# AnishDelft/ModelCompression

Hardware: AMD Instinct MI355X
Metric: images/sec (fwd+bwd, 416x416) (higher is better)
Workload: dtype fp16

## Files before the change

### include/mcamd.h

```cpp
#ifndef MCAMD_H
#define MCAMD_H

#include <stddef.h>
#include <stdint.h>

#ifdef __cplusplus
extern "C" {
#endif

#define MCAMD_OK 0
#define MCAMD_EINVAL (-1)
#define MCAMD_ELAUNCH (-2)
#define MCAMD_EWORKSPACE (-3)

int mcamd_version(void);
void mcamd_reload_config(void);
const char* mcamd_arch(void);
const char* mcamd_last_error(void);

typedef struct mcamd_conv_geom {
    int32_t B, H, W;
    int32_t ksize;
    int32_t cin;
    int32_t cout;
// ... 11 lines not shown
#define MCAMD_EPI_NCHW_F32 1
#define MCAMD_EPI_PAD_F16 2
#define MCAMD_EPI_RAW_F32 3
typedef struct mcamd_conv_epilogue {
    int32_t mode;
    int32_t y_ld, y_choff;
    void* y;
    const float* bias;
    float* stats;
    int32_t stats_rows;
    int32_t stats_ld;
    const float* scale;
    const float* shift;
    float slope;
    int32_t* overflow;
    int32_t dst_mode;
    void* y2;
    int32_t y2_ld, y2_choff;
    int32_t concurrent;
} mcamd_conv_epilogue;

int32_t mcamd_conv_stats_rows(const mcamd_conv_geom* g);
int32_t mcamd_conv_stats_rows_mode(const mcamd_conv_geom* g, int32_t mode);

int mcamd_conv_tile_info(const mcamd_conv_geom* g, int32_t dgrad, int32_t out[4]);

int64_t mcamd_packed_elems_fwd(const mcamd_conv_geom* g);
int64_t mcamd_packed_elems_dgrad(const mcamd_conv_geom* g);

typedef struct mcamd_chan_map {
    const int32_t* rows;
    const int32_t* cols;
} mcamd_chan_map;

int mcamd_pack_weights(const mcamd_conv_geom* g, const float* w_oihw, const float* mask_oihw,
                       const mcamd_chan_map* map, void* wp_fwd, void* wp_dgrad, void* stream);

typedef struct mcamd_pack_job {
    const float* w;
    const float* mask;
    void* dst_fwd;
    void* dst_dgrad;
    const int32_t* rows;
    const int32_t* cols;
    int64_t first_tile;
    int32_t cout, cin, ksize;
    int32_t split;
    int32_t f8_wexp;
} mcamd_pack_job;
int mcamd_pack_weights_many(const mcamd_pack_job* jobs_dev, int32_t njobs, int64_t total_tiles, void* stream);

int mcamd_conv_fwd(const mcamd_conv_geom* g, const void* x, const void* wp_fwd,
                   const mcamd_conv_epilogue* epi, void* stream);

int32_t mcamd_conv_fwd_sparse24_ok(const mcamd_conv_geom* g);
int mcamd_sparse24_elems(const mcamd_conv_geom* g, int64_t out[2]);
int mcamd_pack_sparse24(const mcamd_conv_geom* g, const float* w_oihw, const float* mask_oihw, void* wsp, void* idx, void* stream);
int mcamd_conv_fwd_sparse24(const mcamd_conv_geom* g, const void* x, const void* wsp, const void* idx,
                            const mcamd_conv_epilogue* epi, void* stream);

int32_t mcamd_conv_fwd_q8_ok(const mcamd_conv_geom* g);
int mcamd_q8_elems(const mcamd_conv_geom* g, int64_t out[2]);
int mcamd_pack_q8(const mcamd_conv_geom* g, const float* w_oihw, const float* mask_oihw, void* wq, int32_t* wexp, void* stream);
int mcamd_conv_fwd_q8(const mcamd_conv_geom* g, const void* x8, const void* wq, const int32_t* wexp,
                      const mcamd_conv_epilogue* epi, int32_t y_f8, int32_t y2_f8, void* stream);
int mcamd_cast_q8(const void* src, int64_t pixels, int32_t src_ld, int32_t src_choff, int32_t C, void* dst, int32_t dst_ld,
                  int32_t dst_choff, void* stream);

int32_t mcamd_conv_fwd_q8_stats_rows(const mcamd_conv_geom* g);
int mcamd_fakequant_q8(const mcamd_conv_geom* g, const float* w_oihw, const float* mask_oihw, const int32_t* wexp,
                       float* wq_oihw, void* stream);
int mcamd_cast_q8_train(void* src, int64_t pixels, int32_t src_ld, int32_t src_choff, int32_t C, void* dst, int32_t dst_ld,
                        int32_t dst_choff, void* stream);

int32_t mcamd_conv_fwd_q8_sparse24_ok(const mcamd_conv_geom* g);
int mcamd_q8_sparse24_elems(const mcamd_conv_geom* g, int64_t out[3]);
int mcamd_pack_q8_sparse24(const mcamd_conv_geom* g, const float* w_oihw, const float* mask_oihw, void* wq, void* idx,
                           int32_t* wexp, void* stream);
int mcamd_conv_fwd_q8_sparse24(const mcamd_conv_geom* g, const void* x8, const void* wq, const void* idx, const int32_t* wexp,
                               const mcamd_conv_epilogue* epi, int32_t y_f8, int32_t y2_f8, void* stream);

int mcamd_conv_dgrad(const mcamd_conv_geom* g, const void* dy, int32_t dy_ld, int32_t dy_choff,
                     const void* wp_dgrad, const mcamd_conv_epilogue* epi, void* stream);

size_t mcamd_conv_wgrad_workspace_bytes(const mcamd_conv_geom* g);
int mcamd_conv_wgrad(const mcamd_conv_geom* g, const void* x, const void* dy, int32_t dy_ld,
                     int32_t dy_choff, const float* mask_oihw, const mcamd_chan_map* map,
                     float grad_scale, float* dw_oihw, float* dbias, void* workspace,
                     size_t workspace_bytes, void* stream);

#define MCAMD_WGRAD_GENERIC 0
#define MCAMD_WGRAD_STEM 1
#define MCAMD_WGRAD_WIN 2
#define MCAMD_WGRAD_NINE 3
#define MCAMD_WGRAD_NINE_WIDE 4
#define MCAMD_WFIN_ROW 0
#define MCAMD_WFIN_VEC 1
#define MCAMD_WFIN_GENERIC 2
#define MCAMD_WGRAD_PLAN_INFO_N 13
int mcamd_conv_wgrad_plan_info(const mcamd_conv_geom* g, int32_t has_cmap, int32_t out[MCAMD_WGRAD_PLAN_INFO_N]);
int32_t mcamd_wgrad_generic_instances(int32_t* out, int32_t cap);

int mcamd_bn_coeffs(const float* stats, int32_t stats_rows, int32_t stats_ld, int32_t C, int64_t count,
                    const float* gamma, const float* beta, float* running_mean, float* running_var,
                    float momentum, float eps, int32_t training,
                    float* scale, float* shift, float* save_mean, float* save_invstd,
                    const int32_t* chan_perm, void* stream);

int mcamd_bn_coeffs_ex(const float* stats, int32_t stats_rows, int32_t stats_ld, int32_t C, int64_t count,
                       const float* gamma, const float* beta, float* running_mean, float* running_var,
                       float momentum, float eps, int32_t training,
                       float* scale, float* shift, float* save_mean, float* save_invstd,
                       const int32_t* chan_perm, int32_t ones_channel, void* stream);

#define MCAMD_DST_PLAIN 0
#define MCAMD_DST_POOL 1
#define MCAMD_DST_REORG 2
typedef struct mcamd_act_desc {
    int32_t B, H, W, C;
    const void* y; int32_t y_ld, y_choff;
    const float* scale; const float* shift;
    float slope;
    int32_t mode;
    void* dst; int32_t dst_ld, dst_choff;
    void* dst2; int32_t dst2_ld, dst2_choff;
    int32_t y_dtype;
    int32_t planes;
    int32_t dst_plane, dst2_plane;
    int32_t dst_pad, dst2_pad;
    const float* border;
    int32_t planes2;
    void* pool_act;
    int32_t pool_act_ld, pool_act_pad;
    void* dst_q8;
    void* dst2_q8;
} mcamd_act_desc;
int mcamd_bn_act_fwd(const mcamd_act_desc* d, void* stream);

typedef struct mcamd_act_bwd_desc {
    int32_t B, H, W, C;
    const void* y; int32_t y_ld, y_choff;
    const float* scale; const float* shift; const float* mean; const float* invstd;
    float slope;
    int32_t mode;
    const void* g; int32_t g_ld, g_choff;
    const void* g2; int32_t g2_ld, g2_choff;
    void* dy; int32_t dy_ld, dy_choff;
    float* dgamma; float* dbeta;
    float grad_scale;
    const float* dy_keep;
    const int32_t* chan_perm;
    int32_t y_dtype;
    int32_t* overflow;
    int32_t dy_pad;
    int32_t skip_dead_param_grads;
    const void* act;
    int32_t act_ld, act_choff, act_pad;
    const void* pool_out;
    int32_t pool_out_ld, pool_out_choff, pool_out_pad;
} mcamd_act_bwd_desc;
size_t mcamd_bn_act_bwd_workspace_bytes(const mcamd_act_bwd_desc* d);
int mcamd_bn_act_bwd(const mcamd_act_bwd_desc* d, void* workspace, size_t workspace_bytes, void* stream);

typedef struct mcamd_fold_desc {
    const float* w; const float* mask;
    const int32_t* rows; const int32_t* cols;
    const float* beta; float slope;
    int32_t n, cin_t, cin_k, cin_aug, ksize;
} mcamd_fold_desc;
int mcamd_fold_weights(const mcamd_fold_desc* d, float* waug, void* stream);
typedef struct mcamd_fold_job {
    mcamd_fold_desc d;
    float* waug;
    int64_t first_block;
} mcamd_fold_job;
int mcamd_fold_weights_many(const mcamd_fold_job* jobs_dev, int32_t njobs, int64_t total_blocks, void* stream);
int mcamd_unfold_wgrad(const mcamd_fold_desc* d, const float* dwaug, float* dw_oihw, float* prod_dbeta,
                       float* prod_dgamma, int32_t accumulate, void* stream);

typedef struct mcamd_stem_block_desc {
    int32_t B, H, W;
    const void* x;
    const void* wp;
    const float* gamma; const float* beta;
    float* running_mean; float* running_var;
    float momentum, eps;
    int32_t training;
    float* scale; float* shift; float* save_mean; float* save_invstd;
    float slope;
    void* dst; int32_t dst_ld, dst_choff;
    const void* g; int32_t g_ld, g_choff;
    const float* mask;
    float grad_scale;
    float* dw;
    float* dgamma; float* dbeta;
    int32_t cout;
    int32_t planes;
    const void* x_lo;
    const void* wp_lo;
} mcamd_stem_block_desc;
size_t mcamd_stem_block_workspace_bytes(void);
int mcamd_stem_block_fwd(const mcamd_stem_block_desc* d, void* workspace, size_t workspace_bytes, void* stream);
int mcamd_stem_block_bwd(const mcamd_stem_block_desc* d, void* workspace, size_t workspace_bytes, void* stream);
int32_t mcamd_stem_block_stats_rows(const mcamd_stem_block_desc* d);
int mcamd_stem_block_stats(const mcamd_stem_block_desc* d, float* stats, int32_t stats_rows, int32_t stats_ld, void* stream);

int mcamd_nchw_f32_to_padded_nhwc_f16(const float* src, int32_t B, int32_t C, int32_t H, int32_t W,
                                      float mul, void* dst, int32_t dst_ld, int32_t dst_choff, int32_t* overflow,
                                      void* stream);
int mcamd_nchw_f32_to_padded_nhwc_f16_pad(const float* src, int32_t B, int32_t C, int32_t H, int32_t W,
                                          float mul, void* dst, int32_t dst_ld, int32_t dst_choff, int32_t pad,
                                          int32_t* overflow, void* stream);
int mcamd_nchw_f32_to_padded_nhwc_f16_split(const float* src, int32_t B, int32_t C, int32_t H, int32_t W,
                                            void* dst, int32_t dst_ld, int32_t dst_choff, int32_t plane, void* stream);

int mcamd_nchw_f32_to_nhwc4_split(const float* src, int32_t B, int32_t H, int32_t W, void* hi, void* lo, void* stream);
int mcamd_pack_stem_split(const float* w_oihw, const float* mask_oihw, int32_t cout, void* wp_hi, void* wp_lo, void* stream);

int32_t mcamd_stem_conv_f32_stats_rows(void);
int mcamd_stem_conv_f32(const float* x_nchw, int32_t B, int32_t H, int32_t W, const float* w_oihw,
                        const float* mask_oihw, int32_t cout, float* weff_scratch, float* y, int32_t y_ld,
                        float* stats, int32_t stats_rows, int32_t stats_ld, void* stream);

typedef struct mcamd_region_desc {
    const float* output; const float* target;
    int32_t B, H, W, num_anchors, num_classes, max_boxes;
    float anchors[16];
    float coord_scale, noobject_scale, object_scale, class_scale, thresh;
} mcamd_region_desc;
size_t mcamd_region_loss_workspace_bytes(int32_t B);
int mcamd_region_loss(const mcamd_region_desc* d, float* loss, float* grad, int32_t* counts, void* workspace,
                      size_t workspace_bytes, void* stream);

typedef struct mcamd_augment_desc {
    int64_t src_off;
    int64_t tmp_off;
    int32_t src_w, src_h;
    int32_t crop_x, crop_y;
    int32_t crop_w, crop_h;
    int32_t flip;
    int32_t hk, vk;
    int32_t hcoef_off, vcoef_off;
// ... 50 lines not shown
```

### modelcompression_amd/_lib.py

```python
import ctypes as C
import os

_HERE = os.path.dirname(os.path.abspath(__file__))
LIB_PATH = os.path.join(_HERE, "libmcamd.so")


class McamdError(RuntimeError):
    pass


class ConvGeom(C.Structure):
    _fields_ = [("B", C.c_int32), ("H", C.c_int32), ("W", C.c_int32), ("ksize", C.c_int32),
                ("cin", C.c_int32), ("cout", C.c_int32), ("x_ld", C.c_int32), ("x_choff", C.c_int32),
                ("stem", C.c_int32), ("pad", C.c_int32), ("x_wrap", C.c_int32), ("x_f8", C.c_int32), ("x_f8_wexp", C.c_int32)]


class ConvEpilogue(C.Structure):
    _fields_ = [("mode", C.c_int32), ("y_ld", C.c_int32), ("y_choff", C.c_int32),
                ("y", C.c_void_p), ("bias", C.c_void_p), ("stats", C.c_void_p),
                ("stats_rows", C.c_int32), ("stats_ld", C.c_int32),
                ("scale", C.c_void_p), ("shift", C.c_void_p), ("slope", C.c_float), ("overflow", C.c_void_p),
                ("dst_mode", C.c_int32), ("y2", C.c_void_p), ("y2_ld", C.c_int32), ("y2_choff", C.c_int32),
                ("concurrent", C.c_int32)]


class ActDesc(C.Structure):
    _fields_ = [("B", C.c_int32), ("H", C.c_int32), ("W", C.c_int32), ("C", C.c_int32),
                ("y", C.c_void_p), ("y_ld", C.c_int32), ("y_choff", C.c_int32),
                ("scale", C.c_void_p), ("shift", C.c_void_p), ("slope", C.c_float), ("mode", C.c_int32),
                ("dst", C.c_void_p), ("dst_ld", C.c_int32), ("dst_choff", C.c_int32),
                ("dst2", C.c_void_p), ("dst2_ld", C.c_int32), ("dst2_choff", C.c_int32),
                ("y_dtype", C.c_int32), ("planes", C.c_int32), ("dst_plane", C.c_int32), ("dst2_plane", C.c_int32),
                ("dst_pad", C.c_int32), ("dst2_pad", C.c_int32), ("border", C.c_void_p), ("planes2", C.c_int32),
                ("pool_act", C.c_void_p), ("pool_act_ld", C.c_int32), ("pool_act_pad", C.c_int32),
                ("dst_q8", C.c_void_p), ("dst2_q8", C.c_void_p)]


class ChanMap(C.Structure):
    _fields_ = [("rows", C.c_void_p), ("cols", C.c_void_p)]


class PackJob(C.Structure):
    _fields_ = [("w", C.c_void_p), ("mask", C.c_void_p), ("dst_fwd", C.c_void_p), ("dst_dgrad", C.c_void_p),
                ("rows", C.c_void_p), ("cols", C.c_void_p),
                ("first_tile", C.c_int64), ("cout", C.c_int32), ("cin", C.c_int32), ("ksize", C.c_int32),
                ("split", C.c_int32), ("f8_wexp", C.c_int32)]


class ActBwdDesc(C.Structure):
    _fields_ = [("B", C.c_int32), ("H", C.c_int32), ("W", C.c_int32), ("C", C.c_int32),
                ("y", C.c_void_p), ("y_ld", C.c_int32), ("y_choff", C.c_int32),
                ("scale", C.c_void_p), ("shift", C.c_void_p), ("mean", C.c_void_p), ("invstd", C.c_void_p),
                ("slope", C.c_float), ("mode", C.c_int32),
                ("g", C.c_void_p), ("g_ld", C.c_int32), ("g_choff", C.c_int32),
                ("g2", C.c_void_p), ("g2_ld", C.c_int32), ("g2_choff", C.c_int32),
                ("dy", C.c_void_p), ("dy_ld", C.c_int32), ("dy_choff", C.c_int32),
                ("dgamma", C.c_void_p), ("dbeta", C.c_void_p), ("grad_scale", C.c_float),
                ("dy_keep", C.c_void_p), ("chan_perm", C.c_void_p), ("y_dtype", C.c_int32),
                ("overflow", C.c_void_p), ("dy_pad", C.c_int32), ("skip_dead_param_grads", C.c_int32),
                ("act", C.c_void_p), ("act_ld", C.c_int32), ("act_choff", C.c_int32), ("act_pad", C.c_int32),
                ("pool_out", C.c_void_p), ("pool_out_ld", C.c_int32), ("pool_out_choff", C.c_int32),
                ("pool_out_pad", C.c_int32)]


class FoldDesc(C.Structure):
    _fields_ = [("w", C.c_void_p), ("mask", C.c_void_p), ("rows", C.c_void_p), ("cols", C.c_void_p),
                ("beta", C.c_void_p), ("slope", C.c_float),
                ("n", C.c_int32), ("cin_t", C.c_int32), ("cin_k", C.c_int32), ("cin_aug", C.c_int32), ("ksize", C.c_int32)]


class StemBlockDesc(C.Structure):
    _fields_ = [("B", C.c_int32), ("H", C.c_int32), ("W", C.c_int32),
                ("x", C.c_void_p), ("wp", C.c_void_p), ("gamma", C.c_void_p), ("beta", C.c_void_p),
                ("running_mean", C.c_void_p), ("running_var", C.c_void_p),
                ("momentum", C.c_float), ("eps", C.c_float), ("training", C.c_int32),
                ("scale", C.c_void_p), ("shift", C.c_void_p), ("save_mean", C.c_void_p), ("save_invstd", C.c_void_p),
                ("slope", C.c_float),
                ("dst", C.c_void_p), ("dst_ld", C.c_int32), ("dst_choff", C.c_int32),
                ("g", C.c_void_p), ("g_ld", C.c_int32), ("g_choff", C.c_int32),
                ("mask", C.c_void_p), ("grad_scale", C.c_float),
                ("dw", C.c_void_p), ("dgamma", C.c_void_p), ("dbeta", C.c_void_p), ("cout", C.c_int32), ("planes", C.c_int32),
                ("x_lo", C.c_void_p), ("wp_lo", C.c_void_p)]


class RegionDesc(C.Structure):
    _fields_ = [("output", C.c_void_p), ("target", C.c_void_p),
                ("B", C.c_int32), ("H", C.c_int32), ("W", C.c_int32), ("num_anchors", C.c_int32), ("num_classes", C.c_int32),
                ("max_boxes", C.c_int32), ("anchors", C.c_float * 16),
                ("coord_scale", C.c_float), ("noobject_scale", C.c_float), ("object_scale", C.c_float),
                ("class_scale", C.c_float), ("thresh", C.c_float)]


class FoldJob(C.Structure):
    _fields_ = [("d", FoldDesc), ("waug", C.c_void_p), ("first_block", C.c_int64)]


class AugmentDesc(C.Structure):
    _fields_ = [("src_off", C.c_int64), ("tmp_off", C.c_int64),
                ("src_w", C.c_int32), ("src_h", C.c_int32), ("crop_x", C.c_int32), ("crop_y", C.c_int32),
                ("crop_w", C.c_int32), ("crop_h", C.c_int32), ("flip", C.c_int32),
                ("hk", C.c_int32), ("vk", C.c_int32), ("hcoef_off", C.c_int32), ("vcoef_off", C.c_int32),
                ("lut_off", C.c_int32)]


class AugmentBatch(C.Structure):
    _fields_ = [("desc", C.c_void_p), ("desc_dev", C.c_void_p),
                ("src", C.c_void_p), ("src_bytes", C.c_int64),
                ("coef", C.c_void_p), ("coef_elems", C.c_int64),
                ("lut", C.c_void_p), ("lut_bytes", C.c_int64),
                ("tmp", C.c_void_p), ("tmp_bytes", C.c_int64),
                ("out", C.c_void_p), ("B", C.c_int32), ("H", C.c_int32), ("W", C.c_int32)]


EPI_RAW_F16, EPI_NCHW_F32, EPI_PAD_F16, EPI_RAW_F32 = 0, 1, 2, 3
DST_PLAIN, DST_POOL, DST_REORG = 0, 1, 2
WGRAD_GENERIC, WGRAD_STEM, WGRAD_WIN, WGRAD_NINE, WGRAD_NINE_WIDE = 0, 1, 2, 3, 4
WFIN_ROW, WFIN_VEC, WFIN_GENERIC = 0, 1, 2
WGRAD_PLAN_INFO_N = 13

_P, _I32, _I64, _F, _SZ = C.c_void_p, C.c_int32, C.c_int64, C.c_float, C.c_size_t
SIGNATURES = {
    "mcamd_version": (C.c_int, []),
    "mcamd_arch": (C.c_char_p, []),
    "mcamd_last_error": (C.c_char_p, []),
    "mcamd_reload_config": (None, []),
    "mcamd_conv_stats_rows": (_I32, [C.POINTER(ConvGeom)]),
    "mcamd_conv_stats_rows_mode": (_I32, [C.POINTER(ConvGeom), _I32]),
    "mcamd_conv_fwd_f8_ok": (_I32, [C.POINTER(ConvGeom)]),
    "mcamd_conv_tile_info": (C.c_int, [C.POINTER(ConvGeom), _I32, C.POINTER(_I32)]),
    "mcamd_packed_elems_fwd": (_I64, [C.POINTER(ConvGeom)]),
    "mcamd_packed_elems_dgrad": (_I64, [C.POINTER(ConvGeom)]),
    "mcamd_pack_weights": (C.c_int, [C.POINTER(ConvGeom), _P, _P, C.POINTER(ChanMap), _P, _P, _P]),
    "mcamd_pack_weights_many": (C.c_int, [_P, _I32, _I64, _P]),
    "mcamd_conv_fwd": (C.c_int, [C.POINTER(ConvGeom), _P, _P, C.POINTER(ConvEpilogue), _P]),
    "mcamd_conv_fwd_sparse24_ok": (_I32, [C.POINTER(ConvGeom)]),
    "mcamd_sparse24_elems": (C.c_int, [C.POINTER(ConvGeom), C.POINTER(_I64)]),
    "mcamd_pack_sparse24": (C.c_int, [C.POINTER(ConvGeom), _P, _P, _P, _P, _P]),
    "mcamd_conv_fwd_sparse24": (C.c_int, [C.POINTER(ConvGeom), _P, _P, _P, C.POINTER(ConvEpilogue), _P]),
    "mcamd_conv_fwd_q8_ok": (_I32, [C.POINTER(ConvGeom)]),
    "mcamd_q8_elems": (C.c_int, [C.POINTER(ConvGeom), C.POINTER(_I64)]),
    "mcamd_pack_q8": (C.c_int, [C.POINTER(ConvGeom), _P, _P, _P, _P, _P]),
    "mcamd_conv_fwd_q8": (C.c_int, [C.POINTER(ConvGeom), _P, _P, _P, C.POINTER(ConvEpilogue), _I32, _I32, _P]),
    "mcamd_conv_fwd_q8_sparse24_ok": (_I32, [C.POINTER(ConvGeom)]),
    "mcamd_q8_sparse24_elems": (C.c_int, [C.POINTER(ConvGeom), C.POINTER(_I64)]),
    "mcamd_pack_q8_sparse24": (C.c_int, [C.POINTER(ConvGeom), _P, _P, _P, _P, _P, _P]),
    "mcamd_conv_fwd_q8_sparse24": (C.c_int, [C.POINTER(ConvGeom), _P, _P, _P, _P, C.POINTER(ConvEpilogue), _I32, _I32, _P]),
    "mcamd_cast_q8": (C.c_int, [_P, _I64, _I32, _I32, _I32, _P, _I32, _I32, _P]),
    "mcamd_conv_fwd_q8_stats_rows": (_I32, [C.POINTER(ConvGeom)]),
    "mcamd_fakequant_q8": (C.c_int, [C.POINTER(ConvGeom), _P, _P, _P, _P, _P]),
    "mcamd_cast_q8_train": (C.c_int, [_P, _I64, _I32, _I32, _I32, _P, _I32, _I32, _P]),
    "mcamd_conv_dgrad": (C.c_int, [C.POINTER(ConvGeom), _P, _I32, _I32, _P, C.POINTER(ConvEpilogue), _P]),
    "mcamd_conv_wgrad_workspace_bytes": (_SZ, [C.POINTER(ConvGeom)]),
    "mcamd_conv_wgrad": (C.c_int, [C.POINTER(ConvGeom), _P, _P, _I32, _I32, _P, C.POINTER(ChanMap), _F, _P, _P, _P, _SZ, _P]),
    "mcamd_conv_wgrad_plan_info": (C.c_int, [C.POINTER(ConvGeom), _I32, C.POINTER(_I32)]),
    "mcamd_wgrad_generic_instances": (_I32, [C.POINTER(_I32), _I32]),
    "mcamd_bn_coeffs": (C.c_int, [_P, _I32, _I32, _I32, _I64, _P, _P, _P, _P, _F, _F, _I32, _P, _P, _P, _P, _P, _P]),
    "mcamd_bn_coeffs_ex": (C.c_int, [_P, _I32, _I32, _I32, _I64, _P, _P, _P, _P, _F, _F, _I32, _P, _P, _P, _P, _P, _I32, _P]),
    "mcamd_fold_weights": (C.c_int, [C.POINTER(FoldDesc), _P, _P]),
    "mcamd_fold_weights_many": (C.c_int, [_P, _I32, _I64, _P]),
    "mcamd_unfold_wgrad": (C.c_int, [C.POINTER(FoldDesc), _P, _P, _P, _P, _I32, _P]),
    "mcamd_bn_act_fwd": (C.c_int, [C.POINTER(ActDesc), _P]),
    "mcamd_bn_act_bwd_workspace_bytes": (_SZ, [C.POINTER(ActBwdDesc)]),
    "mcamd_bn_act_bwd": (C.c_int, [C.POINTER(ActBwdDesc), _P, _SZ, _P]),
    "mcamd_stem_block_workspace_bytes": (_SZ, []),
    "mcamd_stem_block_fwd": (C.c_int, [C.POINTER(StemBlockDesc), _P, _SZ, _P]),
    "mcamd_stem_block_bwd": (C.c_int, [C.POINTER(StemBlockDesc), _P, _SZ, _P]),
    "mcamd_stem_block_stats_rows": (_I32, [C.POINTER(StemBlockDesc)]),
    "mcamd_stem_block_stats": (C.c_int, [C.POINTER(StemBlockDesc), _P, _I32, _I32, _P]),
    "mcamd_nchw_f32_to_nhwc4_split": (C.c_int, [_P, _I32, _I32, _I32, _P, _P, _P]),
    "mcamd_pack_stem_split": (C.c_int, [_P, _P, _I32, _P, _P, _P]),
    "mcamd_nchw_f32_to_padded_nhwc_f16": (C.c_int, [_P, _I32, _I32, _I32, _I32, _F, _P, _I32, _I32, _P, _P]),
    "mcamd_nchw_f32_to_padded_nhwc_f16_pad": (C.c_int, [_P, _I32, _I32, _I32, _I32, _F, _P, _I32, _I32, _I32, _P, _P]),
    "mcamd_nchw_f32_to_padded_nhwc_f16_split": (C.c_int, [_P, _I32, _I32, _I32, _I32, _P, _I32, _I32, _I32, _P]),
    "mcamd_stem_conv_f32_stats_rows": (_I32, []),
    "mcamd_stem_conv_f32": (C.c_int, [_P, _I32, _I32, _I32, _P, _P, _I32, _P, _P, _I32, _P, _I32, _I32, _P]),
    "mcamd_region_loss_workspace_bytes": (_SZ, [_I32]),
    "mcamd_region_loss": (C.c_int, [C.POINTER(RegionDesc), _P, _P, _P, _P, _SZ, _P]),
    "mcamd_augment": (C.c_int, [C.POINTER(AugmentBatch), _P]),
    "mcamd_plan_begin": (C.c_int, [C.POINTER(_P), _I32]),
    "mcamd_plan_mark": (_I32, []),
    "mcamd_plan_end": (_P, []),
    "mcamd_plan_segments": (_I32, [_P]),
    "mcamd_plan_launches": (_I32, [_P]),
    "mcamd_plan_run": (C.c_int, [_P, _I32, _I32, C.POINTER(_P), _I32]),
    "mcamd_plan_destroy": (None, [_P]),
    "mcamd_stream_wait": (C.c_int, [_P, _P]),
    "mcamd_memset_zero": (C.c_int, [_P, _SZ, _P]),
    "mcamd_step_flags": (C.c_int, [_P, _I32, _P, _P, _P, _P, _P]),
    "mcamd_kth_magnitude_workspace_bytes": (_SZ, []),
    "mcamd_kth_magnitude": (C.c_int, [C.POINTER(_P), C.POINTER(_I64), _I32, _I64, _P, _P, _SZ, _P]),
    "mcamd_magnitude_mask": (C.c_int, [_P, _I64, _P, _P, _P]),
    "mcamd_filter_scores_workspace_bytes": (_SZ, [_I32]),
    "mcamd_filter_scores": (C.c_int, [_P, _I32, _I32, _I32, _I32, _P, _P, _SZ, _P]),
    "mcamd_filter_mean_square": (C.c_int, [_P, _I32, _I32, _I32, _I32, _P, _P, _SZ, _P]),
    "mcamd_filter_mask": (C.c_int, [_P, _I32, _I64, _P, _P]),
    "mcamd_count_zeros": (C.c_int, [_P, _I64, _P, _P]),
    "mcamd_masked_residual": (C.c_int, [_P, _P, _I64, _P, _P]),
    "mcamd_nm_mask": (C.c_int, [_P, _P, _I32, _I32, _I32, _I32, _I32, _P, _P]),
    "mcamd_nm_violations": (C.c_int, [_P, _I32, _I32, _I32, _P, _P]),
}

_lib = None


def lib():
    global _lib
    if _lib is None:
        if not os.path.exists(LIB_PATH):
            raise McamdError(
                "libmcamd.so is missing (%s). Build it with `python -m modelcompression_amd.build`; "
                "modelcompression_amd has no CPU/PyTorch fallback for its compute path." % LIB_PATH)
        import torch
        h = C.CDLL(LIB_PATH)
        for name, (res, args) in SIGNATURES.items():
            fn = getattr(h, name)
            fn.restype = res
            fn.argtypes = args
        _lib = h
    return _lib


def reload_config():
    lib().mcamd_reload_config()


def check(rc, what=""):
    if rc != 0:
        msg = lib().mcamd_last_error().decode()
        raise McamdError("%s failed (%d): %s" % (what or "mcamd call", rc, msg))


def ptr(t):
    return None if t is None else C.c_void_p(t.data_ptr())

# ... 5 lines not shown
```

### modelcompression_amd/csrc/api.hip

```cpp
#include <stdarg.h>
#include <stdlib.h>
#include <string.h>

#include "kernels.h"

static thread_local char g_err[512] = "";

void mcamd_set_error(const char* fmt, ...) {
    va_list ap;
    va_start(ap, fmt);
    vsnprintf(g_err, sizeof(g_err), fmt, ap);
    va_end(ap);
}

int g_mcamd_env_generation = 0;
int McamdEnvSlot::get(const char* name, int dflt) {
    const int g = __atomic_load_n(&g_mcamd_env_generation, __ATOMIC_ACQUIRE);
    if (gen != g) {
        const char* s = getenv(name);
        has = s && *s ? 1 : 0;
        val = has ? atoi(s) : 0;
        __atomic_store_n(&gen, g, __ATOMIC_RELEASE);
    }
    return has ? val : dflt;
// ... 607 lines not shown
    return (int32_t)(((long long)g->B * g->H * g->W + MCAMD_Q8_TILE_M - 1) / MCAMD_Q8_TILE_M);
}

extern "C" int mcamd_fakequant_q8(const mcamd_conv_geom* g, const float* w_oihw, const float* mask_oihw, const int32_t* wexp,
                                  float* wq_oihw, void* stream) {
    if (mcamd_recording()) {
        MCAMD_REQUIRE(g, "fakequant_q8: null geometry");
        const mcamd_conv_geom g_ = *g;
        return mcamd_rec_push(stream, [=](void* s) { return mcamd_fakequant_q8(&g_, w_oihw, mask_oihw, wexp, wq_oihw, s); });
    }
    MCAMD_REQUIRE(g && mcamd_conv_fwd_q8_ok(g), "fakequant_q8: geometry has no fp8 form (mcamd_conv_fwd_q8_ok)");
    MCAMD_REQUIRE(w_oihw && wexp && wq_oihw, "fakequant_q8: null pointer");
    return mcamd_fakequant_q8_launch(w_oihw, mask_oihw, wexp, wq_oihw, g->cout, g->cin, ntaps_of(g), (hipStream_t)stream);
}

extern "C" int32_t mcamd_conv_fwd_q8_sparse24_ok(const mcamd_conv_geom* g) {
    return mcamd_conv_fwd_q8_ok(g);
}

extern "C" int mcamd_q8_sparse24_elems(const mcamd_conv_geom* g, int64_t out[3]) {
    MCAMD_REQUIRE(g && out, "q8_sparse24_elems: null argument");
    MCAMD_REQUIRE(mcamd_conv_fwd_q8_sparse24_ok(g), "q8_sparse24_elems: geometry has no 2:4 fp8 form (mcamd_conv_fwd_q8_sparse24_ok)");
    const long long npad = round_up_int(g->cout, 256), ktot = (long long)ntaps_of(g) * g->cin;
    out[0] = npad * ktot / 2;
    out[1] = npad * ktot / 32;
    out[2] = npad;
    return MCAMD_OK;
}

extern "C" int mcamd_pack_q8_sparse24(const mcamd_conv_geom* g, const float* w_oihw, const float* mask_oihw, void* wq, void* idx,
                                      int32_t* wexp, void* stream) {
    if (mcamd_recording()) {
        MCAMD_REQUIRE(g, "pack_q8_sparse24: null geometry");
        const mcamd_conv_geom g_ = *g;
        return mcamd_rec_push(stream, [=](void* s) { return mcamd_pack_q8_sparse24(&g_, w_oihw, mask_oihw, wq, idx, wexp, s); });
    }
    MCAMD_REQUIRE(g && mcamd_conv_fwd_q8_sparse24_ok(g), "pack_q8_sparse24: geometry has no 2:4 fp8 form (mcamd_conv_fwd_q8_sparse24_ok)");
    MCAMD_REQUIRE(w_oihw && wq && idx && wexp, "pack_q8_sparse24: null pointer");
    return mcamd_pack_q8_sparse24_launch(w_oihw, mask_oihw, wq, idx, wexp, g->cout, g->cin, ntaps_of(g), (hipStream_t)stream);
}

extern "C" int mcamd_conv_fwd_q8_sparse24(const mcamd_conv_geom* g, const void* x8, const void* wq, const void* idx,
                                          const int32_t* wexp, const mcamd_conv_epilogue* epi, int32_t y_f8, int32_t y2_f8,
                                          void* stream) {
    if (mcamd_recording()) {
        MCAMD_REQUIRE(g && epi, "conv_fwd_q8_sparse24: null geometry / epilogue");
        const mcamd_conv_geom g_ = *g;
        const mcamd_conv_epilogue e_ = *epi;
        return mcamd_rec_push(stream, [=](void* s) { return mcamd_conv_fwd_q8_sparse24(&g_, x8, wq, idx, wexp, &e_, y_f8, y2_f8, s); });
    }
    if (check_geom(g, "conv_fwd_q8_sparse24")) return MCAMD_EINVAL;
    MCAMD_REQUIRE(mcamd_conv_fwd_q8_sparse24_ok(g), "conv_fwd_q8_sparse24: geometry has no 2:4 fp8 form (mcamd_conv_fwd_q8_sparse24_ok)");
    MCAMD_REQUIRE(x8 && wq && idx && wexp, "conv_fwd_q8_sparse24: null input");
    MCAMD_REQUIRE(epi && epi->mode == MCAMD_EPI_PAD_F16, "conv_fwd_q8_sparse24: epilogue mode 2 (MCAMD_EPI_PAD_F16) only");
    IgemmArgs a;
    fill_operand(a, g, x8, wq, g->x_ld, g->x_choff, g->cout, g->cin, 0);
    if (fill_epilogue(a, epi, g->cout, "conv_fwd_q8_sparse24", 0)) return MCAMD_EINVAL;
    return mcamd_conv_q8_sparse_launch(a, idx, wexp, y_f8 != 0, y2_f8 != 0, (hipStream_t)stream);
}

static int cast_q8_any(const void* src, int64_t pixels, int32_t src_ld, int32_t src_choff, int32_t C, void* dst, int32_t dst_ld,
                       int32_t dst_choff, int back, void* stream) {
    MCAMD_REQUIRE(src && dst && pixels > 0 && C > 0, "cast_q8: null pointer / empty");
    MCAMD_REQUIRE(C % 8 == 0 && src_ld % 8 == 0 && src_choff % 8 == 0 && dst_ld % 8 == 0 && dst_choff % 8 == 0 &&
                      src_choff >= 0 && dst_choff >= 0 && src_choff + C <= src_ld && dst_choff + C <= dst_ld,
                  "cast_q8: channel slices must be multiples of 8 inside their leading dimensions");
    return mcamd_cast_q8_launch(src, pixels, src_ld, src_choff, C, dst, dst_ld, dst_choff, back, (hipStream_t)stream);
}

extern "C" int mcamd_cast_q8(const void* src, int64_t pixels, int32_t src_ld, int32_t src_choff, int32_t C, void* dst,
                             int32_t dst_ld, int32_t dst_choff, void* stream) {
    if (mcamd_recording())
        return mcamd_rec_push(stream, [=](void* s) { return mcamd_cast_q8(src, pixels, src_ld, src_choff, C, dst, dst_ld, dst_choff, s); });
    return cast_q8_any(src, pixels, src_ld, src_choff, C, dst, dst_ld, dst_choff, 0, stream);
}

extern "C" int mcamd_cast_q8_train(void* src, int64_t pixels, int32_t src_ld, int32_t src_choff, int32_t C, void* dst,
                                   int32_t dst_ld, int32_t dst_choff, void* stream) {
    if (mcamd_recording())
        return mcamd_rec_push(stream, [=](void* s) { return mcamd_cast_q8_train(src, pixels, src_ld, src_choff, C, dst, dst_ld, dst_choff, s); });
    return cast_q8_any(src, pixels, src_ld, src_choff, C, dst, dst_ld, dst_choff, 1, stream);
}

extern "C" int mcamd_conv_dgrad(const mcamd_conv_geom* g, const void* dy, int32_t dy_ld, int32_t dy_choff,
                                const void* wp_dgrad, const mcamd_conv_epilogue* epi, void* stream) {
    if (mcamd_recording()) {
        MCAMD_REQUIRE(g && epi, "conv_dgrad: null geometry / epilogue");
        const mcamd_conv_geom g_ = *g;
        const mcamd_conv_epilogue e_ = *epi;
        return mcamd_rec_push(stream, [=](void* s) { return mcamd_conv_dgrad(&g_, dy, dy_ld, dy_choff, wp_dgrad, &e_, s); });
    }
    if (check_geom(g, "conv_dgrad")) return MCAMD_EINVAL;
    MCAMD_REQUIRE(g->x_wrap == 0 && g->x_f8 == 0, "conv_dgrad: x_wrap / x_f8 are forward-only fields");
    MCAMD_REQUIRE(!g->stem, "conv_dgrad: the stem layer has no input gradient");
    MCAMD_REQUIRE(dy && wp_dgrad, "conv_dgrad: null input");
    int cout_p = cout_p_of(g);
    MCAMD_REQUIRE(dy_ld % 8 == 0 && dy_choff % 8 == 0 && dy_choff + cout_p <= dy_ld,
                  "conv_dgrad: dy slice [%d, %d) does not fit dy_ld %d", dy_choff, dy_choff + cout_p, dy_ld);
    IgemmArgs a;
    fill_operand(a, g, dy, wp_dgrad, dy_ld, dy_choff, g->cin, cout_p, 0);
    MCAMD_REQUIRE(epi && epi->mode != MCAMD_EPI_PAD_F16 && !epi->stats && epi->dst_mode == 0 && !epi->y2,
                  "conv_dgrad: epilogue must be mode 0 (no stats) or 1");
    a.concurrent = epi->concurrent != 0;
    const ConvRoute r = conv_route(g, a.concurrent ? DIR_DGRAD_CONCURRENT : DIR_DGRAD, epi->mode, MCAMD_DST_PLAIN, false);
    if (fill_epilogue(a, epi, g->cin, "conv_dgrad", r.rows)) return MCAMD_EINVAL;
    return launch_route(a, r, g, (hipStream_t)stream);
}

static WgradPlan wgrad_plan_for(const mcamd_conv_geom* g) {
    if (mcamd_wgrad_stem_ok(g->stem, g->cout, g->W, (long long)g->B * g->H * g->W))
        return mcamd_wgrad_stem_plan((long long)g->B * g->H * g->W);
    if (mcamd_wgrad_win_ok(g->ksize, g->stem, g->cout, cin_tap_of(g), g->W, (long long)g->B * g->H * g->W))
        return mcamd_wgrad_win_plan((long long)g->B * g->H * g->W, g->cout);
    if (mcamd_wgrad_use9(g->ksize, g->stem, g->cout, cin_tap_of(g), g->W))
        return mcamd_wgrad_plan9(padded_pixels(g), g->cout, cin_tap_of(g), g->W, g->W + pw_of(g), g->B);
    return mcamd_wgrad_plan((long long)g->B * g->H * g->W, g->cout, cin_tap_of(g), ntaps_of(g));
}

extern "C" size_t mcamd_conv_wgrad_workspace_bytes(const mcamd_conv_geom* g) {
    if (!g) return 0;
    return wgrad_plan_for(g).bytes;
}

extern "C" int mcamd_conv_wgrad_plan_info(const mcamd_conv_geom* g, int32_t has_cmap, int32_t out[MCAMD_WGRAD_PLAN_INFO_N]) {
    if (check_geom(g, "conv_wgrad_plan_info")) return MCAMD_EINVAL;
    MCAMD_REQUIRE(out, "conv_wgrad_plan_info: null output");
    MCAMD_REQUIRE(!(g->stem && has_cmap), "conv_wgrad_plan_info: the stem layer takes no input-channel map");
    const WgradPlan p = wgrad_plan_for(g);
    const WgradFinish f = mcamd_wgrad_finish_pick(p.nsplit, g->stem, g->cin, g->ksize, has_cmap != 0);
    const int tiles = p.n_otiles * p.n_tapgroups * p.n_ctiles;
    out[0] = p.nine == 2 ? MCAMD_WGRAD_NINE_WIDE : p.nine ? MCAMD_WGRAD_NINE : p.stemw == 1 ? MCAMD_WGRAD_STEM
             : p.stemw == 2 ? MCAMD_WGRAD_WIN : MCAMD_WGRAD_GENERIC;
    out[1] = p.tmo, out[2] = p.tnc, out[3] = p.taps, out[4] = p.kp, out[5] = p.ns;
    out[6] = p.nsplit, out[7] = p.pix_per_split, out[8] = p.rows_pad;
    out[9] = f.kernel, out[10] = f.sg;
    out[11] = tiles;
    out[12] = p.stemw ? p.nsplit : round_up_int(tiles * p.nsplit, 8);
    return MCAMD_OK;
}

extern "C" int32_t mcamd_wgrad_generic_instances(int32_t* out, int32_t cap) {
    static_assert(sizeof(int32_t) == sizeof(int), "instance tuples are copied as int");
    return mcamd_wgrad_instances((int (*)[4])out, out ? cap : 0);
}

extern "C" int mcamd_conv_wgrad(const mcamd_conv_geom* g, const void* x, const void* dy, int32_t dy_ld, int32_t dy_choff,
                                const float* mask_oihw, const mcamd_chan_map* map, float grad_scale, float* dw_oihw,
                                float* dbias, void* workspace, size_t workspace_bytes, void* stream) {
    if (mcamd_recording()) {
        MCAMD_REQUIRE(g, "conv_wgrad: null geometry");
        const mcamd_conv_geom g_ = *g;
        const bool has_map = map != nullptr;
        const mcamd_chan_map m_ = has_map ? *map : mcamd_chan_map{nullptr, nullptr};
        return mcamd_rec_push(stream, [=](void* s) {
            return mcamd_conv_wgrad(&g_, x, dy, dy_ld, dy_choff, mask_oihw, has_map ? &m_ : nullptr, grad_scale, dw_oihw, dbias,
                                    workspace, workspace_bytes, s);
        });
    }
    if (check_geom(g, "conv_wgrad")) return MCAMD_EINVAL;
    MCAMD_REQUIRE(g->x_wrap == 0 && g->x_f8 == 0, "conv_wgrad: x_wrap / x_f8 are forward-only fields");
    MCAMD_REQUIRE(x && dy && dw_oihw && workspace, "conv_wgrad: null argument");
    MCAMD_REQUIRE(grad_scale > 0.f, "conv_wgrad: grad_scale must be positive");
    const int* rmap = map ? (const int*)map->rows : nullptr;
    const int* cmap = map ? (const int*)map->cols : nullptr;
    MCAMD_REQUIRE(!(g->stem && cmap), "conv_wgrad: the stem layer takes no input-channel map");
    const int cin_tap = cin_tap_of(g), ntaps = ntaps_of(g);
    const long long M = (long long)g->B * g->H * g->W;
    WgradPlan p = wgrad_plan_for(g);
    MCAMD_REQUIRE(dy_ld % 8 == 0 && dy_choff % 8 == 0 && dy_choff + p.rows_pad <= dy_ld,
                  "conv_wgrad: dy slice [%d, %d) does not fit dy_ld %d", dy_choff, dy_choff + p.rows_pad, dy_ld);
    if (workspace_bytes < p.bytes) {
        mcamd_set_error("conv_wgrad: workspace %zu < %zu bytes", workspace_bytes, p.bytes);
        return MCAMD_EWORKSPACE;
    }
    hipStream_t st = (hipStream_t)stream;
    WgradArgs a;
    memset(&a, 0, sizeof(a));
    a.x = (const half_t*)x;
    a.dy = (const half_t*)dy;
    a.slab = (float*)workspace;
    a.x_ld = g->x_ld;
    a.x_row_stride = (g->W + pw_of(g)) * g->x_ld;
    a.x_img_stride = (long long)(g->H + pw_of(g)) * a.x_row_stride;
    a.x_off = g->x_choff;
    a.dy_ld = dy_ld;
    a.dy_row_stride = (g->W + pw_of(g)) * dy_ld;
    a.dy_img_stride = (long long)(g->H + pw_of(g)) * a.dy_row_stride;
    a.dy_off = dy_choff + a.dy_row_stride + dy_ld;
    a.dy_zero_off = dy_choff;
// ... 22 lines not shown
```

### modelcompression_amd/csrc/bn_act.hip

```cpp
#include "common.h"
#include "conv_epi.h"

constexpr int RED_CPB = 8, RED_RG = 128;

__device__ __forceinline__ double shfl_xor_f64(double v, int m) {
    int lo = __double2loint(v), hi = __double2hiint(v);
    lo = __shfl_xor(lo, m);
    hi = __shfl_xor(hi, m);
    return __hiloint2double(hi, lo);
}

__device__ __forceinline__ void block_reduce2(double& a, double& b, double (*red)[16][RED_CPB]) {
    const int lane = threadIdx.x & 63, wave = threadIdx.x >> 6, cx = threadIdx.x & (RED_CPB - 1);
#pragma unroll
    for (int m = RED_CPB; m < 64; m <<= 1) {
        a += shfl_xor_f64(a, m);
        b += shfl_xor_f64(b, m);
    }
    if (lane < RED_CPB) {
        red[0][wave][cx] = a;
        red[1][wave][cx] = b;
    }
    __syncthreads();
    if (threadIdx.x < RED_CPB) {
// ... 421 lines not shown
            }
        }
    }
    if (PHASE == 1 && sat && a.overflow) atomicOr(a.overflow, 1);

    if (PHASE == 0) {
        block_partials_to_slab(sb, sg, CH, a.slab, a.C);
    }
}

template <int PHASE, bool Y32>
__global__ __launch_bounds__(256) void bn_plain_bwd_kernel(ActBwdArgs a) {
    const int CH = a.C >> 3, lg = __ffs(CH) - 1;
    const int c8 = (threadIdx.x & (CH - 1)) * 8;
    float sc[8], sh[8], mu[8], is[8], A[8], Bc[8], dm[8];
    loadf8(a.scale + c8, sc);
    loadf8(a.shift + c8, sh);
    loadf8(a.mean + c8, mu);
    loadf8(a.invstd + c8, is);
    if (PHASE == 1) {
        float c1[8], c2[8];
        loadf8(a.coef + c8, c1);
        loadf8(a.coef + a.C + c8, c2);
        if (a.dy_keep) {
            float kp[8];
            loadf8(a.dy_keep + c8, kp);
#pragma unroll
            for (int i = 0; i < 8; ++i) dm[i] = kp[i] != 0.f ? sc[i] : 0.f;
        } else {
#pragma unroll
            for (int i = 0; i < 8; ++i) dm[i] = sc[i];
        }
#pragma unroll
        for (int i = 0; i < 8; ++i) {
            Bc[i] = dm[i] * c2[i] * is[i];
            A[i] = dm[i] * c1[i] - Bc[i] * mu[i];
        }
    }
    float sb[8], sg[8];
#pragma unroll
    for (int i = 0; i < 8; ++i) sb[i] = sg[i] = 0.f;
    float satmax = 0.f;
    const int HW = a.H * a.W;
    const unsigned npix = (unsigned)(a.items >> lg);
    const unsigned stride = (gridDim.x * 256u) >> lg;
    unsigned pix = (blockIdx.x * 256u + threadIdx.x) >> lg;
    int b = (int)(pix / (unsigned)HW), rem = (int)(pix - (unsigned)b * (unsigned)HW);
    int h = rem / a.W, w = rem - h * a.W;
    const int sb_ = (int)(stride / (unsigned)HW), srem = (int)(stride - (unsigned)sb_ * (unsigned)HW);
    const int sh_ = srem / a.W, sw_ = srem - sh_ * a.W;
    for (; pix < npix; pix += stride) {
        float yv[8], gv[8];
        load_y<Y32>(a.y, (long long)pix * a.y_ld + a.y_choff + c8, yv);
        load8(a.g + (long long)pix * a.g_ld + a.g_choff + c8, gv);
        float out[8];
#pragma unroll
        for (int i = 0; i < 8; ++i) {
            const float z = yv[i] * sc[i] + sh[i];
            const float gz = z > 0.f ? gv[i] : gv[i] * a.slope;
            if (PHASE == 0) {
                sb[i] += gz;
                sg[i] += gz * ((yv[i] - mu[i]) * is[i]);
            } else {
                const float o = dm[i] * gz - (Bc[i] * yv[i] + A[i]);
                out[i] = o;
                satmax = fmaxf(satmax, fabsf(o));
            }
        }
        if (PHASE == 1) {
            store8(a.dy + pad_off(b, h, w, a.H, a.W, a.dy_ld, a.dy_pw) + a.dy_choff + c8, out);
            w += sw_;
            if (w >= a.W) w -= a.W, ++h;
            h += sh_;
            if (h >= a.H) h -= a.H, ++b;
            b += sb_;
        }
    }
    if (PHASE == 1 && satmax > 65504.f && a.overflow) atomicOr(a.overflow, 1);
    if (PHASE == 0) {
        block_partials_to_slab(sb, sg, CH, a.slab, a.C);
    }
}

constexpr float BN_ACT_T = 0.03125f;

__device__ __forceinline__ bool act_xhat_source(const float (&sc)[8], const float (&sh)[8], const float (&mu)[8],
                                                const float (&is)[8], bool have_y, float (&off)[8], float (&mul)[8],
                                                bool (&usey)[8]) {
    bool any = false;
#pragma unroll
    for (int i = 0; i < 8; ++i) {
        const float beta = sh[i] + mu[i] * sc[i];
        usey[i] = have_y && fabsf(sc[i]) < BN_ACT_T * fmaxf(fabsf(beta), 1.f) * is[i];
        off[i] = usey[i] ? mu[i] : beta;
        mul[i] = usey[i] ? is[i] : (sc[i] != 0.f ? is[i] / sc[i] : 0.f);
        any |= usey[i];
    }
    return any;
}

template <int PHASE>
__global__ __launch_bounds__(256) void bn_plain_bwd_act_kernel(ActBwdArgs a) {
    const int CH = a.C >> 3, lg = __ffs(CH) - 1;
    const int c8 = (threadIdx.x & (CH - 1)) * 8;
    float sc[8], sh[8], mu[8], is[8], off[8], mul[8], P[8], Q[8], dm[8];
    bool usey[8];
    loadf8(a.scale + c8, sc);
    loadf8(a.shift + c8, sh);
    loadf8(a.mean + c8, mu);
    loadf8(a.invstd + c8, is);
    const bool need_y = act_xhat_source(sc, sh, mu, is, a.y != nullptr, off, mul, usey);
    if (PHASE == 1) {
        float c1[8], c2[8];
        loadf8(a.coef + c8, c1);
        loadf8(a.coef + a.C + c8, c2);
        if (a.dy_keep) {
            float kp[8];
            loadf8(a.dy_keep + c8, kp);
#pragma unroll
            for (int i = 0; i < 8; ++i) dm[i] = kp[i] != 0.f ? sc[i] : 0.f;
        } else {
#pragma unroll
            for (int i = 0; i < 8; ++i) dm[i] = sc[i];
        }
#pragma unroll
        for (int i = 0; i < 8; ++i) {
            P[i] = dm[i] * c2[i] * mul[i];
            Q[i] = dm[i] * c1[i] - P[i] * off[i];
        }
    }
    float sb[8], sg[8];
#pragma unroll
    for (int i = 0; i < 8; ++i) sb[i] = sg[i] = 0.f;
    float satmax = 0.f;
    const float inv_slope = 1.0f / a.slope;
    const int HW = a.H * a.W;
    const unsigned npix = (unsigned)(a.items >> lg);
    const unsigned stride = (gridDim.x * 256u) >> lg;
    unsigned pix = (blockIdx.x * 256u + threadIdx.x) >> lg;
    int b = (int)(pix / (unsigned)HW), rem = (int)(pix - (unsigned)b * (unsigned)HW);
    int h = rem / a.W, w = rem - h * a.W;
    const int sb_ = (int)(stride / (unsigned)HW), srem = (int)(stride - (unsigned)sb_ * (unsigned)HW);
    const int sh_ = srem / a.W, sw_ = srem - sh_ * a.W;
    for (; pix < npix; pix += stride) {
        float av[8], gv[8];
        load8(a.act + pad_off(b, h, w, a.H, a.W, a.act_ld, a.act_pw) + a.act_choff + c8, av);
        load8(a.g + (long long)pix * a.g_ld + a.g_choff + c8, gv);
        float out[8], z[8];
#pragma unroll
        for (int i = 0; i < 8; ++i) z[i] = av[i] > 0.f ? av[i] : av[i] * inv_slope;
        if (need_y) {
            float yv[8];
            load_y<true>(a.y, (long long)pix * a.y_ld + a.y_choff + c8, yv);
#pragma unroll
            for (int i = 0; i < 8; ++i) z[i] = usey[i] ? yv[i] : z[i];
        }
#pragma unroll
        for (int i = 0; i < 8; ++i) {
            const float gz = av[i] > 0.f ? gv[i] : gv[i] * a.slope;
            if (PHASE == 0) {
                sb[i] += gz;
                sg[i] += gz * ((z[i] - off[i]) * mul[i]);
            } else {
                const float o = dm[i] * gz - (P[i] * z[i] + Q[i]);
                out[i] = o;
                satmax = fmaxf(satmax, fabsf(o));
            }
        }
        if (PHASE == 1) store8(a.dy + pad_off(b, h, w, a.H, a.W, a.dy_ld, a.dy_pw) + a.dy_choff + c8, out);
        w += sw_;
        if (w >= a.W) w -= a.W, ++h;
        h += sh_;
        if (h >= a.H) h -= a.H, ++b;
        b += sb_;
    }
    if (PHASE == 1 && satmax > 65504.f && a.overflow) atomicOr(a.overflow, 1);
    if (PHASE == 0) {
        block_partials_to_slab(sb, sg, CH, a.slab, a.C);
    }
}

template <int PHASE, bool Y32, bool G2>
// ... 327 lines not shown
                }
        }
#pragma unroll
        for (int i = 0; i < 8; ++i) {
            if (r == 0) best[i] = av[0][i], ys[i] = yv[0][i];
#pragma unroll
            for (int k = r == 0 ? 1 : 0; k < 2; ++k) {
                const bool gt = av[k][i] > best[i];
                best[i] = gt ? av[k][i] : best[i], ys[i] = gt ? yv[k][i] : ys[i];
            }
        }
    }
#pragma unroll
    for (int i = 0; i < 8; ++i) z[i] = usey[i] ? ys[i] : z[i];
}
template <bool ACT>
__global__ __launch_bounds__(256) void bn_pool_sums_kernel(ActBwdArgs a) {
    const int CH = a.C >> 3, lg = __ffs(CH) - 1;
    const int c8 = (threadIdx.x & (CH - 1)) * 8;
    float sc[8], sh[8], mu[8], is[8], off[8], mul[8];
    bool usey[8];
    loadf8(a.scale + c8, sc);
    loadf8(a.shift + c8, sh);
    loadf8(a.mean + c8, mu);
    loadf8(a.invstd + c8, is);
    const bool need_y = act_xhat_source(sc, sh, mu, is, a.y != nullptr, off, mul, usey);
    float sb[8], sg[8];
#pragma unroll
    for (int i = 0; i < 8; ++i) sb[i] = sg[i] = 0.f;
    const float inv_slope = 1.0f / a.slope;
    const int Ho = a.H >> 1, Wo = a.W >> 1, HoWo = Ho * Wo;
    const unsigned npix = (unsigned)(a.items >> lg);
    const unsigned stride = (gridDim.x * 256u) >> lg;
    PoolPos p0 = pool_pos((blockIdx.x * 256u + threadIdx.x) >> lg, HoWo, Wo);
    const half_t* pout = a.pool_out + a.pool_out_choff + c8;
    const half_t* gp = a.g + a.g_choff + c8;
    auto add = [&](const float (&z)[8], const float (&pv)[8], const float (&gv)[8]) {
#pragma unroll
        for (int i = 0; i < 8; ++i) {
            const float gz = pv[i] > 0.f ? gv[i] : gv[i] * a.slope;
            sb[i] += gz;
            sg[i] += gz * ((z[i] - off[i]) * mul[i]);
        }
    };
    auto window = [&](const PoolPos& p, float (&pv)[8], float (&gv)[8]) {
        load8(pout + pad_off(p.b, p.ho, p.wo, Ho, Wo, a.pool_out_ld, a.pool_out_pw), pv);
        load8(gp + (long long)p.pix * a.g_ld, gv);
    };
    auto z_of = [&](const float (&pv)[8], float (&z)[8]) {
#pragma unroll
        for (int i = 0; i < 8; ++i) z[i] = pv[i] > 0.f ? pv[i] : pv[i] * inv_slope;
    };
    if (need_y) {
        const PoolPos step = pool_pos(stride, HoWo, Wo);
        for (; p0.pix < npix; pool_pos_step(p0, step, Ho, Wo)) {
            float pv[8], gv[8], z[8];
            window(p0, pv, gv);
            z_of(pv, z);
            pool_sums_z_from_y<ACT>(a, p0, c8, usey, sc, sh, z);
            add(z, pv, gv);
        }
    } else {
        const PoolPos step2 = pool_pos(2u * stride, HoWo, Wo);
        PoolPos p1 = pool_pos(p0.pix + stride, HoWo, Wo);
        for (; p1.pix < npix; pool_pos_step(p0, step2, Ho, Wo), pool_pos_step(p1, step2, Ho, Wo)) {
            float pv0[8], gv0[8], pv1[8], gv1[8], z[8];
            window(p0, pv0, gv0);
            window(p1, pv1, gv1);
            z_of(pv0, z);
            add(z, pv0, gv0);
            z_of(pv1, z);
            add(z, pv1, gv1);
        }
        if (p0.pix < npix) {
            float pv[8], gv[8], z[8];
            window(p0, pv, gv);
            z_of(pv, z);
            add(z, pv, gv);
        }
    }
    block_partials_to_slab(sb, sg, CH, a.slab, a.C);
}

__global__ __launch_bounds__(1024) void bn_bwd_finalize_kernel(const float* slab, int nblocks, int C, double count,
                                                               float inv_scale, float* dgamma, float* dbeta,
                                                               float* coef, const int* perm, int skip_from) {
    __shared__ double red[2][16][RED_CPB];
    const int cx = threadIdx.x & (RED_CPB - 1), ry = threadIdx.x / RED_CPB;
    const int c = blockIdx.x * RED_CPB + cx;
    double sb = 0.0, sg = 0.0;
    if (c < C) {
        for (int p = ry; p < nblocks; p += RED_RG) {
            sb += (double)slab[((long long)p * 2 + 0) * C + c];
            sg += (double)slab[((long long)p * 2 + 1) * C + c];
        }
    }
    block_reduce2(sb, sg, red);
    if (ry != 0 || c >= C) return;
    const int pc = perm ? perm[c] : c;
    const bool skip = skip_from > 0 && c >= skip_from;
    if (dbeta && !skip) dbeta[pc] = (float)(sb * inv_scale);
    if (dgamma && !skip) dgamma[pc] = (float)(sg * inv_scale);
    coef[c] = (float)(sb / count);
    coef[C + c] = (float)(sg / count);
}

__global__ __launch_bounds__(256) void nchw_to_nhwc_kernel(const float* src, int B, int C, int H, int W, float mul,
                                                           half_t* dst, int ld, int choff, int cgroups, int* overflow,
                                                           int plane, int pw) {
    bool sat = false;
    const long long HW = (long long)H * W;
    const long long items = (long long)B * HW * cgroups;
    for (long long item = (long long)blockIdx.x * 256 + threadIdx.x; item < items; item += (long long)gridDim.x * 256) {
        long long pg = item / ((long long)B * HW);
        long long pix = item - pg * (long long)B * HW;
        int b = (int)(pix / HW);
        int rem = (int)(pix - (long long)b * HW);
        int h = rem / W, w = rem - h * W;
        int c0 = (int)pg * 8;
        half_t* d = dst + pad_off(b, h, w, H, W, ld, pw) + choff + c0;
        const float* s = src + ((long long)b * C + c0) * HW + rem;
        int nc = C - c0 < 8 ? C - c0 : 8;
        if (overflow)
            for (int i = 0; i < nc; ++i) sat |= fabsf(s[i * HW] * mul) > 65504.f;
        if (plane > 0) {
            for (int i = 0; i < nc; ++i) {
                const float v = s[i * HW] * mul;
                const half_t hi = sat_half(v);
                d[i] = hi;
                d[plane + i] = (half_t)(v - (float)hi);
                d[2 * plane + i] = hi;
            }
        } else if (ld == 4) {
            h4_t q;
#pragma unroll
            for (int i = 0; i < 4; ++i) q[i] = (i < nc) ? sat_half(s[i * HW] * mul) : (half_t)0.f;
            *(h4_t*)d = q;
        } else if (nc == 8) {
            float v[8];
#pragma unroll
            for (int i = 0; i < 8; ++i) v[i] = s[i * HW] * mul;
            store8(d, v);
        } else {
            for (int i = 0; i < nc; ++i) d[i] = sat_half(s[i * HW] * mul);
        }
    }
    if (sat && overflow) atomicOr(overflow, 1);
}

static int stream_grid(long long items) {
    long long g = (items + 255) / 256;
    if (g > 4096) g = 4096;
    if (g < 1) g = 1;
    return (int)g;
}

extern "C" int mcamd_bn_coeffs_ex(const float* stats, int32_t stats_rows, int32_t stats_ld, int32_t C, int64_t count,
                                  const float* gamma, const float* beta, float* running_mean, float* running_var,
                                  float momentum, float eps, int32_t training, float* scale, float* shift,
                                  float* save_mean, float* save_invstd, const int32_t* chan_perm, int32_t ones_channel,
                                  void* stream) {
    if (mcamd_recording())
        return mcamd_rec_push(stream, [=](void* s) {
            return mcamd_bn_coeffs_ex(stats, stats_rows, stats_ld, C, count, gamma, beta, running_mean, running_var, momentum, eps,
                                      training, scale, shift, save_mean, save_invstd, chan_perm, ones_channel, s);
        });
    MCAMD_REQUIRE(C > 0 && gamma && beta && running_mean && running_var && scale && shift, "bn_coeffs: null argument");
    MCAMD_REQUIRE(!training || (stats && stats_rows > 0 && stats_ld >= C && count > 0), "bn_coeffs: bad statistics slab");
    MCAMD_REQUIRE(ones_channel < C, "bn_coeffs: ones_channel %d outside the %d channels", ones_channel, C);
    hipLaunchKernelGGL(bn_coeffs_kernel, dim3((C + RED_CPB - 1) / RED_CPB), dim3(1024), 0, (hipStream_t)stream, stats, stats_rows,
                       stats_ld, C, (double)count, gamma, beta, running_mean, running_var, momentum, eps, training,
                       scale, shift, save_mean, save_invstd, (const int*)chan_perm, ones_channel < 0 ? -1 : ones_channel);
    MCAMD_LAUNCH_CHECK("bn_coeffs");
    return MCAMD_OK;
}

extern "C" int mcamd_bn_coeffs(const float* stats, int32_t stats_rows, int32_t stats_ld, int32_t C, int64_t count,
// ... 136 lines not shown
    float* coef = (float*)workspace + (size_t)kBwdBlocks * 2 * d->C;
    a.coef = coef;
    a.dy_keep = d->dy_keep;
    a.overflow = (int*)d->overflow;
    a.B = d->B, a.H = d->H, a.W = d->W, a.C = d->C;
    a.y_ld = d->y_ld, a.y_choff = d->y_choff, a.g_ld = d->g_ld, a.g_choff = d->g_choff;
    a.g2_ld = d->g2_ld, a.g2_choff = d->g2_choff, a.dy_ld = d->dy_ld, a.dy_choff = d->dy_choff;
    MCAMD_REQUIRE(d->dy_pad == 0 || d->dy_pad == 1, "bn_act_bwd: dy_pad must be 0 or 1");
    a.dy_pw = d->dy_pad ? 1 : 2;
    a.slope = d->slope;
    a.act = (const half_t*)d->act;
    a.act_ld = d->act_ld, a.act_choff = d->act_choff;
    a.act_pw = d->act_pad ? 1 : 2;
    if (d->act) {
        MCAMD_REQUIRE((d->mode == MCAMD_DST_PLAIN && !d->g2) || d->mode == MCAMD_DST_POOL,
                      "bn_act_bwd: `act` (backward from the stored activation) is for PLAIN blocks without a second gradient "
                      "and for MaxPool blocks (a full-resolution copy of the activation)");
        MCAMD_REQUIRE(d->act_ld % 8 == 0 && d->act_choff % 8 == 0 && d->act_choff + d->C <= d->act_ld &&
                          (d->act_pad == 0 || d->act_pad == 1),
                      "bn_act_bwd: activation slice [%d, %d) does not fit act_ld %d", d->act_choff, d->act_choff + d->C, d->act_ld);
        MCAMD_REQUIRE(d->slope > 0.f, "bn_act_bwd: `act` needs an invertible activation (slope > 0)");
        MCAMD_REQUIRE(!d->y || d->y_dtype == 1, "bn_act_bwd: with `act`, `y` is NULL or the fp32 raw output (read for the "
                                                "channels with |gamma| < %g max(|beta|, 1) only)", (double)BN_ACT_T);
    }
    a.pool_out = MCAMD_ENV_INT("MCAMD_BN_POOL_SUMS_POOLED", 1) != 0 ? (const half_t*)d->pool_out : nullptr;
    a.pool_out_ld = d->pool_out_ld, a.pool_out_choff = d->pool_out_choff;
    a.pool_out_pw = d->pool_out_pad ? 1 : 2;
    if (d->pool_out) {
        MCAMD_REQUIRE(d->mode == MCAMD_DST_POOL && !d->g2 && (d->act || (d->y && y32)) && d->slope > 0.f,
                      "bn_act_bwd: `pool_out` (sums from the pooled activation) is for MaxPool blocks without a second gradient, "
                      "with `act` or an fp32 `y`, and an invertible activation (slope > 0)");
        MCAMD_REQUIRE(d->pool_out_ld % 8 == 0 && d->pool_out_choff % 8 == 0 && d->pool_out_choff + d->C <= d->pool_out_ld &&
                          (d->pool_out_pad == 0 || d->pool_out_pad == 1),
                      "bn_act_bwd: pooled activation slice [%d, %d) does not fit pool_out_ld %d", d->pool_out_choff,
                      d->pool_out_choff + d->C, d->pool_out_ld);
    }
    long long pixels = (long long)d->B * d->H * d->W;
    double count = (double)pixels;
    if (d->mode != MCAMD_DST_PLAIN) pixels /= 4;
    a.items = pixels * (d->C / 8);
    int grid = stream_grid(a.items);
    const int max_blocks = MCAMD_ENV_INT("MCAMD_BN_BWD_BLOCKS", kBwdBlocks);
    if (grid > kBwdBlocks) grid = kBwdBlocks;
    if (max_blocks >= 1 && grid > max_blocks) grid = max_blocks;
    hipStream_t st = (hipStream_t)stream;
#define BWD_INST(MODE_, PHASE)                                                                                     \
    do {                                                                                                          \
        if (y32) hipLaunchKernelGGL((bn_act_bwd_kernel<MODE_, PHASE, true>), dim3(grid), dim3(256), 0, st, a);    \
        else hipLaunchKernelGGL((bn_act_bwd_kernel<MODE_, PHASE, false>), dim3(grid), dim3(256), 0, st, a);       \
    } while (0)
#define BWD_LAUNCH(PHASE)                                                                                         \
    if (d->mode == MCAMD_DST_PLAIN)                                                                               \
        BWD_INST(MCAMD_DST_PLAIN, PHASE);                                                                         \
    else if (d->mode == MCAMD_DST_POOL)                                                                           \
        BWD_INST(MCAMD_DST_POOL, PHASE);                                                                          \
    else if (d->mode == MCAMD_DST_REORG)                                                                          \
        BWD_INST(MCAMD_DST_REORG, PHASE);                                                                         \
    else                                                                                                          \
        MCAMD_REQUIRE(false, "bn_act_bwd: bad mode %d", d->mode);
    const bool pool_fast_on = MCAMD_ENV_INT("MCAMD_BN_POOL_FAST", 1) != 0;
    const bool pool_fast = pool_fast_on && d->mode == MCAMD_DST_POOL && a.items < (1ll << 31) &&
                           (unsigned long long)grid * 256ull < (1ull << 31);
#define POOL_INST(PHASE, Y32_, G2_) hipLaunchKernelGGL((bn_pool_bwd_kernel<PHASE, Y32_, G2_>), dim3(grid), dim3(256), 0, st, a)
#define POOL_LAUNCH(PHASE)                                                                                        \
    do {                                                                                                          \
        if (a.act && d->g2) hipLaunchKernelGGL((bn_pool_bwd_act_kernel<PHASE, true>), dim3(grid), dim3(256), 0, st, a);   \
        else if (a.act) hipLaunchKernelGGL((bn_pool_bwd_act_kernel<PHASE, false>), dim3(grid), dim3(256), 0, st, a);      \
        else if (y32 && d->g2) POOL_INST(PHASE, true, true);                                                      \
        else if (y32) POOL_INST(PHASE, true, false);                                                              \
        else if (d->g2) POOL_INST(PHASE, false, true);                                                            \
        else POOL_INST(PHASE, false, false);                                                                      \
    } while (0)
    const bool plain_fast = MCAMD_ENV_INT("MCAMD_BN_PLAIN_FAST", 1) != 0 &&
                            d->mode == MCAMD_DST_PLAIN && !d->g2 && a.items < (1ll << 31) &&
                            (unsigned long long)grid * 256ull < (1ull << 31);
    MCAMD_REQUIRE(!d->act || plain_fast || pool_fast, "bn_act_bwd: `act` needs the plain / pool fast path (fewer than 2^31 items, "
                                                      "MCAMD_BN_POOL_FAST / MCAMD_BN_PLAIN_FAST not 0)");
#define PLAIN_LAUNCH(PHASE)                                                                                       \
    do {                                                                                                          \
        if (a.act) hipLaunchKernelGGL((bn_plain_bwd_act_kernel<PHASE>), dim3(grid), dim3(256), 0, st, a);         \
        else if (y32) hipLaunchKernelGGL((bn_plain_bwd_kernel<PHASE, true>), dim3(grid), dim3(256), 0, st, a);    \
        else hipLaunchKernelGGL((bn_plain_bwd_kernel<PHASE, false>), dim3(grid), dim3(256), 0, st, a);            \
    } while (0)
    if (pool_fast && a.pool_out && a.act) hipLaunchKernelGGL(bn_pool_sums_kernel<true>, dim3(grid), dim3(256), 0, st, a);
    else if (pool_fast && a.pool_out) hipLaunchKernelGGL(bn_pool_sums_kernel<false>, dim3(grid), dim3(256), 0, st, a);
    else if (pool_fast) POOL_LAUNCH(0);
    else if (plain_fast) PLAIN_LAUNCH(0);
    else {
        BWD_LAUNCH(0)
    }
    MCAMD_LAUNCH_CHECK("bn_act_bwd reduce");
    hipLaunchKernelGGL(bn_bwd_finalize_kernel, dim3((d->C + RED_CPB - 1) / RED_CPB), dim3(1024), 0, st, (const float*)a.slab, grid, d->C,
                       count, 1.0f / d->grad_scale, d->dgamma, d->dbeta, coef, (const int*)d->chan_perm,
                       d->skip_dead_param_grads);
    MCAMD_LAUNCH_CHECK("bn_act_bwd finalize");
    if (pool_fast) POOL_LAUNCH(1);
    else if (plain_fast) PLAIN_LAUNCH(1);
    else {
        BWD_LAUNCH(1)
    }
    MCAMD_LAUNCH_CHECK("bn_act_bwd apply");
#undef POOL_LAUNCH
#undef PLAIN_LAUNCH
#undef POOL_INST
#undef BWD_LAUNCH
#undef BWD_INST
    return MCAMD_OK;
}

extern "C" int mcamd_nchw_f32_to_padded_nhwc_f16(const float* src, int32_t B, int32_t C, int32_t H, int32_t W, float mul,
                                                 void* dst, int32_t dst_ld, int32_t dst_choff, int32_t* overflow,
                                                 void* stream) {
    if (mcamd_recording())
        return mcamd_rec_push(stream, [=](void* s) {
            return mcamd_nchw_f32_to_padded_nhwc_f16(src, B, C, H, W, mul, dst, dst_ld, dst_choff, overflow, s);
        });
    MCAMD_REQUIRE(src && dst && B > 0 && C > 0 && H > 0 && W > 0, "nchw_to_nhwc: bad argument");
    MCAMD_REQUIRE(dst_choff + C <= dst_ld || dst_ld == 4, "nchw_to_nhwc: channel slice exceeds ld");
    MCAMD_REQUIRE((C >= 8) ? (dst_ld % 8 == 0 && dst_choff % 8 == 0) : true, "nchw_to_nhwc: alignment");
    int cgroups = (C + 7) / 8;
    long long items = (long long)B * H * W * cgroups;
    hipLaunchKernelGGL(nchw_to_nhwc_kernel, dim3(stream_grid(items)), dim3(256), 0, (hipStream_t)stream, src, B, C, H, W,
                       mul, (half_t*)dst, dst_ld, dst_choff, cgroups, (int*)overflow, 0, 2);
    MCAMD_LAUNCH_CHECK("nchw_to_nhwc");
    return MCAMD_OK;
}

extern "C" int mcamd_nchw_f32_to_padded_nhwc_f16_pad(const float* src, int32_t B, int32_t C, int32_t H, int32_t W, float mul,
                                                     void* dst, int32_t dst_ld, int32_t dst_choff, int32_t pad,
                                                     int32_t* overflow, void* stream) {
    if (mcamd_recording())
        return mcamd_rec_push(stream, [=](void* s) {
            return mcamd_nchw_f32_to_padded_nhwc_f16_pad(src, B, C, H, W, mul, dst, dst_ld, dst_choff, pad, overflow, s);
        });
    MCAMD_REQUIRE(src && dst && B > 0 && C > 0 && H > 0 && W > 0 && (pad == 0 || pad == 1), "nchw_to_nhwc_pad: bad argument");
    MCAMD_REQUIRE(dst_choff + C <= dst_ld && dst_ld != 4, "nchw_to_nhwc_pad: channel slice exceeds ld (and not the stem image)");
    MCAMD_REQUIRE((C >= 8) ? (dst_ld % 8 == 0 && dst_choff % 8 == 0) : true, "nchw_to_nhwc_pad: alignment");
    int cgroups = (C + 7) / 8;
    long long items = (long long)B * H * W * cgroups;
    hipLaunchKernelGGL(nchw_to_nhwc_kernel, dim3(stream_grid(items)), dim3(256), 0, (hipStream_t)stream, src, B, C, H, W,
                       mul, (half_t*)dst, dst_ld, dst_choff, cgroups, (int*)overflow, 0, pad ? 1 : 2);
    MCAMD_LAUNCH_CHECK("nchw_to_nhwc_pad");
    return MCAMD_OK;
}

extern "C" int mcamd_nchw_f32_to_padded_nhwc_f16_split(const float* src, int32_t B, int32_t C, int32_t H, int32_t W,
                                                       void* dst, int32_t dst_ld, int32_t dst_choff, int32_t plane,
                                                       void* stream) {
    if (mcamd_recording())
        return mcamd_rec_push(stream, [=](void* s) {
            return mcamd_nchw_f32_to_padded_nhwc_f16_split(src, B, C, H, W, dst, dst_ld, dst_choff, plane, s);
        });
    MCAMD_REQUIRE(src && dst && B > 0 && C > 0 && H > 0 && W > 0, "nchw_to_nhwc_split: bad argument");
    MCAMD_REQUIRE(plane >= C && dst_choff + 2 * plane + C <= dst_ld, "nchw_to_nhwc_split: three planes of %d channels, %d apart, exceed ld %d",
                  C, plane, dst_ld);
    int cgroups = (C + 7) / 8;
    long long items = (long long)B * H * W * cgroups;
    hipLaunchKernelGGL(nchw_to_nhwc_kernel, dim3(stream_grid(items)), dim3(256), 0, (hipStream_t)stream, src, B, C, H, W,
                       1.0f, (half_t*)dst, dst_ld, dst_choff, cgroups, (int*)nullptr, plane, 2);
    MCAMD_LAUNCH_CHECK("nchw_to_nhwc_split");
    return MCAMD_OK;
}
```

### modelcompression_amd/csrc/common.h

```cpp
#pragma once
#include <hip/hip_runtime.h>
#include <stdint.h>
#include <stdio.h>

#include <mutex>

#include "../../include/mcamd.h"

typedef _Float16 half_t;
typedef _Float16 h8_t __attribute__((ext_vector_type(8)));
typedef _Float16 h4_t __attribute__((ext_vector_type(4)));
typedef _Float16 h2_t __attribute__((ext_vector_type(2)));
typedef float f32x16_t __attribute__((ext_vector_type(16)));
typedef float f32x4_t __attribute__((ext_vector_type(4)));
typedef __fp16 fp16x4_t __attribute__((__vector_size__(4 * sizeof(__fp16))));
typedef int i32x8_t __attribute__((ext_vector_type(8)));
typedef int i32x4_t __attribute__((ext_vector_type(4)));
typedef int i32x2_t __attribute__((ext_vector_type(2)));

#define MCAMD_WAVE 64

#define MCAMD_LDS_OPT_IN(kernel, bytes)                                                                       \
    do {                                                                                                      \
        static std::once_flag once_;                                                                          \
        std::call_once(once_, [&] {                                                                           \
            (void)hipFuncSetAttribute((const void*)(kernel), hipFuncAttributeMaxDynamicSharedMemorySize,      \
                                      (int)(bytes));                                                          \
        });                                                                                                   \
    } while (0)

void mcamd_set_error(const char* fmt, ...);

extern int g_mcamd_env_generation;
struct McamdEnvSlot {
    int gen = -1, has = 0, val = 0;
    int get(const char* name, int dflt);
};
#define MCAMD_ENV_INT(name, dflt) (([]() -> McamdEnvSlot* { static McamdEnvSlot slot_; return &slot_; }())->get(name, dflt))

#define MCAMD_REQUIRE(cond, ...)            \
    do {                                    \
        if (!(cond)) {                      \
            mcamd_set_error(__VA_ARGS__);   \
            return MCAMD_EINVAL;            \
        }                                   \
    } while (0)

#define MCAMD_LAUNCH_CHECK(what)                                                    \
    do {                                                                            \
        hipError_t e_ = hipGetLastError();                                          \
        if (e_ != hipSuccess) {                                                     \
            mcamd_set_error("%s: launch failed: %s", what, hipGetErrorString(e_));  \
            return MCAMD_ELAUNCH;                                                   \
        }                                                                           \
    } while (0)

#include <functional>
struct mcamd_plan;
extern thread_local mcamd_plan* g_mcamd_rec;
static inline bool mcamd_recording() { return g_mcamd_rec != nullptr; }
int mcamd_rec_push(void* stream, std::function<int(void*)> fn);

static inline int round_up_int(int v, int m) { return (v + m - 1) / m * m; }
static inline long long round_up_ll(long long v, long long m) { return (v + m - 1) / m * m; }

__device__ __forceinline__ int mfma32_row(int reg, int lane) { return (reg & 3) + 8 * (reg >> 2) + 4 * (lane >> 5); }

__device__ __forceinline__ void glds16(const void* gsrc, void* lds_wave_base) {
    __builtin_amdgcn_global_load_lds((const __attribute__((address_space(1))) void*)gsrc,
                                     (__attribute__((address_space(3))) void*)lds_wave_base, 16, 0, 0);
}

template <int N>
__device__ __forceinline__ void wait_vmcnt() {
    asm volatile("s_waitcnt vmcnt(%0)" ::"n"(N) : "memory");
}

__device__ __forceinline__ long long pad_off(int b, int h, int w, int H, int W, int ld, int pw = 2) {
    return (((long long)b * (H + pw) + h + 1) * (W + pw) + w + 1) * ld;
}

template <int CPR>
__device__ __forceinline__ int swz(int row) {
    return CPR == 4 ? ((row >> 2) & 3) : ((row >> 1) & 7);
}

#define MCAMD_F8_SXL 12
#define MCAMD_F8_SX8 1
#define MCAMD_F8_WEXP_DEFAULT 5
static_assert(MCAMD_F8_SXL == MCAMD_F8_SX8 + 11, "one scale for both correction terms: w_lo is scaled 2^11 above w_hi");
```

### modelcompression_amd/csrc/conv_epi.h

```cpp
#pragma once
#include "kernels.h"

__device__ __forceinline__ void split_image(int p, int HW, int& b, int& hw) {
    b = p / HW;
    hw = p - b * HW;
}
__device__ __forceinline__ void split_pixel(int p, int HW, int W, int& b, int& h, int& w) {
    int r;
    split_image(p, HW, b, r);
    h = r / W;
    w = r - h * W;
}

__device__ __forceinline__ void tile_pixel(const IgemmArgs& __restrict__ a, bool pooled, int m, int& b, int& h, int& w) {
    if (pooled) {
        const int Wo = a.W >> 1, q = m & 3;
        int ho, wo;
        split_pixel(m >> 2, (a.H >> 1) * Wo, Wo, b, ho, wo);
        h = 2 * ho + (q >> 1);
        w = 2 * wo + (q & 1);
    } else {
        split_pixel(m, a.HW, a.W, b, h, w);
    }
}
// ... 49 lines not shown
                                               int mt, int nt, int tid) {
    constexpr int CH = COLS / 8;
    if (a.dst_mode == MCAMD_DST_PLAIN) {
        for (int slot = tid; slot < ROWS * CH; slot += NT) {
            const int row = slot / CH, ch = slot - row * CH;
            const int m = mt * ROWS + row;
            const int n0 = nt * COLS + ch * 8;
            if (m < a.M && n0 < a.N) {
                int b, h, w;
                split_pixel(m, a.HW, a.W, b, h, w);
                put8(a.y, y_f8, pad_off(b, h, w, a.H, a.W, a.y_ld) + a.y_choff + n0, bt, ht, row * PITCH + ch * 8);
            }
        }
        return;
    }
    const int Wo = a.W >> 1, Ho = a.H >> 1, HWo = Ho * Wo;
    if (a.dst_mode == MCAMD_DST_POOL) {
        const bool has2 = a.y2 != nullptr;
        for (int slot = tid; slot < (ROWS / 4) * CH; slot += NT) {
            const int pr = slot / CH, ch = slot - pr * CH;
            const int idx = mt * (ROWS / 4) + pr;
            const int n0 = nt * COLS + ch * 8;
            if (4 * idx < a.M && n0 < a.N) {
                int b, ho, wo;
                split_pixel(idx, HWo, Wo, b, ho, wo);
                const long long off = pad_off(b, ho, wo, Ho, Wo, a.y_ld) + a.y_choff + n0;
                if (y_f8) {
                    unsigned k0 = 0, k1 = 0;
#pragma unroll
                    for (int q = 0; q < 4; ++q) {
                        const i32x2_t v = *(const i32x2_t*)(bt + (4 * pr + q) * PITCH + ch * 8);
                        k0 = e4m3_max4(k0, e4m3_key((unsigned)v[0]));
                        k1 = e4m3_max4(k1, e4m3_key((unsigned)v[1]));
                    }
                    i32x2_t mx;
                    mx[0] = (int)e4m3_unkey(k0), mx[1] = (int)e4m3_unkey(k1);
                    *(i32x2_t*)((char*)a.y + off) = mx;
                } else {
                    h8_t v[4];
#pragma unroll
                    for (int q = 0; q < 4; ++q) v[q] = *(const h8_t*)(ht + (4 * pr + q) * PITCH + ch * 8);
                    h8_t mx;
#pragma unroll
                    for (int e = 0; e < 8; ++e) {
                        const half_t m01 = v[0][e] > v[1][e] ? v[0][e] : v[1][e], m23 = v[2][e] > v[3][e] ? v[2][e] : v[3][e];
                        mx[e] = m01 > m23 ? m01 : m23;
                    }
                    *(h8_t*)((half_t*)a.y + off) = mx;
                }
                if (has2) {
#pragma unroll
                    for (int q = 0; q < 4; ++q)
                        put8(a.y2, y2_f8, pad_off(b, 2 * ho + (q >> 1), 2 * wo + (q & 1), a.H, a.W, a.y2_ld) + a.y2_choff + n0,
                             bt, ht, (4 * pr + q) * PITCH + ch * 8);
                }
            }
        }
    } else {
        for (int slot = tid; slot < ROWS * CH; slot += NT) {
            const int row = slot / CH, ch = slot - row * CH;
            const int m = mt * ROWS + row;
            const int n0 = nt * COLS + ch * 8;
            if (m < a.M && n0 < a.N) {
                int b, ho, wo;
                split_pixel(m >> 2, HWo, Wo, b, ho, wo);
                put8(a.y, y_f8, pad_off(b, ho, wo, Ho, Wo, a.y_ld) + a.y_choff + (m & 3) * a.N + n0, bt, ht, row * PITCH + ch * 8);
            }
        }
    }
}

template <int ROWS, int COLS, int NT>
__device__ __forceinline__ void store_raw_tile(const IgemmArgs& __restrict__ a, const half_t* ct, int mt, int nt, int tid) {
    constexpr int CH = COLS / 8;
    half_t* y = (half_t*)a.y;
    for (int slot = tid; slot < ROWS * CH; slot += NT) {
        const int row = slot / CH, ch = slot - row * CH;
        const int m = mt * ROWS + row;
        const int n0 = nt * COLS + ch * 8;
        if (m < a.M && n0 < a.N) *(h8_t*)(y + (long long)m * a.y_ld + a.y_choff + n0) = *(const h8_t*)(ct + row * COLS + ch * 8);
    }
}

template <int BMW, int PITCH, int WM, int WN, int TM, int TN, class ScaleOf>
__device__ __forceinline__ bool write_ch_tile(const IgemmArgs& __restrict__ a, const f32x16_t (&acc)[TM][TN], ScaleOf scale_of, bool need_b,
                                              bool need_h, char* bt, half_t* ht, int nt, int wm, int wn, int lane) {
    bool sat = false;
#pragma unroll
    for (int i = 0; i < TM; ++i) {
#pragma unroll
        for (int g = 0; g < 4; ++g) {
            const int ch0 = wm * WM + i * 32 + 8 * g + 4 * (lane >> 5);
            float sc[4], sh[4];
#pragma unroll
            for (int e = 0; e < 4; ++e) {
                const int n = nt * BMW + ch0 + e;
                sc[e] = 1.f, sh[e] = 0.f;
                if (n < a.N) {
                    sc[e] = scale_of(n);
                    if (a.shift) sh[e] = a.shift[n];
                }
            }
#pragma unroll
            for (int j = 0; j < TN; ++j) {
                const int pix = wn * WN + j * 32 + (lane & 31);
                float v[4];
#pragma unroll
                for (int e = 0; e < 4; ++e) {
                    v[e] = acc[i][j][4 * g + e] * sc[e] + sh[e];
                    v[e] = v[e] > 0.f ? v[e] : v[e] * a.slope;
                }
                if (need_b) *(int*)(bt + pix * PITCH + ch0) = e4m3_bytes4(v);
                if (need_h) {
                    h4_t hv;
#pragma unroll
                    for (int e = 0; e < 4; ++e) {
                        sat |= fabsf(v[e]) > 65504.f;
                        hv[e] = (half_t)fminf(fmaxf(v[e], -65504.f), 65504.f);
                    }
                    *(h4_t*)(ht + pix * PITCH + ch0) = hv;
                }
            }
        }
    }
    return sat;
}
```

### modelcompression_amd/csrc/conv_igemm.hip

```cpp
#include "kernels.h"
#include "conv_epi.h"
#include <stdlib.h>


template <int BM, int BN, int WM, int WN, int BK, int NSTAGE, int EPI>
__global__ __launch_bounds__((BM / WM) * (BN / WN) * 64,
                              (BN >= 128 ? (NSTAGE * BK <= 96 ? 3 : 2) : (BN >= 64 ? 3 : 4)))
void igemm_kernel(IgemmArgs a) {
    constexpr int WAVES_N = BN / WN;
    constexpr int NT = (BM / WM) * (BN / WN) * 64;
    constexpr int CPR = BK / 8;
    constexpr int A_SLOTS = BM * CPR, B_SLOTS = BN * CPR;
    constexpr int A_IT = (A_SLOTS + NT - 1) / NT, B_IT = (B_SLOTS + NT - 1) / NT;
    constexpr int TM = WM / 32, TN = WN / 32;
    constexpr int STAGE_BYTES = (A_SLOTS + B_SLOTS) * 16;
    constexpr int DMIN = A_SLOTS / NT + B_SLOTS / NT;
    static_assert(A_SLOTS % 64 == 0 && B_SLOTS % 64 == 0, "whole waves per DMA instruction");
    static_assert(NSTAGE >= 2 && NSTAGE <= 4 && DMIN * (NSTAGE - 2) < 64, "vmcnt immediate range");

    extern __shared__ __attribute__((aligned(16))) char smem[];

    const int tid = threadIdx.x;
    const int lane = tid & 63;
    const int wave = __builtin_amdgcn_readfirstlane(tid >> 6);
    const int wm = wave / WAVES_N, wn = wave % WAVES_N;
    int nt, pslot;
    if (a.xcd_order == 0) {
        const int total_items = a.num_ntiles * a.num_pslots;
        const int chunk = (total_items + 7) >> 3;
        const int item = (blockIdx.x & 7) * chunk + (blockIdx.x >> 3);
        if ((int)(blockIdx.x >> 3) >= chunk || item >= total_items) return;
        nt = item / a.num_pslots;
        pslot = item - nt * a.num_pslots;
    } else {
        if (!xcd_tile(a.num_ntiles, a.num_pslots, nt, pslot)) return;
    }
    const int nchunks = a.ktot / BK;
    const int cpt = a.cin_tap / BK;

    long long bbase[B_IT];
#pragma unroll
    for (int it = 0; it < B_IT; ++it) {
        int slot = it * NT + tid;
        int row = slot / CPR, phys = slot % CPR;
        int logical = phys ^ swz<CPR>(row);
        bbase[it] = (long long)(nt * BN + row) * a.ktot + logical * 8;
    }

    float s1[TN], s2[TN];
#pragma unroll
    for (int j = 0; j < TN; ++j) s1[j] = s2[j] = 0.f;
    bool sat = false;

    for (int mt = pslot; mt < a.num_mtiles; mt += a.num_pslots) {
        long long abase[A_IT];
#pragma unroll
        for (int it = 0; it < A_IT; ++it) {
            int slot = it * NT + tid;
            int row = slot / CPR, phys = slot % CPR;
            int logical = phys ^ swz<CPR>(row);
            abase[it] = tile_x_base(a, EPI == MCAMD_EPI_PAD_F16 && a.dst_mode != 0, mt * BM + row) + logical * 8;
        }

        f32x16_t acc[TM][TN];
#pragma unroll
        for (int i = 0; i < TM; ++i)
#pragma unroll
            for (int j = 0; j < TN; ++j)
#pragma unroll
                for (int r = 0; r < 16; ++r) acc[i][j][r] = 0.f;

        auto stage = [&](int q, int buf) {
            const int sub = a.kb / BK > 0 ? a.kb / BK : 1, per_block = a.ntaps * sub;
            const int cb = q / per_block, r = q - cb * per_block;
            const int tap = r / sub;
            int cbo = cb * a.kb;
            if (cbo >= a.wrap) cbo -= a.wrap;
            int koff = a.tap_off[tap] + cbo + (r - tap * sub) * BK;
            char* sa = smem + buf * STAGE_BYTES;
            char* sb = sa + A_SLOTS * 16;
#pragma unroll
            for (int it = 0; it < A_IT; ++it) {
                int wslot = it * NT + wave * 64;
                if (wslot < A_SLOTS) glds16(a.x + abase[it] + koff, sa + wslot * 16);
            }
#pragma unroll
            for (int it = 0; it < B_IT; ++it) {
                int wslot = it * NT + wave * 64;
                if (wslot < B_SLOTS) glds16(a.w + bbase[it] + (long long)q * BK, sb + wslot * 16);
            }
        };

        __syncthreads();
#pragma unroll
        for (int p = 0; p < NSTAGE - 1; ++p)
            if (p < nchunks) stage(p, p);
        int sidx = 0;
        for (int q = 0; q < nchunks; ++q) {
            int issued = q + NSTAGE - 1;
            if (issued > nchunks) issued = nchunks;
            const int inflight = issued - q - 1;
            if (NSTAGE == 2 || inflight == 0) wait_vmcnt<0>();
            else if (inflight == 1) wait_vmcnt<DMIN>();
            else wait_vmcnt<(NSTAGE > 3 ? 2 * DMIN : DMIN)>();
            __builtin_amdgcn_s_barrier();
            if (q + NSTAGE - 1 < nchunks) {
                int ns = sidx + NSTAGE - 1;
                if (ns >= NSTAGE) ns -= NSTAGE;
                stage(q + NSTAGE - 1, ns);
            }
            const char* sa = smem + sidx * STAGE_BYTES;
            const char* sb = sa + A_SLOTS * 16;
            sidx = sidx + 1 == NSTAGE ? 0 : sidx + 1;
            constexpr int KS = BK / 16;
            constexpr int NSET = (TM * TN <= 4) ? 2 : 1;
            h8_t af[NSET][TM], bf[NSET][TN];
            auto load_frags = [&](int s, int set) {
                const int chunk = 2 * s + (lane >> 5);
#pragma unroll
                for (int i = 0; i < TM; ++i) {
                    int row = wm * WM + i * 32 + (lane & 31);
                    af[set][i] = *(const h8_t*)(sa + (row * CPR + (chunk ^ swz<CPR>(row))) * 16);
                }
#pragma unroll
                for (int j = 0; j < TN; ++j) {
                    int row = wn * WN + j * 32 + (lane & 31);
                    bf[set][j] = *(const h8_t*)(sb + (row * CPR + (chunk ^ swz<CPR>(row))) * 16);
                }
            };
            if (NSET == 2) load_frags(0, 0);
#pragma unroll
            for (int s = 0; s < KS; ++s) {
                if (NSET == 2) {
                    if (s + 1 < KS) load_frags(s + 1, (s + 1) & 1);
                    __builtin_amdgcn_sched_barrier(0);
                } else {
                    load_frags(s, 0);
                }
                constexpr int M1 = NSET - 1;
#pragma unroll
                for (int i = 0; i < TM; ++i)
#pragma unroll
                    for (int j = 0; j < TN; ++j)
                        acc[i][j] = __builtin_amdgcn_mfma_f32_32x32x16_f16(af[s & M1][i], bf[s & M1][j], acc[i][j], 0, 0, 0);
                if (NSET == 2) __builtin_amdgcn_sched_barrier(0);
            }
        }

        if constexpr (EPI == MCAMD_EPI_NCHW_F32) {
            float* y = (float*)a.y;
#pragma unroll
            for (int i = 0; i < TM; ++i)
#pragma unroll
                for (int r = 0; r < 16; ++r) {
                    int m = mt * BM + wm * WM + i * 32 + mfma32_row(r, lane);
                    if (m < a.M) {
                        int b, hw;
                        split_image(m, a.HW, b, hw);
#pragma unroll
                        for (int j = 0; j < TN; ++j) {
                            int n = nt * BN + wn * WN + j * 32 + (lane & 31);
                            if (n < a.N) {
                                float v = acc[i][j][r];
                                if (a.bias) v += a.bias[n];
                                y[((long long)b * a.N + n) * a.HW + hw] = v;
                            }
                        }
                    }
                }
        } else if constexpr (EPI == MCAMD_EPI_RAW_F32) {
            float* y = (float*)a.y;
            const int mlim = a.M - mt * BM;
#pragma unroll
            for (int j = 0; j < TN; ++j) {
                const int n = nt * BN + wn * WN + j * 32 + (lane & 31);
#pragma unroll
                for (int i = 0; i < TM; ++i)
#pragma unroll
                    for (int r = 0; r < 16; ++r) {
                        const int row = wm * WM + i * 32 + mfma32_row(r, lane);
                        const float v = acc[i][j][r];
                        if (row < mlim) {
                            if (n < a.N) y[(long long)(mt * BM + row) * a.y_ld + a.y_choff + n] = v;
                            s1[j] += v;
                            s2[j] += v * v;
                        }
                    }
            }
        } else {
            __syncthreads();
            half_t* ct = (half_t*)smem;
            const int mlim = a.M - mt * BM;
#pragma unroll
            for (int j = 0; j < TN; ++j) {
                const int col = wn * WN + j * 32 + (lane & 31);
                float sc = 1.f, sh = 0.f;
                if constexpr (EPI == MCAMD_EPI_PAD_F16) {
                    int n = nt * BN + col;
                    if (n < a.N) {
                        if (a.scale) sc = a.scale[n];
                        if (a.shift) sh = a.shift[n];
                    }
                }
#pragma unroll
                for (int i = 0; i < TM; ++i)
#pragma unroll
                    for (int r = 0; r < 16; ++r) {
                        const int row = wm * WM + i * 32 + mfma32_row(r, lane);
                        float v = acc[i][j][r];
                        if constexpr (EPI == MCAMD_EPI_PAD_F16) {
                            v = v * sc + sh;
                            v = v > 0.f ? v : v * a.slope;
                        }
                        half_t hv = (half_t)fminf(fmaxf(v, -65504.f), 65504.f);
                        sat |= fabsf(v) > 65504.f;
                        ct[row * BN + col] = hv;
                        if (EPI == MCAMD_EPI_RAW_F16 && a.stats) {
                            float fv = (row < mlim) ? (float)hv : 0.f;
                            s1[j] += fv;
                            s2[j] += fv * fv;
                        }
                    }
            }
            __syncthreads();
            if constexpr (EPI == MCAMD_EPI_PAD_F16) store_pad_tile<BM, BN, BN, NT>(a, nullptr, ct, false, false, mt, nt, tid);
            else store_raw_tile<BM, BN, NT>(a, ct, mt, nt, tid);
        }
    }

    if (sat && a.overflow) atomicOr(a.overflow, 1);
    if ((EPI == MCAMD_EPI_RAW_F16 || EPI == MCAMD_EPI_RAW_F32) && a.stats) {
#pragma unroll
        for (int j = 0; j < TN; ++j) {
            s1[j] += __shfl_xor(s1[j], 32);
            s2[j] += __shfl_xor(s2[j], 32);
        }
        __syncthreads();
        float* red = (float*)smem;
        if (lane < 32) {
#pragma unroll
            for (int j = 0; j < TN; ++j) {
                red[(wm * 2 + 0) * BN + wn * WN + j * 32 + lane] = s1[j];
                red[(wm * 2 + 1) * BN + wn * WN + j * 32 + lane] = s2[j];
            }
        }
        __syncthreads();
        for (int t = tid; t < 2 * BN; t += NT) {
            int which = t / BN, col = t - which * BN;
            float v = 0.f;
#pragma unroll
            for (int k = 0; k < BM / WM; ++k) v += red[(k * 2 + which) * BN + col];
            a.stats[((long long)pslot * 2 + which) * a.stats_ld + nt * BN + col] = v;
        }
    }
}

struct TileCfg {
    int bm, bn, bk;
    int kind;
};

static TileCfg pick_tile(long long M, int n, int cin_tap, int ktot, bool raw_epilogue = true, bool concurrent = false) {
    TileCfg t;
    t.kind = 0;
    if (raw_epilogue && mcamd_small3x3_ok(M, n, cin_tap, ktot)) {
        t.bm = 32, t.bn = round_up_int(n, 32), t.bk = cin_tap, t.kind = 4;
        return t;
    }
    {
        const int pp = MCAMD_ENV_INT("MCAMD_PP", 1);
        if (pp && ktot >= 256 && n >= 128 && M >= 256) {
            bool use = pp == 2;
            int bm = 256, bn = 256;
            if (pp == 1 && ktot >= 1152) {
                double best_cost = -1.0, best_span = 0.0;
                const int bms[2] = {256, 192}, bns[2] = {256, 128};
                for (int cn = 0; cn < 2; ++cn) {
                    if (n < bns[cn]) continue;
                    for (int c = 0; c < 2; ++c) {
                        const long long tiles = ((M + bms[c] - 1) / bms[c]) * ((n + bns[cn] - 1) / bns[cn]);
                        const long long rounds = (tiles + 255) / 256;
                        const double fill = (double)tiles / (double)(rounds * 256);
                        const double rate = bns[cn] == 256 ? 1.0 : 0.8;
                        if (fill < 0.8 && !(concurrent && rounds == 1 && fill >= 0.4)) continue;
                        const double span = (double)rounds * bms[c] * bns[cn] / rate;
                        const double cost = concurrent ? (double)tiles * bms[c] * bns[cn] / rate : span;
                        const bool better = best_cost < 0 || (concurrent ? (cost < 0.97 * best_cost || (cost < 1.03 * best_cost && span < best_span))
                                                                         : cost < best_cost);
                        if (better) best_cost = cost, best_span = span, bm = bms[c], bn = bns[cn];
                    }
                }
                use = best_cost >= 0;
            }
            if (pp >= 2) {
                if (MCAMD_ENV_INT("MCAMD_PP_BM", 256) == 192) bm = 192;
                if (MCAMD_ENV_INT("MCAMD_PP_BN", 256) == 128) bn = 128;
            }
            if (use) {
                t.bm = bm, t.bn = bn, t.bk = 32, t.kind = 2;
                return t;
            }
        }
    }
    int best = 128, waste = round_up_int(n, 128);
    for (int bn = 64; bn >= 32; bn /= 2)
        if (round_up_int(n, bn) < waste) {
            waste = round_up_int(n, bn);
            best = bn;
        }
    t.bm = 128;
    t.bn = best;
    if (t.bn == 128 && (n % 64 == 0 || round_up_int(n, 64) == round_up_int(n, 128))) {
        const long long t128 = ((M + 127) / 128) * ((n + 127) / 128);
        if (t128 < 256 && 2 * t128 <= 512) t.bn = 64;
    }
    int want_bk = MCAMD_ENV_INT("MCAMD_BK", 64);
    t.bk = (want_bk == 64 && cin_tap % 64 == 0) ? 64 : 32;
    if (t.bm == 128 && t.bn == 128 && t.bk == 64 && ktot >= 2048) {
        const long long nt = (n + 127) / 128;
        const long long t128 = ((M + 127) / 128) * nt, t192 = ((M + 191) / 192) * nt;
        const long long cost128 = ((t128 + 511) / 512) * 128, cost192 = ((t192 + 511) / 512) * 192;
        if (cost192 <= cost128) t.bm = 192;
    }
    return t;
}

static int igemm_mtiles(long long M, int bm) { return (int)((M + bm - 1) / bm); }

ConvRoute mcamd_igemm_route(long long M, int n, int cin_tap, int ktot, bool raw_epilogue, bool concurrent) {
    const TileCfg t = pick_tile(M, n, cin_tap, ktot, raw_epilogue, concurrent);
    if (t.kind == ROUTE_SMALL3X3) return {t.kind, t.bm, t.bn, t.bk, mcamd_small3x3_rows(M)};
    int ntiles = (n + t.bn - 1) / t.bn;
    int mtiles = igemm_mtiles(M, t.bm);
    int target = t.kind == ROUTE_PP ? 256 : 2048;
    int p = target / ntiles;
    if (p < 1) p = 1;
    if (p > mtiles) p = mtiles;
    return {t.kind, t.bm, t.bn, t.bk, p};
}

template <int BM, int BN, int WM, int WN, int BK, int NSTAGE, int EPI>
static void launch_inst(const IgemmArgs& a, int rows, int ntiles, hipStream_t st) {
    constexpr int NT = (BM / WM) * (BN / WN) * 64;
    constexpr int STAGE_BYTES = (BM + BN) * (BK / 8) * 16;
    size_t lds = NSTAGE * STAGE_BYTES;
    if (lds < (size_t)BM * BN * 2) lds = (size_t)BM * BN * 2;
    if (lds < (size_t)(BM / WM) * 2 * BN * 4) lds = (size_t)(BM / WM) * 2 * BN * 4;
    if (lds > 64 * 1024) MCAMD_LDS_OPT_IN((igemm_kernel<BM, BN, WM, WN, BK, NSTAGE, EPI>), lds);
    hipLaunchKernelGGL((igemm_kernel<BM, BN, WM, WN, BK, NSTAGE, EPI>), dim3(round_up_int(rows, 8) * ntiles + 8), dim3(NT), lds, st, a);
}

template <int BM, int BN, int WM, int WN, int BK, int NSTAGE>
static void launch_one(const IgemmArgs& a, int rows, int ntiles, hipStream_t st) {
    if (a.mode == MCAMD_EPI_NCHW_F32) launch_inst<BM, BN, WM, WN, BK, NSTAGE, MCAMD_EPI_NCHW_F32>(a, rows, ntiles, st);
    else if (a.mode == MCAMD_EPI_RAW_F32) launch_inst<BM, BN, WM, WN, BK, NSTAGE, MCAMD_EPI_RAW_F32>(a, rows, ntiles, st);
    else if (a.mode == MCAMD_EPI_PAD_F16) launch_inst<BM, BN, WM, WN, BK, NSTAGE, MCAMD_EPI_PAD_F16>(a, rows, ntiles, st);
    else launch_inst<BM, BN, WM, WN, BK, NSTAGE, MCAMD_EPI_RAW_F16>(a, rows, ntiles, st);
}

int mcamd_igemm_launch(IgemmArgs& a, const ConvRoute& r, hipStream_t st) {
    if (a.cin_tap % r.bk != 0 || a.ktot % r.bk != 0) {
        mcamd_set_error("igemm: K per tap (%d) must be a multiple of %d", a.cin_tap, r.bk);
        return MCAMD_EINVAL;
    }
    const int rows = r.rows, ntiles = (a.N + r.bn - 1) / r.bn;
    a.num_mtiles = igemm_mtiles(a.M, r.bm);
    a.num_pslots = rows;
    a.num_ntiles = ntiles;
    a.xcd_order = 1;
    if (r.kernel == ROUTE_PP) return mcamd_igemm_pp_launch(a, r.bm, r.bn, rows, ntiles, st);
    const int stages = r.bk == 32 ? 3 : 2;
#define I_CASE(BN_, WM_, WN_, BK_, ST_)                              \
    if (!done && r.bm == 128 && r.bn == BN_ && r.bk == BK_ && stages == ST_) { \
        launch_one<128, BN_, WM_, WN_, BK_, ST_>(a, rows, ntiles, st); \
        done = true;                                                  \
    }
    bool done = false;
    if (r.bm == 192 && r.bn == 128 && r.bk == 64) { launch_one<192, 128, 96, 64, 64, 2>(a, rows, ntiles, st); done = true; }
    I_CASE(128, 64, 64, 32, 3) I_CASE(128, 64, 64, 64, 2)
    I_CASE(64, 64, 32, 32, 3) I_CASE(64, 64, 32, 64, 2)
    I_CASE(32, 32, 32, 32, 3) I_CASE(32, 32, 32, 64, 2)
#undef I_CASE
    if (!done) {
        mcamd_set_error("igemm: no kernel instance for BM %d BN %d BK %d stages %d", r.bm, r.bn, r.bk, stages);
        return MCAMD_EINVAL;
    }
    MCAMD_LAUNCH_CHECK("igemm");
    return MCAMD_OK;
}
```

### modelcompression_amd/csrc/conv_igemm_pp.hip

```cpp
#include "kernels.h"
#include "conv_epi.h"
#include <stdlib.h>

namespace {

constexpr int BK = 32, NST = 4;
constexpr int WAVES_N = 4;
constexpr int NT = 512;
constexpr int CPR = BK / 8;

template <int MS> struct Shape;
template <> struct Shape<32> {
    typedef f32x16_t acc_t;
    static constexpr int AR = 16, KS = 2;
    __device__ static __forceinline__ int swz4(int row) { return (row >> 2) & 3; }
    __device__ static __forceinline__ int rowof(int r, int lane) { return mfma32_row(r, lane); }
    __device__ static __forceinline__ acc_t mfma(h8_t a, h8_t b, acc_t c) {
        return __builtin_amdgcn_mfma_f32_32x32x16_f16(a, b, c, 0, 0, 0);
    }
};
template <> struct Shape<16> {
    typedef f32x4_t acc_t;
    static constexpr int AR = 4, KS = 1;
    __device__ static __forceinline__ int swz4(int row) {
        const int q = (row >> 2) & 3;
        return (((q & 1) ^ (q >> 1)) << 1) | (q >> 1);
    }
    __device__ static __forceinline__ int rowof(int r, int lane) { return (lane >> 4) * 4 + r; }
    __device__ static __forceinline__ acc_t mfma(h8_t a, h8_t b, acc_t c) {
        return __builtin_amdgcn_mfma_f32_16x16x32_f16(a, b, c, 0, 0, 0);
    }
};

__device__ __forceinline__ i32x8_t read_pair(const char* p0, const char* p1) {
    const i32x4_t lo = *(const i32x4_t*)p0, hi = *(const i32x4_t*)p1;
    return __builtin_shufflevector(lo, hi, 0, 1, 2, 3, 4, 5, 6, 7);
}
__device__ __forceinline__ h8_t half_of(i32x8_t v, int s) {
    const i32x4_t q = s ? __builtin_shufflevector(v, v, 4, 5, 6, 7) : __builtin_shufflevector(v, v, 0, 1, 2, 3);
    return __builtin_bit_cast(h8_t, q);
}

}

template <int EPI, int BM, int BN, int MS, bool F8 = false>
__global__ __launch_bounds__(512, 1) void igemm_pp_kernel(IgemmArgs a) {
    static_assert(!F8 || MS == 32, "the fp8 correction chunks are 32x32x64 blocks");
    typedef Shape<MS> SH;
    typedef typename SH::acc_t acc_v;
    constexpr int AR = SH::AR, KS = SH::KS;
    constexpr int WN = BN / WAVES_N, B_SLOTS = BN * CPR, B_IT = B_SLOTS / NT;
    static_assert(BN == 256 || BN == 128, "wave tiles of 64 or 32 columns");
    constexpr int WM = BM / 2, TM = WM / MS, TN = WN / MS;
    constexpr int A_SLOTS = BM * CPR;
    constexpr int A_IT = (A_SLOTS + NT - 1) / NT;
    constexpr bool RAGGED = A_SLOTS % NT != 0;
    constexpr int DPC = A_IT + B_IT;
    constexpr int STAGE_BYTES = (A_SLOTS + B_SLOTS) * 16;
    static_assert(BM == 256 || BM == 192, "wave tiles of 128 or 96 rows");
    extern __shared__ __attribute__((aligned(16))) char smem[];
    const int tid = threadIdx.x, lane = tid & 63;
    const int wave = __builtin_amdgcn_readfirstlane(tid >> 6);
    const int wm = wave / WAVES_N, wn = wave % WAVES_N;
    const int group = wave >> 2;
    auto wait_chunks = [&](int n) {
        if (RAGGED && group == 1) {
            if (n == 2) wait_vmcnt<2 * (DPC - 1)>();
            else if (n == 1) wait_vmcnt<DPC - 1>();
            else wait_vmcnt<0>();
        } else {
            if (n == 2) wait_vmcnt<2 * DPC>();
            else if (n == 1) wait_vmcnt<DPC>();
            else wait_vmcnt<0>();
        }
    };

    int nt, pslot;
    if (!xcd_tile(a.num_ntiles, a.num_pslots, nt, pslot)) return;
    const int nchunks = a.ktot / BK;
    const int cpt = a.cin_tap / BK;

    long long bbase[B_IT];
#pragma unroll
    for (int it = 0; it < B_IT; ++it) {
        const int slot = it * NT + tid;
        const int row = slot / CPR, phys = slot % CPR;
        bbase[it] = (long long)(nt * BN + row) * a.ktot + (phys ^ SH::swz4(row)) * 8;
    }

    float s1[TN], s2[TN];
#pragma unroll
    for (int j = 0; j < TN; ++j) s1[j] = s2[j] = 0.f;
    bool sat = false;

    for (int mt = pslot; mt < a.num_mtiles; mt += a.num_pslots) {
        long long abase[A_IT];
#pragma unroll
        for (int it = 0; it < A_IT; ++it) {
            const int slot = it * NT + tid;
            const int row = (slot / CPR) % BM, phys = slot % CPR;
            abase[it] = tile_x_base(a, EPI == MCAMD_EPI_PAD_F16 && a.dst_mode != 0, mt * BM + row) + (phys ^ SH::swz4(row)) * 8;
        }

        acc_v acc[TM][TN];
#pragma unroll
        for (int i = 0; i < TM; ++i)
#pragma unroll
            for (int j = 0; j < TN; ++j)
#pragma unroll
                for (int r = 0; r < AR; ++r) acc[i][j][r] = 0.f;

        const char* aptr[A_IT];
        const char* bptr[B_IT];
#pragma unroll
        for (int it = 0; it < A_IT; ++it) aptr[it] = (const char*)(a.x + abase[it]);
#pragma unroll
        for (int it = 0; it < B_IT; ++it) bptr[it] = (const char*)(a.w + bbase[it]);
        int st_cb = 0, st_tap = 0, st_c = 0, st_q = 0;
        auto stage_next = [&]() {
            const int koff = (a.tap_off[st_tap] + (st_cb >= a.wrap ? st_cb - a.wrap : st_cb) + st_c) * 2;
            const int woff = st_q * (BK * 2);
            char* sa = smem + (st_q & (NST - 1)) * STAGE_BYTES;
            char* sb = sa + A_SLOTS * 16;
#pragma unroll
            for (int it = 0; it < A_IT; ++it)
                if (it * NT + wave * 64 < A_SLOTS) glds16(aptr[it] + koff, sa + (it * NT + wave * 64) * 16);
#pragma unroll
            for (int it = 0; it < B_IT; ++it) glds16(bptr[it] + woff, sb + (it * NT + wave * 64) * 16);
            ++st_q;
            st_c += BK;
            if (st_c == a.kb) {
                st_c = 0;
                if (++st_tap == a.ntaps) {
                    st_tap = 0;
                    st_cb += a.kb;
                }
            }
        };
        const int lrow = lane & (MS - 1);
        const int c0 = (lane / MS) ^ SH::swz4(lrow);
        const int a_off0 = ((wm * WM + lrow) * CPR + c0) * 16, a_off1 = ((wm * WM + lrow) * CPR + (c0 ^ 2)) * 16;
        const int b_off0 = A_SLOTS * 16 + ((wn * WN + lrow) * CPR + c0) * 16;
        const int b_off1 = A_SLOTS * 16 + ((wn * WN + lrow) * CPR + (c0 ^ 2)) * 16;

        __syncthreads();
#pragma unroll
        for (int q = 0; q < NST - 1; ++q)
            if (q < nchunks) stage_next();
        wait_chunks(nchunks >= 3 ? 2 : nchunks - 1);
        __builtin_amdgcn_s_barrier();
        if (group == 1) __builtin_amdgcn_s_barrier();

        auto chunk_phases = [&](const int p, const bool IS8) __attribute__((always_inline)) {
            __builtin_amdgcn_sched_barrier(0);
            const bool more = p + NST - 1 < nchunks;
            const int koff = (a.tap_off[st_tap] + (st_cb >= a.wrap ? st_cb - a.wrap : st_cb) + st_c) * 2;
            const int woff = st_q * (BK * 2);
            char* sa = smem + (st_q & (NST - 1)) * STAGE_BYTES;
            char* sb = sa + A_SLOTS * 16;
            auto issue_piece = [&](int piece) {
                if (piece < A_IT) {
                    if (piece * NT + wave * 64 < A_SLOTS) glds16(aptr[piece] + koff, sa + (piece * NT + wave * 64) * 16);
                } else if (piece - A_IT < B_IT) {
                    glds16(bptr[piece - A_IT] + woff, sb + ((piece - A_IT) * NT + wave * 64) * 16);
                }
            };
            wait_chunks(p + 2 < nchunks ? 1 : 0);
            const char* sbase = smem + (p & (NST - 1)) * STAGE_BYTES;
            h8_t af[F8 ? 1 : KS][F8 ? 1 : TM], bf[F8 ? 1 : KS][F8 ? 1 : TN];
            i32x8_t af8[F8 ? TM : 1], bf8[F8 ? TN : 1];
            if constexpr (F8) {
#pragma unroll
                for (int j = 0; j < TN; ++j) bf8[j] = read_pair(sbase + b_off0 + j * (MS * CPR * 16), sbase + b_off1 + j * (MS * CPR * 16));
#pragma unroll
                for (int i = 0; i < TM; ++i) af8[i] = read_pair(sbase + a_off0 + i * (MS * CPR * 16), sbase + a_off1 + i * (MS * CPR * 16));
            } else {
// ... 34 lines not shown
            }
            if (!did8) {
#pragma unroll
                for (int s = 0; s < KS; ++s)
#pragma unroll
                    for (int i = 0; i < TM; ++i)
#pragma unroll
                        for (int j = 0; j < TN; ++j) {
                            if constexpr (F8) acc[i][j] = SH::mfma(half_of(af8[i], s), half_of(bf8[j], s), acc[i][j]);
                            else acc[i][j] = SH::mfma(af[s][i], bf[s][j], acc[i][j]);
                            const int m = (s * TM + i) * TN + j;
                            constexpr int NM = KS * TM * TN;
#pragma unroll
                            for (int q = 0; q < 4; ++q)
                                if (more && q * NM / 4 + (NM >= 8 ? 1 : 0) == m) issue_piece(q);
                        }
            }
            __builtin_amdgcn_s_setprio(0);
            if (more) {
                ++st_q;
                st_c += BK;
                if (st_c == a.kb) {
                    st_c = 0;
                    if (++st_tap == a.ntaps) {
                        st_tap = 0;
                        st_cb += a.kb;
                    }
                }
            }
            __builtin_amdgcn_sched_barrier(0);
            __builtin_amdgcn_s_barrier();
        };
        {
            const int p8 = F8 ? (a.f8_from < nchunks ? a.f8_from : nchunks) : nchunks;
            int p = 0;
            for (; p < p8; ++p) chunk_phases(p, false);
            if constexpr (F8)
                for (; p < nchunks; ++p) chunk_phases(p, true);
        }
        if (group == 0) __builtin_amdgcn_s_barrier();
        if constexpr (F8) asm volatile("s_nop 15\n\ts_nop 15" ::: "memory");

        if constexpr (EPI == MCAMD_EPI_NCHW_F32) {
            float* y = (float*)a.y;
#pragma unroll
            for (int i = 0; i < TM; ++i)
#pragma unroll
                for (int r = 0; r < AR; ++r) {
                    const int m = mt * BM + wm * WM + i * MS + SH::rowof(r, lane);
                    if (m < a.M) {
                        int b, hw;
                        split_image(m, a.HW, b, hw);
#pragma unroll
                        for (int j = 0; j < TN; ++j) {
                            const int n = nt * BN + wn * WN + j * MS + (lane & (MS - 1));
                            if (n < a.N) {
                                float v = acc[i][j][r];
                                if (a.bias) v += a.bias[n];
                                y[((long long)b * a.N + n) * a.HW + hw] = v;
                            }
                        }
                    }
                }
        } else if constexpr (EPI == MCAMD_EPI_RAW_F32) {
            float* y = (float*)a.y;
            const int mlim = a.M - mt * BM;
#pragma unroll
            for (int j = 0; j < TN; ++j) {
                const int n = nt * BN + wn * WN + j * MS + (lane & (MS - 1));
#pragma unroll
                for (int i = 0; i < TM; ++i)
#pragma unroll
                    for (int r = 0; r < AR; ++r) {
                        const int row = wm * WM + i * MS + SH::rowof(r, lane);
                        const float v = acc[i][j][r];
                        if (row < mlim) {
                            if (n < a.N) y[(long long)(mt * BM + row) * a.y_ld + a.y_choff + n] = v;
                            s1[j] += v;
                            s2[j] += v * v;
                        }
                    }
            }
        } else {
            __syncthreads();
            half_t* ct = (half_t*)smem;
            const int mlim = a.M - mt * BM;
#pragma unroll
            for (int j = 0; j < TN; ++j) {
                const int col = wn * WN + j * MS + (lane & (MS - 1));
                float sc = 1.f, sh = 0.f;
                if constexpr (EPI == MCAMD_EPI_PAD_F16) {
                    const int n = nt * BN + col;
                    if (n < a.N) {
                        if (a.scale) sc = a.scale[n];
                        if (a.shift) sh = a.shift[n];
                    }
                }
#pragma unroll
                for (int i = 0; i < TM; ++i)
#pragma unroll
                    for (int r = 0; r < AR; ++r) {
                        const int row = wm * WM + i * MS + SH::rowof(r, lane);
                        float v = acc[i][j][r];
                        if constexpr (EPI == MCAMD_EPI_PAD_F16) {
                            v = v * sc + sh;
                            v = v > 0.f ? v : v * a.slope;
                        }
                        const half_t hv = (half_t)fminf(fmaxf(v, -65504.f), 65504.f);
                        sat |= fabsf(v) > 65504.f;
                        ct[row * BN + col] = hv;
                        if (EPI == MCAMD_EPI_RAW_F16 && a.stats) {
                            const float fv = (row < mlim) ? (float)hv : 0.f;
                            s1[j] += fv;
                            s2[j] += fv * fv;
                        }
                    }
            }
            __syncthreads();
            if constexpr (EPI == MCAMD_EPI_PAD_F16) store_pad_tile<BM, BN, BN, NT>(a, nullptr, ct, false, false, mt, nt, tid);
            else store_raw_tile<BM, BN, NT>(a, ct, mt, nt, tid);
        }
    }

    if (sat && a.overflow) atomicOr(a.overflow, 1);
    if ((EPI == MCAMD_EPI_RAW_F16 || EPI == MCAMD_EPI_RAW_F32) && a.stats) {
#pragma unroll
        for (int j = 0; j < TN; ++j) {
            s1[j] += __shfl_xor(s1[j], 32);
            s2[j] += __shfl_xor(s2[j], 32);
            if (MS == 16) {
                s1[j] += __shfl_xor(s1[j], 16);
                s2[j] += __shfl_xor(s2[j], 16);
            }
        }
        __syncthreads();
        float* red = (float*)smem;
        if (lane < MS) {
#pragma unroll
            for (int j = 0; j < TN; ++j) {
                red[(wm * 2 + 0) * BN + wn * WN + j * MS + lane] = s1[j];
                red[(wm * 2 + 1) * BN + wn * WN + j * MS + lane] = s2[j];
            }
        }
        __syncthreads();
        for (int t = tid; t < 2 * BN; t += NT) {
            const int which = t / BN, col = t - which * BN;
            float v = 0.f;
#pragma unroll
            for (int k = 0; k < BM / WM; ++k) v += red[(k * 2 + which) * BN + col];
            a.stats[((long long)pslot * 2 + which) * a.stats_ld + nt * BN + col] = v;
        }
    }
}

template <int EPI, int BM, int BN, int MS, bool F8 = false>
static void launch_pp(const IgemmArgs& a, int rows, int ntiles, hipStream_t st) {
    constexpr size_t ring = (size_t)NST * (BM + BN) * CPR * 16;
    static_assert((size_t)BM * BN * 2 <= ring, "output tile fits the ring");
    MCAMD_LDS_OPT_IN((igemm_pp_kernel<EPI, BM, BN, MS, F8>), ring);
    hipLaunchKernelGGL((igemm_pp_kernel<EPI, BM, BN, MS, F8>), dim3(round_up_int(rows, 8) * ntiles + 8), dim3(NT), ring, st, a);
}

int mcamd_igemm_pp_launch(const IgemmArgs& a, int bm, int bn, int rows, int ntiles, hipStream_t st) {
    if (a.cin_tap % BK != 0 || a.ktot < BK || a.kb % BK != 0 || (bm != 256 && bm != 192) || (bn != 256 && bn != 128)) {
        mcamd_set_error("igemm_pp: K per tap (%d) must be a multiple of %d, tile (%d x %d) 256|192 x 256|128", a.cin_tap, BK, bm, bn);
        return MCAMD_EINVAL;
    }
    if (a.f8_from != 0x7fffffff) {
        if (a.mode != MCAMD_EPI_RAW_F32 || a.f8_from <= 0 || a.f8_from >= a.ktot / BK || a.wrap != 0x7fffffff) {
            mcamd_set_error("igemm_pp: the fp8 correction form needs epilogue mode 3, no x_wrap and 0 < f8_from (%d) < chunks", a.f8_from);
            return MCAMD_EINVAL;
        }
        if (bm == 256 && bn == 256) launch_pp<MCAMD_EPI_RAW_F32, 256, 256, 32, true>(a, rows, ntiles, st);
        else if (bm == 192 && bn == 256) launch_pp<MCAMD_EPI_RAW_F32, 192, 256, 32, true>(a, rows, ntiles, st);
        else if (bm == 256) launch_pp<MCAMD_EPI_RAW_F32, 256, 128, 32, true>(a, rows, ntiles, st);
        else launch_pp<MCAMD_EPI_RAW_F32, 192, 128, 32, true>(a, rows, ntiles, st);
        MCAMD_LAUNCH_CHECK("igemm_pp(f8)");
        return MCAMD_OK;
    }
    const int ms = MCAMD_ENV_INT("MCAMD_PP_MFMA", 16) == 32 ? 32 : 16;
#define PP_SHAPE(EPI_, BM_, BN_)                                           \
    do {                                                                   \
        if (ms == 32) launch_pp<EPI_, BM_, BN_, 32>(a, rows, ntiles, st);  \
        else launch_pp<EPI_, BM_, BN_, 16>(a, rows, ntiles, st);           \
    } while (0)
#define PP_CASE(EPI_)                                                      \
    do {                                                                   \
        if (bm == 256 && bn == 256) PP_SHAPE(EPI_, 256, 256);              \
        else if (bm == 192 && bn == 256) PP_SHAPE(EPI_, 192, 256);         \
        else if (bm == 256) PP_SHAPE(EPI_, 256, 128);                      \
        else PP_SHAPE(EPI_, 192, 128);                                     \
    } while (0)
    if (a.mode == MCAMD_EPI_NCHW_F32) PP_CASE(MCAMD_EPI_NCHW_F32);
    else if (a.mode == MCAMD_EPI_RAW_F32) PP_CASE(MCAMD_EPI_RAW_F32);
    else if (a.mode == MCAMD_EPI_PAD_F16) PP_CASE(MCAMD_EPI_PAD_F16);
    else PP_CASE(MCAMD_EPI_RAW_F16);
#undef PP_CASE
#undef PP_SHAPE
    MCAMD_LAUNCH_CHECK("igemm_pp");
    return MCAMD_OK;
}
```

### modelcompression_amd/csrc/kernels.h

```cpp
#pragma once
#include "common.h"

struct IgemmArgs {
    const half_t* x;
    const half_t* w;
    void* y;
    const float* bias;
    float* stats;
    const float* scale;
    const float* shift;
    long long x_img_stride;
    int x_row_stride;
    int x_ld;
    int x_off;
    int H, W, HW, M, N;
    int ktot;
    int cin_tap;
    int ntaps;
    int kb;
    int tap_off[9];
    int mode;
    int y_ld, y_choff;
    int stats_ld;
    float slope;
    int num_mtiles;
    int num_pslots;
    int num_ntiles;
    int xcd_order;
    int* overflow;
    int dst_mode;
    void* y2;
    int y2_ld, y2_choff;
    int concurrent;
    int wrap;
    int f8_from;
    int f8_sb;
};


struct StemArgs {
    const half_t* x;
    const half_t* w;
    half_t* y;
    float* stats;
    int y_ld, y_choff, stats_ld;
    int H, W, HW, M;
};

struct WgradArgs {
    const half_t* x;
    const half_t* dy;
    float* slab;
    long long x_img_stride, dy_img_stride;
    int x_row_stride, dy_row_stride, x_ld, dy_ld;
    int x_off;
    int dy_off;
    int dy_zero_off;
    int H, W, HW, M;
    int rows_pad;
    int ktot, cin_tap, ntaps;
    int tap_off[9];
    int n_ctiles;
    int n_otiles, n_tapgroups, nsplit;
    int pix_per_split;
};

struct WgradPlan {
    int tmo, tnc, taps, kp, rows_pad, n_otiles, n_ctiles, n_tapgroups, nsplit, pix_per_split;
    int nine;
    int stemw;
    int ns;
    size_t bytes;
};

struct WgradFinish {
    int kernel;
    int sg;
};

enum { ROUTE_IGEMM = 0, ROUTE_STEM = 1, ROUTE_PP = 2, ROUTE_SMALL3X3 = 4, ROUTE_WIN3X3 = 5, ROUTE_WRES = 6, ROUTE_SMALL3X3_SPLIT = 7 };
struct ConvRoute {
    int kernel;
    int bm, bn, bk;
    int rows;
};

ConvRoute mcamd_igemm_route(long long M, int n, int cin_tap, int ktot, bool raw_epilogue, bool concurrent);
int mcamd_igemm_pp_launch(const IgemmArgs& a, int bm, int bn, int rows, int ntiles, hipStream_t st);
int mcamd_igemm_launch(IgemmArgs& a, const ConvRoute& r, hipStream_t st);
int mcamd_sparse24_launch(IgemmArgs& a, const void* idx, hipStream_t st);
int mcamd_pack_sparse24_launch(const float* w, const float* mask, void* vals, void* idx, int cout, int cin, int ntaps,
                               int cin_tap, int kb, hipStream_t st);
int mcamd_conv_q8_launch(IgemmArgs& a, const void* wexp, int y_f8, int y2_f8, hipStream_t st);
int mcamd_pack_q8_launch(const float* w, const float* mask, void* wq, void* wexp, int cout, int cin, int ntaps, hipStream_t st);
#define MCAMD_Q8_TILE_M 128
int mcamd_cast_q8_launch(const void* src, long long pixels, int src_ld, int src_choff, int C, void* dst, int dst_ld,
                         int dst_choff, int back, hipStream_t st);
int mcamd_fakequant_q8_launch(const float* w, const float* mask, const void* wexp, float* out, int cout, int cin, int ntaps,
                              hipStream_t st);
int mcamd_conv_q8_sparse_launch(IgemmArgs& a, const void* idx, const void* wexp, int y_f8, int y2_f8, hipStream_t st);
int mcamd_pack_q8_sparse24_launch(const float* w, const float* mask, void* wq, void* idx, void* wexp, int cout, int cin,
                                  int ntaps, hipStream_t st);

WgradPlan mcamd_wgrad_plan(long long M, int cout, int cin_tap, int ntaps);
int mcamd_wgrad_launch(WgradArgs& a, const WgradPlan& p, hipStream_t st);
bool mcamd_wgrad_stem_ok(int stem, int cout, int W, long long M);
WgradPlan mcamd_wgrad_stem_plan(long long M);
int mcamd_wgrad_stem_launch(WgradArgs& a, const WgradPlan& p, hipStream_t st);
bool mcamd_wgrad_win_ok(int ksize, int stem, int cout, int cin_tap, int W, long long M);
WgradPlan mcamd_wgrad_win_plan(long long M, int cout);
int mcamd_wgrad_win_launch(WgradArgs& a, const WgradPlan& p, hipStream_t st);
bool mcamd_wgrad_use9(int ksize, int stem, int cout, int cin_tap, int W);
WgradPlan mcamd_wgrad_plan9(long long P, int cout, int cin_tap, int W, int pitch, int B);
int mcamd_wgrad9_launch(const WgradArgs& w, const WgradPlan& p, int pitch, long long P, hipStream_t st);
WgradFinish mcamd_wgrad_finish_pick(int nsplit, int stem, int Cin, int ksize, bool has_cmap);
int mcamd_wgrad_instances(int (*out)[4], int cap);
int mcamd_wgrad_finish_launch(const float* slab, const WgradPlan& p, int ktot, int cin_tap, int stem, int Cout, int Cin,
                              int ksize, const float* mask, float inv_scale, float* dw, const int* rmap, const int* cmap,
                              hipStream_t st);
int mcamd_colsum_launch(const half_t* dy, long long rows, int ld, int choff, int C, float inv_scale, float* out,
                        hipStream_t st, void* scratch, size_t scratch_bytes);

bool mcamd_win3x3_ok(int mode, bool stats, long long M, int n, int cin_tap, int ktot, int H, int W);
int mcamd_win3x3_launch(const IgemmArgs& a, hipStream_t st);
bool mcamd_small3x3_ok(long long M, int n, int cin_tap, int ktot);
int mcamd_small3x3_rows(long long M);
int mcamd_small3x3_launch(const IgemmArgs& a, int rows, hipStream_t st);
bool mcamd_small3x3_split_ok(long long M, int n, int cin_tap, int ktot, int wrap, int mode);
int mcamd_small3x3_split_launch(const IgemmArgs& a, int rows, hipStream_t st);

bool mcamd_wres_ok(int ksize, int stem, int n, int cin_tap, int ktot, int B, int H, int W, int mode);
int mcamd_wres_rows(int n, int B, int H, int W);
int mcamd_wres_launch(IgemmArgs& a, int B, int rows, hipStream_t st);

bool mcamd_stem_direct_ok(int stem, int cout, int mode);
int mcamd_stem_rows(long long M);
int mcamd_stem_launch(const StemArgs& a, int cout, int rows, hipStream_t st);
```

### modelcompression_amd/engine.py

```python
import contextlib
import math
import os
import time

import torch

from . import ops
from . import _lib as L
from ._lib import McamdError


class _T:
    __slots__ = ("buf", "ld", "choff", "C", "H", "W", "ps", "ps0")

    def __init__(self, buf, ld, choff, C, H, W, ps=0):
        self.buf, self.ld, self.choff, self.C, self.H, self.W, self.ps = buf, ld, choff, C, H, W, ps
        self.ps0 = ps


class _Layer:
    pass


def _resolve_routes(blocks):
# ... 11 lines not shown
            raise NotImplementedError("block type %r is outside the YOLOv2 conv hot path" % t)
    return ops_


PLAIN_BLOCK_ERR = 2.9e-4
MIXED_BUDGET = 5.5e-4
MIXED_BUDGET_TRAIN = 7.0e-4
TRAIN_GAIN = 1.1


def _probe_side_stream(device, tries=8):
    lock = None
    try:
        import fcntl
        import tempfile
        lock = open(os.path.join(tempfile.gettempdir(), "mcamd_side_probe.lock"), "w")
        fcntl.flock(lock, fcntl.LOCK_EX)
    except Exception:
        lock = None
    try:
        main = torch.cuda.current_stream(device)
        big = torch.empty(64 << 20, dtype=torch.float32, device=device)
        tiny = torch.zeros(64, dtype=torch.float32, device=device)
        first = None
        for _ in range(tries):
            cand = torch.cuda.Stream(device)
            first = first or cand
            torch.cuda.synchronize(device)
            busy, done = torch.cuda.Event(enable_timing=True), torch.cuda.Event(enable_timing=True)
            for _ in range(80):
                big.fill_(1.0)
            busy.record(main)
            with torch.cuda.stream(cand):
                tiny.add_(1.0)
                done.record(cand)
            torch.cuda.synchronize(device)
            concurrent = done.elapsed_time(busy) > 0.0
            if concurrent:
                return cand, True
        return first, False
    finally:
        if lock is not None:
            try:
                import fcntl
                fcntl.flock(lock, fcntl.LOCK_UN)
                lock.close()
            except Exception:
                pass


class Engine:
    def __init__(self, model, B, H, W, device, grad_scale=256.0, precision="fp16", for_training=False, train_layout=False):
        if precision not in ("fp16", "fp16x3", "mixed", "fp8", "fp8-2:4", "fp8-qat"):
            raise McamdError("precision must be 'fp16', 'fp16x3', 'mixed', 'fp8', 'fp8-2:4' or 'fp8-qat' (got %r)" % (precision,))
        self.model, self.B, self.device = model, B, device
        self.precision = precision
        self.for_training = bool(for_training)
        self.train_layout = bool(train_layout)
        self.precise = precision not in ("fp16", "fp8", "fp8-2:4", "fp8-qat")
        self.q8 = precision in ("fp8", "fp8-2:4", "fp8-qat")
        self.qat = precision == "fp8-qat"
        self.fp8_layers = []
        self.q8_sparse = precision == "fp8-2:4"
        self.fp8_sparse_layers = []
        self.qbufs = {}
        self._q8_keys = None
        self.grad_scale = float(grad_scale)
        self.serial = 0
        self._packed_sig = None
        self.events = None
        self.overlap_wgrad = os.environ.get("MCAMD_OVERLAP_WGRAD", "1") == "1"
        self.wgrad_chunk = 1
        self.use_plan = os.environ.get("MCAMD_PLAN", "1") == "1"
        self._fwd_plans, self._bwd_plan, self._plan_epoch = {}, None, 0
        self._logits = self._gout = self._flat = None
        self._pack_on_side = False
        self.sparse_layers = []
        self._sparse_mode, self._sparse_keys = None, None
        self.fold_dead = os.environ.get("MCAMD_FOLD_DEAD", "1") == "1"
        self.f8 = precision == "mixed" and os.environ.get("MCAMD_F8", "1") == "1"
        self.bn_narrow_on = True
        self.bwd_from_act = True
        self.pool_act_on = True
        self._side_stream = None
        self._side_concurrent = True
        self._side_ws = None
        self.overflow = torch.zeros(1, dtype=torch.int32, device=device)
        self._build_plan(H, W)

    def _build_plan(self, H0, W0):
        model, B, dev = self.model, self.B, self.device
        blocks = model.blocks
        bops = _resolve_routes(blocks)
        n = len(bops)

        def alias(t):
            while t >= 0 and bops[t][0] == "route" and len(bops[t][1]) == 1:
                t = bops[t][1][0]
            return t

        srcs = [[alias(s) for s in o[1]] for o in bops]
        consumers = {}
        for ind, (t, _) in enumerate(bops):
            if t == "route" and len(srcs[ind]) == 1:
                continue
            for s in srcs[ind]:
                consumers.setdefault(s, []).append(ind)

        shape = {-1: (int(blocks[0]["channels"]), H0, W0)}
        for ind, (t, _) in enumerate(bops):
            if t == "convolutional":
                c, h, w = shape[srcs[ind][0]]
                assert int(blocks[ind + 1]["stride"]) == 1, "only stride-1 convolutions (YOLOv2)"
                shape[ind] = (int(blocks[ind + 1]["filters"]), h, w)
            elif t == "maxpool":
                c, h, w = shape[srcs[ind][0]]
                if int(blocks[ind + 1]["size"]) != 2 or int(blocks[ind + 1]["stride"]) != 2:
                    raise NotImplementedError("only maxpool size=2 stride=2 is on the YOLOv2 path")
                shape[ind] = (c, h // 2, w // 2)
            elif t == "reorg":
                c, h, w = shape[srcs[ind][0]]
                assert int(blocks[ind + 1]["stride"]) == 2
                shape[ind] = (4 * c, h // 2, w // 2)
            elif t == "route":
                if len(srcs[ind]) == 1:
                    shape[ind] = shape[srcs[ind][0]]
                else:
                    (c1, h, w), (c2, h2, w2) = shape[srcs[ind][0]], shape[srcs[ind][1]]
                    assert (h, w) == (h2, w2)
                    shape[ind] = (c1 + c2, h, w)

        self._bops, self._srcs, self._shape = bops, srcs, shape
        conv_inds = [i for i, (t, _) in enumerate(bops) if t == "convolutional"]
        fused = {}
        for ci in conv_inds:
            cons = consumers.get(ci, [])
            pools = [c for c in cons if bops[c][0] == "maxpool"]
            reorgs = [c for c in cons if bops[c][0] == "reorg"]
            if len(pools) == 1 and len(cons) == 1:
                fused[ci] = (L.DST_POOL, pools[0], None)
            elif len(pools) == 1 and not reorgs:
                fused[ci] = (L.DST_POOL, pools[0], ci)
            elif len(reorgs) == 1 and len(cons) == 1:
                fused[ci] = (L.DST_REORG, reorgs[0], None)
            elif not pools and not reorgs:
                fused[ci] = (L.DST_PLAIN, ci, None)
            else:
                raise NotImplementedError("unsupported consumer pattern after conv block %d" % ci)
        for ind, (t, _) in enumerate(bops):
            if t in ("maxpool", "reorg") and not any(f[1] == ind for f in fused.values()):
                raise NotImplementedError("stand-alone %s block %d (not directly after a conv)" % (t, ind))

        place = {}
        self.bufs = []

        self.shared_halo_maxw = 0
        if self.train_layout:
            self.shared_halo_maxw = 26

        def pad_for(w):
            return 1 if (w <= self.shared_halo_maxw and w >= 4) else 0

        def new_buf(Bn, h, w, ld):
            self.bufs.append(ops.alloc_padded(Bn, h, w, ld, dev, pad=pad_for(w)))
            return len(self.bufs) - 1
        self._pad_for = pad_for
# ... 862 lines not shown
                ops.bn_act_fwd(B, lay.H, lay.W, lay.bn_width or lay.cout, lay.y, lay.cout, 0, lay.scale, lay.shift,
                               lay.slope, lay.mode, self.bufs[t.buf], t.ld, t.choff,
                               self.bufs[t2.buf] if t2 is not None else None,
                               t2.ld if t2 is not None else 0, t2.choff if t2 is not None else 0, border=lay.border,
                               planes=self._planes_for(lay.out_id), dst_plane=t.ps, dst2_plane=t2.ps if t2 is not None else 0,
                               dst_pad=self._pad_for(t.W), dst2_pad=self._pad_for(t2.W) if t2 is not None else 0,
                               planes2=self._planes_for(lay.out2_id) if t2 is not None else 0,
                               pool_act=af, pool_act_ld=ops.round_up(lay.cout, 8) if af is not None else 0,
                               pool_act_pad=self._pad_for(lay.W) if af is not None else 0)
                continue
            if not training and self._fused_eval(lay):
                ops.bn_coeffs(None, lay.cout, lay.M, bn.weight.data, bn.bias.data, bn.running_mean, bn.running_var, False,
                              lay.scale, lay.shift, lay.mean, lay.invstd, eps=bn.eps)
                t, t2 = lay.out_t, lay.out2_t
                q8 = self.q8 and lay.q8_on
                y2 = None if t2 is None else (self.qbufs if q8 and lay.q8_y2 else self.bufs)[t2.buf]
                dst = dict(dst_mode=lay.mode, y2=y2, y2_ld=t2.ld if t2 is not None else 0,
                           y2_choff=t2.choff if t2 is not None else 0)
                if q8:
                    x8 = self.qbufs.get(lay.tin.buf)
                    if lay.xq is not None:
                        ti, x8 = lay.tin, lay.xq
                        self._timed('cast', lay, ops.cast_q8, xin, B * (ti.H + 2) * (ti.W + 2), ti.ld, ti.choff, lay.cin,
                                    x8, ti.ld, ti.choff)
                    y = self.qbufs[t.buf] if lay.q8_y else self.bufs[t.buf]
                    if lay.q8s_on:
                        self._timed('fwd', lay, ops.conv_fwd_q8_sparse24, lay.geom_act, x8, lay.wqs, lay.widx8, lay.wexp, y,
                                    t.ld, t.choff, lay.scale, lay.shift, lay.slope, y_f8=lay.q8_y, y2_f8=lay.q8_y2, **dst)
                        continue
                    self._timed('fwd', lay, ops.conv_fwd_q8, lay.geom_act, x8, lay.wq, lay.wexp, y, t.ld, t.choff, lay.scale,
                                lay.shift, lay.slope, y_f8=lay.q8_y, y2_f8=lay.q8_y2, **dst)
                    continue
                if lay.sp_on:
                    self._timed('fwd', lay, ops.conv_fwd_sparse24, lay.geom_act, xin, lay.wsp, lay.widx, self.bufs[t.buf], t.ld,
                                t.choff, lay.scale, lay.shift, lay.slope, **dst)
                    continue
                self._timed('fwd', lay, ops.conv_fwd_padded, lay.geom_act, xin, lay.wp, self.bufs[t.buf], t.ld, t.choff,
                            lay.scale, lay.shift, lay.slope, **dst)
                continue
            if training and self._qat_train(lay):
                self._qat_forward(lay, xin)
                continue
            self._timed('fwd', lay, ops.conv_fwd_raw, lay.geom_act, xin, lay.wp, lay.y, lay.cout, 0, lay.stats if training else None)
            ops.bn_coeffs(lay.stats if training else None, lay.cout, lay.M, bn.weight.data, bn.bias.data,
                          bn.running_mean, bn.running_var, training, lay.scale, lay.shift, lay.mean, lay.invstd,
                          momentum=bn.momentum if bn.momentum is not None else 0.1, eps=bn.eps, perm=lay.perm32,
                          ones_channel=lay.ones_idx)
            t, t2 = lay.out_t, lay.out2_t
            ops.bn_act_fwd(B, lay.H, lay.W, lay.bn_width or lay.cout, lay.y, lay.cout, 0, lay.scale, lay.shift,
                           lay.slope, lay.mode, self.bufs[t.buf], t.ld, t.choff,
                           self.bufs[t2.buf] if t2 is not None else None,
                           t2.ld if t2 is not None else 0, t2.choff if t2 is not None else 0, border=lay.border,
                           dst_pad=self._pad_for(t.W), dst2_pad=self._pad_for(t2.W) if t2 is not None else 0)

    def _qat_forward(self, lay, xin):
        B, bn = self.B, lay.bn
        x8 = self.qbufs.get(lay.tin.buf)
        if lay.xq is not None:
            ti, x8 = lay.tin, lay.xq
            self._timed('cast', lay, ops.cast_q8, xin, ops.padded_pixels(B, ti.H, ti.W, self._pad_for(ti.W)), ti.ld, ti.choff,
                        lay.cin, x8, ti.ld, ti.choff, write_back=True)
        self._timed('fwd', lay, ops.conv_fwd_q8_raw, lay.geom_act, x8, lay.wq, lay.wexp, lay.y, lay.cout, 0, lay.stats)
        ops.bn_coeffs(lay.stats, lay.cout, lay.M, bn.weight.data, bn.bias.data, bn.running_mean, bn.running_var, True,
                      lay.scale, lay.shift, lay.mean, lay.invstd, momentum=bn.momentum if bn.momentum is not None else 0.1,
                      eps=bn.eps)
        t, t2 = lay.out_t, lay.out2_t
        ops.bn_act_fwd(B, lay.H, lay.W, lay.cout, lay.y, lay.cout, 0, lay.scale, lay.shift, lay.slope, lay.mode,
                       self.bufs[t.buf], t.ld, t.choff, self.bufs[t2.buf] if t2 is not None else None,
                       t2.ld if t2 is not None else 0, t2.choff if t2 is not None else 0,
                       dst_pad=self._pad_for(t.W), dst2_pad=self._pad_for(t2.W) if t2 is not None else 0,
                       dst_q8=self.qbufs[t.buf] if lay.q8_y else None,
                       dst2_q8=self.qbufs[t2.buf] if (t2 is not None and lay.q8_y2) else None)

    def _stem_split_forward(self, lay):
        bn, t = lay.bn, lay.out_t
        ops.stem_block_stats(self.B, lay.H, lay.W, lay.sh_img, lay.sh_wp, lay.stats, x_lo=lay.sh_img_lo, wp_lo=lay.sh_wp_lo)
        ops.bn_coeffs(lay.stats, lay.cout, lay.M, bn.weight.data, bn.bias.data, bn.running_mean, bn.running_var, True,
                      lay.scale, lay.shift, lay.mean, lay.invstd, momentum=bn.momentum if bn.momentum is not None else 0.1,
                      eps=bn.eps)
        ops.stem_block_fwd(self.B, lay.H, lay.W, lay.sh_img, lay.sh_wp, bn.weight.data, bn.bias.data, None, None, False,
                           lay.scale, lay.shift, lay.mean, lay.invstd, lay.slope, self.bufs[t.buf], t.ld, t.choff, None,
                           eps=bn.eps, cout=lay.cout, planes=self.act_planes, x_lo=lay.sh_img_lo, wp_lo=lay.sh_wp_lo)

    def bn_act_bwd_layer(self, lay, g, g_ld, g_choff, g2, g2_ld, g2_choff, dy, dgamma, dbeta, grad_scale):
        cb = lay.bn_width or lay.cout
        act = {}
        if self.bwd_from_act and self.precise and lay.mode == L.DST_PLAIN and g2 is None:
            t = lay.out_t
            act = dict(act=self.bufs[t.buf], act_ld=t.ld, act_choff=t.choff, act_pad=self._pad_for(t.W))
        elif self.bwd_from_act and self.precise and self.train_layout and lay.mode == L.DST_POOL and lay.slope > 0.0:
            if self.pool_act_on and getattr(lay, "act_full", None) is not None:
                act = dict(act=lay.act_full, act_ld=ops.round_up(lay.cout, 8), act_choff=0, act_pad=self._pad_for(lay.W))
            if g2 is None and lay.y is not None:
                t = lay.out_t
                act.update(pool_out=self.bufs[t.buf], pool_out_ld=t.ld, pool_out_choff=t.choff,
                           pool_out_pad=self._pad_for(t.W))
        ops.bn_act_bwd(self.B, lay.H, lay.W, cb, lay.y, lay.cout, 0, lay.scale, lay.shift, lay.mean,
                       lay.invstd, lay.slope, lay.mode, g, g_ld, g_choff, dy, lay.cout_p, 0,
                       dgamma, dbeta, grad_scale, g2, g2_ld, g2_choff,
                       self.bwd_ws, None if lay.keep is None else lay.keep[:cb], None if lay.perm32 is None else lay.perm32[:cb],
                       overflow=self.overflow, skip_dead_from=lay.n_act if lay.skip_dead else 0, dy_pad=lay.pad, **act)

    def backward(self, grad_out, on_ready=None):
        S = self.grad_scale
        D = S * float(getattr(self.model, "_grad_div", 1.0))
        if self._flat is None:
            self._flat = torch.empty(self.total_params, dtype=torch.float32, device=self.device)
            self._gout = torch.empty(self.out_shape, dtype=torch.float32, device=self.device)
            self._sizes = [p.numel() for p in self.params]
        flat = self._flat
        views = [v if p.dim() == 1 else v.view(p.shape) for v, p in zip(flat.split_with_sizes(self._sizes), self.params)]
        gmap = {id(p): v for p, v in zip(self.params, views)}
        self._gout.copy_(grad_out.detach())
        main = torch.cuda.current_stream(self.device)
        side = None
        if self.overlap_wgrad and self.events is None:
            side = self._get_side_stream()
            if self._side_ws is None or self._side_ws.numel() < self.wgrad_ws.numel():
                self._side_ws = torch.empty(self.wgrad_ws.numel(), dtype=torch.uint8, device=self.device)
                self._side_ws.record_stream(side)
                self._plan_epoch += 1

        def fence():
            ev2 = torch.cuda.Event()
            ev2.record(main)
            side.wait_event(ev2)
            return torch.cuda.stream(side)

        def on_side():
            return torch.cuda.stream(side)

        def ready(lay):
            if on_ready is None:
                return
            if side is None:
                on_ready(flat, lay.p_lo, lay.p_hi)
            elif getattr(on_ready, "takes_fence", False):
                on_ready(flat, lay.p_lo, lay.p_hi, fence if (lay.fused_stem or lay.stem_shadow) else on_side)
            else:
                with fence():
                    on_ready(flat, lay.p_lo, lay.p_hi)

        if self.use_plan and self.events is None:
            key = (main.cuda_stream, side.cuda_stream if side is not None else 0, D, self._plan_epoch, self._ptr_sig())
            plan = self._bwd_plan
            if plan is None or plan.key != key:
                plan = ops.Plan([main] + ([side] if side is not None else []))
                seg_lays = [[]]

                def close_segment(lay):
                    seg_lays[-1].append(lay)
                    plan.mark()
                    seg_lays.append([])
                with plan:
                    self._backward_body(gmap, main, side, S, D, close_segment)
                plan.key, plan.seg_lays = key, seg_lays
                self._bwd_plan = plan
            if on_ready is None:
                plan.run()
            else:
                for si in range(plan.segments):
                    plan.run(si, si + 1)
                    for lay in plan.seg_lays[si]:
                        ready(lay)
        else:
            self._backward_body(gmap, main, side, S, D, ready)
        return flat, views

    def _backward_body(self, gmap, main, side, S, D, ready):
        pending, chunk = [], self.wgrad_chunk

        def flush():
            if not pending:
                return
            ops.stream_wait(side, main)
            with torch.cuda.stream(side):
                for fn, _ in pending:
                    fn(self._side_ws)
            for _, l in pending:
                ready(l)
            pending.clear()

        for lay in reversed(self.layers):
            if lay.stem_shadow:
                flush()
                cons = self.consumer_of[lay.out_id]
                mask = lay.conv.mask.contiguous() if lay.conv.mask_flag else None
                c = lay.sh_coef
                self._timed('wgrad', lay, ops.stem_block_bwd, self.B, lay.H, lay.W, lay.sh_img, lay.sh_wp,
                            lay.bn.weight.data, c[0], c[1], c[2], c[3], lay.slope, cons.gin, cons.tin.ld,
                            lay.out_t.choff, gmap[id(lay.conv.weight)], gmap[id(lay.bn.weight)], gmap[id(lay.bn.bias)],
                            lay.stem_ws, mask=mask, grad_scale=D)
                ready(lay)
                continue
            if lay.fused_stem:
                flush()
                cons = self.consumer_of[lay.out_id]
                mask = lay.conv.mask.contiguous() if lay.conv.mask_flag else None
                self._timed('wgrad', lay, ops.stem_block_bwd, self.B, lay.H, lay.W, self.bufs[lay.tin.buf], lay.wp,
                            lay.bn.weight.data, lay.scale, lay.shift, lay.mean, lay.invstd, lay.slope, cons.gin, cons.tin.ld,
                            lay.out_t.choff, gmap[id(lay.conv.weight)], gmap[id(lay.bn.weight)], gmap[id(lay.bn.bias)],
                            lay.stem_ws, mask=mask, grad_scale=D)
                ready(lay)
                continue
            if lay.is_last:
                ops.nchw_to_padded(self._gout, lay.dy, lay.cout_p, 0, S, overflow=self.overflow, pad=lay.pad)
            else:
                cons = self.consumer_of[lay.out_id]
                t = lay.out_t
                g2 = g2_ld = g2_choff = None
                if lay.out2_id is not None and lay.out2_id in self.consumer_of:
                    c2, t2 = self.consumer_of[lay.out2_id], lay.out2_t
                    g2, g2_ld, g2_choff = c2.gin, c2.tin.ld, t2.choff
                self.bn_act_bwd_layer(lay, cons.gin, cons.tin.ld, t.choff, g2, g2_ld or 0, g2_choff or 0, lay.dy,
                                      gmap[id(lay.bn.weight)], gmap[id(lay.bn.bias)], D)
            mask = lay.conv.mask.contiguous() if lay.conv.mask_flag else None
            dbias = gmap[id(lay.conv.bias)] if lay.conv.bias is not None else None
            def wgrad_of(ws, lay=lay, mask=mask, dbias=dbias):
                if lay.fold is not None:
                    gw, prod = gmap[id(lay.conv.weight)], lay.fold
                    if lay.perm is not None:
                        ops.memset_zero(gw)
                    self._timed('wgrad', lay, ops.conv_wgrad, lay.geom_act, self.bufs[lay.tin.buf], lay.dy, lay.cout_p, 0,
                                lay.dwaug, None, D, dbias, ws)
                    ops.unfold_wgrad(lay.conv.weight.data, mask, lay.g_rows, lay.g_cols, prod.bn.bias.data, prod.slope, lay.n_act,
                                     lay.fold_cin, lay.dwaug, gw, gmap[id(prod.bn.bias)], gmap[id(prod.bn.weight)],
                                     accumulate=prod.fold_consumers[0] is not lay)
                elif lay.gather:
                    gw = gmap[id(lay.conv.weight)]
                    if lay.perm is not None:
                        ops.memset_zero(gw)
                    self._timed('wgrad', lay, ops.conv_wgrad, lay.geom_act, self.bufs[lay.tin.buf], lay.dy, lay.cout_p, 0,
                                gw, mask, D, dbias, ws, rows=lay.g_rows, cols=lay.g_cols)
                else:
                    self._timed('wgrad', lay, ops.conv_wgrad, lay.geom, self.bufs[lay.tin.buf], lay.dy, lay.cout_p, 0,
                                gmap[id(lay.conv.weight)], mask, D, dbias, ws)

            if side is None:
                wgrad_of(self.wgrad_ws)
                ready(lay)
            else:
                pending.append((wgrad_of, lay))
                if len(pending) >= chunk or lay.li <= 1:
                    flush()
            if lay.li > 0:
                self._timed('dgrad', lay, ops.conv_dgrad_raw, lay.geom_act, lay.dy, lay.cout_p, 0, lay.wd, lay.gin, lay.tin.ld,
                            lay.tin.choff, overflow=self.overflow,
                            concurrent=side is not None and self._side_concurrent)
        if side is not None:
            flush()
            ops.stream_wait(main, side)
```

### modelcompression_amd/ops.py

```python
import collections
import ctypes as C
import weakref

import torch

from . import _lib as L
from ._lib import (ConvGeom, ConvEpilogue, ActDesc, ActBwdDesc, ChanMap, PackJob, StemBlockDesc, FoldDesc, FoldJob, check, ptr,
                   stream_ptr)

HALF = torch.float16
SLACK = 64


def round_up(v, m):
    return (v + m - 1) // m * m


def _need_cuda(*ts):
    for t in ts:
        if t is not None and not t.is_cuda:
            raise L.McamdError("modelcompression_amd compute ops need CUDA (MI355X) tensors; there is no CPU path")


def guard_elems(W, ld):
    return (round_up(W + 3, 4) + 128) * ld + SLACK


_PAD_OF = {}


def alloc_padded(B, H, W, ld, device, pad=0):
    n = (B * (H + 1) * (W + 1) + W + 2) * ld if pad else B * (H + 2) * (W + 2) * ld
    g = guard_elems(W, ld)
    full = torch.zeros(g + n + g, dtype=HALF, device=device)
    buf = full[g:g + n + SLACK]
    buf._mcamd_pad = 1 if pad else 0
    if pad:
        _PAD_OF[buf.data_ptr()] = weakref.ref(buf)
    else:
        _PAD_OF.pop(buf.data_ptr(), None)
    return buf


def pad_of(buf):
    form = getattr(buf, "_mcamd_pad", None)
    if form is not None:
        return form
    ref = _PAD_OF.get(buf.data_ptr())
    if ref is None:
        return 0
    if ref() is None:
        del _PAD_OF[buf.data_ptr()]
        return 0
    return 1


def padded_view(buf, B, H, W, ld, pad=None):
    if pad is None:
        pad = pad_of(buf)
    if pad:
        return torch.as_strided(buf, (B, H + 2, W + 2, ld), ((H + 1) * (W + 1) * ld, (W + 1) * ld, ld, 1))
    return buf[: B * (H + 2) * (W + 2) * ld].view(B, H + 2, W + 2, ld)


F8_WEXP_DEFAULT = 5


def geom(B, H, W, ksize, cin, cout, x_ld, x_choff=0, stem=0, pad=0, x_wrap=0, x_f8=0, x_f8_wexp=F8_WEXP_DEFAULT):
    return ConvGeom(B, H, W, ksize, cin, cout, x_ld, x_choff, stem, pad, x_wrap, x_f8, x_f8_wexp if x_f8 else 0)


def conv_fwd_f8_ok(g):
    return bool(L.lib().mcamd_conv_fwd_f8_ok(C.byref(g)))


def packed_elems(g):
    lib = L.lib()
    return int(lib.mcamd_packed_elems_fwd(C.byref(g))), int(lib.mcamd_packed_elems_dgrad(C.byref(g)))


def _chan_map(g, rows, cols):
    if rows is None and cols is None:
        return None
    m = ChanMap()
    for name, v, n in (("rows", rows, g.cout), ("cols", cols, g.cin)):
        if v is not None:
            if v.dtype != torch.int32 or not v.is_cuda or not v.is_contiguous() or v.numel() != n:
                raise L.McamdError("channel map `%s` must be a contiguous CUDA int32 vector of %d entries" % (name, n))
            setattr(m, name, v.data_ptr())
    return C.byref(m)
# ... 7 lines not shown
        out_fwd = torch.empty(nf, dtype=HALF, device=w.device)
    if want_dgrad and not g.stem and out_dgrad is None:
        out_dgrad = torch.empty(nd, dtype=HALF, device=w.device)
    check(L.lib().mcamd_pack_weights(C.byref(g), ptr(w), ptr(mask), _chan_map(g, rows, cols), ptr(out_fwd) if want_fwd else None,
                                     ptr(out_dgrad) if (want_dgrad and not g.stem) else None, stream_ptr()),
          "mcamd_pack_weights")
    return out_fwd, out_dgrad


def pack_table(jobs, device):
    arr = (PackJob * len(jobs))()
    total = 0
    for a, j in zip(arr, jobs):
        _need_cuda(j["w"], j.get("dst_fwd"), j.get("dst_dgrad"))
        assert j["w"].dtype == torch.float32 and j["w"].is_contiguous()
        a.w = j["w"].data_ptr()
        for name in ("mask", "dst_fwd", "dst_dgrad", "rows", "cols"):
            setattr(a, name, j[name].data_ptr() if j.get(name) is not None else None)
        a.first_tile, a.cout, a.cin, a.ksize = total, j["cout"], j["cin"], j["ksize"]
        a.split = int(j.get("split") or 0)
        a.f8_wexp = int(j.get("f8_wexp", F8_WEXP_DEFAULT))
        total += ((j["cout"] + 31) // 32) * ((j["cin"] + 31) // 32)
    host = torch.frombuffer(bytearray(bytes(arr)), dtype=torch.uint8)
    return host.to(device), len(jobs), total


def pack_many(table, njobs, total):
    check(L.lib().mcamd_pack_weights_many(ptr(table), njobs, total, stream_ptr()), "mcamd_pack_weights_many")


def tile_info(g, dgrad=False, concurrent=False):
    out = (C.c_int32 * 4)()
    check(L.lib().mcamd_conv_tile_info(C.byref(g), (2 if concurrent else 1) if dgrad else 0, out), "mcamd_conv_tile_info")
    return tuple(out)


def stats_rows(g, mode=L.EPI_RAW_F16):
    return int(L.lib().mcamd_conv_stats_rows_mode(C.byref(g), mode))


def _epi(mode, y, y_ld=0, y_choff=0, bias=None, stats=None, stats_rows_=0, stats_ld=0, scale=None, shift=None,
         slope=1.0, overflow=None, dst_mode=0, y2=None, y2_ld=0, y2_choff=0):
    e = ConvEpilogue()
    e.mode, e.y_ld, e.y_choff = mode, y_ld, y_choff
    e.y = y.data_ptr()
    e.bias = bias.data_ptr() if bias is not None else None
    e.stats = stats.data_ptr() if stats is not None else None
    e.stats_rows, e.stats_ld = stats_rows_, stats_ld
    e.scale = scale.data_ptr() if scale is not None else None
    e.shift = shift.data_ptr() if shift is not None else None
    e.slope = slope
    e.overflow = overflow.data_ptr() if overflow is not None else None
    e.dst_mode = dst_mode
    e.y2 = y2.data_ptr() if y2 is not None else None
    e.y2_ld, e.y2_choff = y2_ld, y2_choff
    return e


def conv_fwd_raw(g, x, wp, y, y_ld, y_choff=0, stats=None):
    e = _epi(L.EPI_RAW_F16, y, y_ld, y_choff, stats=stats,
             stats_rows_=stats.shape[0] if stats is not None else 0,
             stats_ld=stats.shape[2] if stats is not None else 0)
    check(L.lib().mcamd_conv_fwd(C.byref(g), ptr(x), ptr(wp), C.byref(e), stream_ptr()), "mcamd_conv_fwd")


def conv_fwd_raw32(g, x, wp, y, y_ld, y_choff=0, stats=None):
    e = _epi(L.EPI_RAW_F32, y, y_ld, y_choff, stats=stats,
             stats_rows_=stats.shape[0] if stats is not None else 0,
             stats_ld=stats.shape[2] if stats is not None else 0)
    check(L.lib().mcamd_conv_fwd(C.byref(g), ptr(x), ptr(wp), C.byref(e), stream_ptr()), "mcamd_conv_fwd")


def conv_fwd_nchw(g, x, wp, y, bias=None):
    e = _epi(L.EPI_NCHW_F32, y, bias=bias)
    check(L.lib().mcamd_conv_fwd(C.byref(g), ptr(x), ptr(wp), C.byref(e), stream_ptr()), "mcamd_conv_fwd")


def conv_fwd_padded(g, x, wp, y, y_ld, y_choff=0, scale=None, shift=None, slope=1.0, dst_mode=0, y2=None, y2_ld=0, y2_choff=0):
    e = _epi(L.EPI_PAD_F16, y, y_ld, y_choff, scale=scale, shift=shift, slope=slope, dst_mode=dst_mode, y2=y2, y2_ld=y2_ld,
             y2_choff=y2_choff)
    check(L.lib().mcamd_conv_fwd(C.byref(g), ptr(x), ptr(wp), C.byref(e), stream_ptr()), "mcamd_conv_fwd")


def conv_dgrad_raw(g, dy, dy_ld, dy_choff, wpd, out, out_ld, out_choff=0, overflow=None, concurrent=False):
    e = _epi(L.EPI_RAW_F16, out, out_ld, out_choff, overflow=overflow)
    e.concurrent = 1 if concurrent else 0
    check(L.lib().mcamd_conv_dgrad(C.byref(g), ptr(dy), dy_ld, dy_choff, ptr(wpd), C.byref(e), stream_ptr()),
          "mcamd_conv_dgrad")


def conv_dgrad_nchw(g, dy, dy_ld, dy_choff, wpd, out):
    e = _epi(L.EPI_NCHW_F32, out)
    check(L.lib().mcamd_conv_dgrad(C.byref(g), ptr(dy), dy_ld, dy_choff, ptr(wpd), C.byref(e), stream_ptr()),
          "mcamd_conv_dgrad")


def wgrad_workspace_bytes(g):
    return int(L.lib().mcamd_conv_wgrad_workspace_bytes(C.byref(g)))


WgradPlanInfo = collections.namedtuple("WgradPlanInfo", "family tmo tnc taps kp ns nsplit pix_per_split rows_pad finish sg tiles grid")


def wgrad_plan_info(g, has_cmap=False):
    out = (C.c_int32 * L.WGRAD_PLAN_INFO_N)()
    check(L.lib().mcamd_conv_wgrad_plan_info(C.byref(g), 1 if has_cmap else 0, out), "mcamd_conv_wgrad_plan_info")
    return WgradPlanInfo(*out)


def wgrad_generic_instances():
    lib = L.lib()
    n = int(lib.mcamd_wgrad_generic_instances(None, 0))
    out = (C.c_int32 * (4 * n))()
    lib.mcamd_wgrad_generic_instances(out, n)
    return [tuple(out[4 * i:4 * i + 4]) for i in range(n)]


def conv_wgrad(g, x, dy, dy_ld, dy_choff, dw, mask=None, grad_scale=1.0, dbias=None, workspace=None, rows=None, cols=None):
    if workspace is None:
        workspace = torch.empty(wgrad_workspace_bytes(g), dtype=torch.uint8, device=dw.device)
    check(L.lib().mcamd_conv_wgrad(C.byref(g), ptr(x), ptr(dy), dy_ld, dy_choff, ptr(mask), _chan_map(g, rows, cols), grad_scale, ptr(dw),
                                   ptr(dbias), ptr(workspace), workspace.numel(), stream_ptr()), "mcamd_conv_wgrad")


def _perm_ptr(perm, C_):
    if perm is None:
        return None
    if perm.dtype != torch.int32 or perm.numel() != C_ or not perm.is_contiguous() or not perm.is_cuda:
        raise L.McamdError("channel permutation must be a contiguous CUDA int32 vector of %d entries" % C_)
    return perm.data_ptr()


def bn_coeffs(stats, C_, count, gamma, beta, rmean, rvar, training, scale, shift, mean=None, invstd=None,
              momentum=0.1, eps=1e-5, perm=None, ones_channel=-1):
    rows = stats.shape[0] if stats is not None else 0
    ld = stats.shape[2] if stats is not None else 0
    check(L.lib().mcamd_bn_coeffs_ex(ptr(stats), rows, ld, C_, count, ptr(gamma), ptr(beta), ptr(rmean), ptr(rvar),
                                     momentum, eps, 1 if training else 0, ptr(scale), ptr(shift), ptr(mean), ptr(invstd),
                                     _perm_ptr(perm, C_), ones_channel, stream_ptr()), "mcamd_bn_coeffs_ex")


def _fold_desc(w, mask, rows, cols, beta, slope, n, cin_k, aug):
    _need_cuda(w, mask, rows, cols, beta)
    assert w.dtype == torch.float32 and w.is_contiguous() and w.dim() == 4 and w.shape[2] == w.shape[3]
    assert beta.dtype == torch.float32 and beta.numel() == w.shape[1]
    d = FoldDesc()
    d.w = w.data_ptr()
    d.mask = mask.data_ptr() if mask is not None else None
    for name, v, cnt in (("rows", rows, n), ("cols", cols, w.shape[1])):
        if v is not None:
            if v.dtype != torch.int32 or not v.is_contiguous() or v.numel() != cnt:
                raise L.McamdError("fold: channel map `%s` must be a contiguous CUDA int32 vector of %d entries" % (name, cnt))
            setattr(d, name, v.data_ptr())
    d.beta, d.slope = beta.data_ptr(), slope
    assert aug.dtype == torch.float32 and aug.is_contiguous() and aug.dim() == 4 and aug.shape[0] == n and aug.shape[1] > cin_k
    d.n, d.cin_t, d.cin_k, d.cin_aug, d.ksize = n, w.shape[1], cin_k, aug.shape[1], w.shape[2]
    return d


def fold_weights(w, mask, rows, cols, beta, slope, n, cin_k, waug):
    d = _fold_desc(w, mask, rows, cols, beta, slope, n, cin_k, waug)
    check(L.lib().mcamd_fold_weights(C.byref(d), ptr(waug), stream_ptr()), "mcamd_fold_weights")


def fold_table(jobs, device):
    arr = (FoldJob * len(jobs))()
    total = 0
    for a, j in zip(arr, jobs):
        a.d = _fold_desc(j["w"], j["mask"], j["rows"], j["cols"], j["beta"], j["slope"], j["n"], j["cin_k"], j["waug"])
        a.waug = j["waug"].data_ptr()
        a.first_block = total
        total += j["n"]
    host = torch.frombuffer(bytearray(bytes(arr)), dtype=torch.uint8)
    return host.to(device), len(jobs), total


def fold_many(table, njobs, total):
    check(L.lib().mcamd_fold_weights_many(ptr(table), njobs, total, stream_ptr()), "mcamd_fold_weights_many")


def unfold_wgrad(w, mask, rows, cols, beta, slope, n, cin_k, dwaug, dw, prod_dbeta, prod_dgamma, accumulate=False):
    d = _fold_desc(w, mask, rows, cols, beta, slope, n, cin_k, dwaug)
    check(L.lib().mcamd_unfold_wgrad(C.byref(d), ptr(dwaug), ptr(dw), ptr(prod_dbeta), ptr(prod_dgamma), 1 if accumulate else 0,
                                     stream_ptr()), "mcamd_unfold_wgrad")


def bn_act_fwd(B, H, W, C_, y, y_ld, y_choff, scale, shift, slope, mode, dst, dst_ld, dst_choff=0, dst2=None,
               dst2_ld=0, dst2_choff=0, border=None, planes=1, dst_plane=0, dst2_plane=0, dst_pad=0, dst2_pad=0, planes2=0,
               pool_act=None, pool_act_ld=0, pool_act_pad=0, dst_q8=None, dst2_q8=None):
    d = ActDesc()
    d.y_dtype = 1 if y.dtype == torch.float32 else 0
    d.planes, d.dst_plane, d.dst2_plane, d.planes2 = planes, dst_plane, dst2_plane, planes2
    d.dst_pad, d.dst2_pad = dst_pad, dst2_pad
    d.B, d.H, d.W, d.C = B, H, W, C_
    d.y, d.y_ld, d.y_choff = y.data_ptr(), y_ld, y_choff
    d.scale, d.shift, d.slope, d.mode = scale.data_ptr(), shift.data_ptr(), slope, mode
    d.dst, d.dst_ld, d.dst_choff = dst.data_ptr(), dst_ld, dst_choff
    d.dst2 = dst2.data_ptr() if dst2 is not None else None
    d.dst2_ld, d.dst2_choff = dst2_ld, dst2_choff
    if border is not None:
        if border.dtype != torch.float32 or tuple(border.shape) != (16, C_) or not border.is_contiguous():
            raise L.McamdError("bn_act_fwd: border table must be contiguous fp32 [16, %d]" % C_)
        d.border = border.data_ptr()
    if pool_act is not None:
        d.pool_act, d.pool_act_ld, d.pool_act_pad = pool_act.data_ptr(), pool_act_ld, pool_act_pad
    d.dst_q8 = dst_q8.data_ptr() if dst_q8 is not None else None
    d.dst2_q8 = dst2_q8.data_ptr() if dst2_q8 is not None else None
    check(L.lib().mcamd_bn_act_fwd(C.byref(d), stream_ptr()), "mcamd_bn_act_fwd")


def bn_act_bwd(B, H, W, C_, y, y_ld, y_choff, scale, shift, mean, invstd, slope, mode, g, g_ld, g_choff, dy, dy_ld,
               dy_choff, dgamma, dbeta, grad_scale=1.0, g2=None, g2_ld=0, g2_choff=0, workspace=None, dy_keep=None,
               perm=None, overflow=None, skip_dead_from=0, dy_pad=0, act=None, act_ld=0, act_choff=0, act_pad=0,
               pool_out=None, pool_out_ld=0, pool_out_choff=0, pool_out_pad=0):
    d = ActBwdDesc()
    d.skip_dead_param_grads = int(skip_dead_from)
    d.dy_pad = dy_pad
    d.B, d.H, d.W, d.C = B, H, W, C_
    if act is not None:
        d.act, d.act_ld, d.act_choff, d.act_pad = act.data_ptr(), act_ld, act_choff, act_pad
    if pool_out is not None:
        d.pool_out, d.pool_out_ld, d.pool_out_choff, d.pool_out_pad = pool_out.data_ptr(), pool_out_ld, pool_out_choff, pool_out_pad
    d.y, d.y_ld, d.y_choff = (y.data_ptr() if y is not None else None), y_ld, y_choff
    d.scale, d.shift, d.mean, d.invstd = scale.data_ptr(), shift.data_ptr(), mean.data_ptr(), invstd.data_ptr()
    d.slope, d.mode = slope, mode
    d.g, d.g_ld, d.g_choff = g.data_ptr(), g_ld, g_choff
    d.g2 = g2.data_ptr() if g2 is not None else None
    d.g2_ld, d.g2_choff = g2_ld, g2_choff
    d.dy, d.dy_ld, d.dy_choff = dy.data_ptr(), dy_ld, dy_choff
    d.dgamma = dgamma.data_ptr() if dgamma is not None else None
    d.dbeta = dbeta.data_ptr() if dbeta is not None else None
    d.grad_scale = grad_scale
    d.dy_keep = dy_keep.data_ptr() if dy_keep is not None else None
    d.chan_perm = _perm_ptr(perm, C_)
    d.y_dtype = 1 if (y is not None and y.dtype == torch.float32) else 0
    d.overflow = overflow.data_ptr() if overflow is not None else None
    need = int(L.lib().mcamd_bn_act_bwd_workspace_bytes(C.byref(d)))
    if workspace is None:
        workspace = torch.empty(need, dtype=torch.uint8, device=g.device)
    check(L.lib().mcamd_bn_act_bwd(C.byref(d), ptr(workspace), workspace.numel(), stream_ptr()), "mcamd_bn_act_bwd")


def bn_act_bwd_workspace_bytes(C_):
    d = ActBwdDesc()
    d.C = C_
    return int(L.lib().mcamd_bn_act_bwd_workspace_bytes(C.byref(d)))


def stem_block_workspace_bytes():
    return int(L.lib().mcamd_stem_block_workspace_bytes())


def _stem_desc(B, H, W, x, wp, gamma, beta, scale, shift, mean, invstd, slope):
    _need_cuda(x, wp, scale, shift)
    d = StemBlockDesc()
    d.B, d.H, d.W = B, H, W
    d.x, d.wp = x.data_ptr(), wp.data_ptr()
    d.gamma = gamma.data_ptr() if gamma is not None else None
    d.beta = beta.data_ptr() if beta is not None else None
    d.scale, d.shift = scale.data_ptr(), shift.data_ptr()
    d.save_mean = mean.data_ptr() if mean is not None else None
    d.save_invstd = invstd.data_ptr() if invstd is not None else None
    d.slope = slope
    return d


def stem_block_fwd(B, H, W, x, wp, gamma, beta, rmean, rvar, training, scale, shift, mean, invstd, slope, dst, dst_ld,
                   dst_choff, workspace, momentum=0.1, eps=1e-5, cout=32, planes=1, x_lo=None, wp_lo=None):
    d = _stem_desc(B, H, W, x, wp, gamma, beta, scale, shift, mean, invstd, slope)
    d.running_mean = rmean.data_ptr() if rmean is not None else None
    d.running_var = rvar.data_ptr() if rvar is not None else None
    d.momentum, d.eps, d.training = momentum, eps, 1 if training else 0
    d.cout, d.planes = cout, planes
    d.dst, d.dst_ld, d.dst_choff = (dst.data_ptr() if dst is not None else None), dst_ld, dst_choff
    d.x_lo = x_lo.data_ptr() if x_lo is not None else None
    d.wp_lo = wp_lo.data_ptr() if wp_lo is not None else None
    check(L.lib().mcamd_stem_block_fwd(C.byref(d), ptr(workspace), workspace.numel() if workspace is not None else 0,
                                       stream_ptr()), "mcamd_stem_block_fwd")


def stem_block_stats_rows(B, H, W):
    d = StemBlockDesc()
    d.B, d.H, d.W = B, H, W
    return int(L.lib().mcamd_stem_block_stats_rows(C.byref(d)))


def stem_block_stats(B, H, W, x, wp, stats, x_lo=None, wp_lo=None):
    _need_cuda(x, wp, stats)
    assert stats.dtype == torch.float32 and stats.dim() == 3 and stats.shape[1] == 2 and stats.is_contiguous()
    d = StemBlockDesc()
    d.B, d.H, d.W = B, H, W
    d.x, d.wp = x.data_ptr(), wp.data_ptr()
    d.x_lo = x_lo.data_ptr() if x_lo is not None else None
    d.wp_lo = wp_lo.data_ptr() if wp_lo is not None else None
    d.cout = 32
    check(L.lib().mcamd_stem_block_stats(C.byref(d), ptr(stats), stats.shape[0], stats.shape[2], stream_ptr()),
          "mcamd_stem_block_stats")

# ... 372 lines not shown
```

Baseline: 5314.

## Fuse BN backward channel sums into the dgrad epilogue of the consumer conv

Result: faster. 5390, median of 6 (+1.4%).

```diff
diff --git a/include/mcamd.h b/include/mcamd.h
--- a/include/mcamd.h
+++ b/include/mcamd.h
@@ -117,6 +117,22 @@
 
 int mcamd_conv_dgrad(const mcamd_conv_geom* g, const void* dy, int32_t dy_ld, int32_t dy_choff,
                      const void* wp_dgrad, const mcamd_conv_epilogue* epi, void* stream);
+
+typedef struct mcamd_dgrad_sums {
+    float* slab;
+    int32_t rows;
+    int32_t ld;
+    const void* act;
+    int32_t act_ld, act_choff, act_pad;
+    const float* scale; const float* shift; const float* mean; const float* invstd;
+    float slope;
+    const float* y;
+    int32_t y_ld, y_choff;
+    int32_t ch_lo, C;
+} mcamd_dgrad_sums;
+int32_t mcamd_conv_dgrad_sums_rows(const mcamd_conv_geom* g, int32_t concurrent);
+int mcamd_conv_dgrad_sums(const mcamd_conv_geom* g, const void* dy, int32_t dy_ld, int32_t dy_choff,
+                          const void* wp_dgrad, const mcamd_conv_epilogue* epi, const mcamd_dgrad_sums* sums, void* stream);
 
 size_t mcamd_conv_wgrad_workspace_bytes(const mcamd_conv_geom* g);
 int mcamd_conv_wgrad(const mcamd_conv_geom* g, const void* x, const void* dy, int32_t dy_ld,
@@ -193,6 +209,8 @@
     int32_t act_ld, act_choff, act_pad;
     const void* pool_out;
     int32_t pool_out_ld, pool_out_choff, pool_out_pad;
+    const float* sums;
+    int32_t sums_rows, sums_ld;
 } mcamd_act_bwd_desc;
 size_t mcamd_bn_act_bwd_workspace_bytes(const mcamd_act_bwd_desc* d);
 int mcamd_bn_act_bwd(const mcamd_act_bwd_desc* d, void* workspace, size_t workspace_bytes, void* stream);
diff --git a/modelcompression_amd/_lib.py b/modelcompression_amd/_lib.py
--- a/modelcompression_amd/_lib.py
+++ b/modelcompression_amd/_lib.py
@@ -60,7 +60,16 @@
                 ("overflow", C.c_void_p), ("dy_pad", C.c_int32), ("skip_dead_param_grads", C.c_int32),
                 ("act", C.c_void_p), ("act_ld", C.c_int32), ("act_choff", C.c_int32), ("act_pad", C.c_int32),
                 ("pool_out", C.c_void_p), ("pool_out_ld", C.c_int32), ("pool_out_choff", C.c_int32),
-                ("pool_out_pad", C.c_int32)]
+                ("pool_out_pad", C.c_int32),
+                ("sums", C.c_void_p), ("sums_rows", C.c_int32), ("sums_ld", C.c_int32)]
+
+
+class DgradSums(C.Structure):
+    _fields_ = [("slab", C.c_void_p), ("rows", C.c_int32), ("ld", C.c_int32),
+                ("act", C.c_void_p), ("act_ld", C.c_int32), ("act_choff", C.c_int32), ("act_pad", C.c_int32),
+                ("scale", C.c_void_p), ("shift", C.c_void_p), ("mean", C.c_void_p), ("invstd", C.c_void_p),
+                ("slope", C.c_float), ("y", C.c_void_p), ("y_ld", C.c_int32), ("y_choff", C.c_int32),
+                ("ch_lo", C.c_int32), ("C", C.c_int32)]
 
 
 class FoldDesc(C.Structure):
@@ -150,6 +159,8 @@
     "mcamd_fakequant_q8": (C.c_int, [C.POINTER(ConvGeom), _P, _P, _P, _P, _P]),
     "mcamd_cast_q8_train": (C.c_int, [_P, _I64, _I32, _I32, _I32, _P, _I32, _I32, _P]),
     "mcamd_conv_dgrad": (C.c_int, [C.POINTER(ConvGeom), _P, _I32, _I32, _P, C.POINTER(ConvEpilogue), _P]),
+    "mcamd_conv_dgrad_sums_rows": (_I32, [C.POINTER(ConvGeom), _I32]),
+    "mcamd_conv_dgrad_sums": (C.c_int, [C.POINTER(ConvGeom), _P, _I32, _I32, _P, C.POINTER(ConvEpilogue), C.POINTER(DgradSums), _P]),
     "mcamd_conv_wgrad_workspace_bytes": (_SZ, [C.POINTER(ConvGeom)]),
     "mcamd_conv_wgrad": (C.c_int, [C.POINTER(ConvGeom), _P, _P, _I32, _I32, _P, C.POINTER(ChanMap), _F, _P, _P, _P, _SZ, _P]),
     "mcamd_conv_wgrad_plan_info": (C.c_int, [C.POINTER(ConvGeom), _I32, C.POINTER(_I32)]),
diff --git a/modelcompression_amd/csrc/api.hip b/modelcompression_amd/csrc/api.hip
--- a/modelcompression_amd/csrc/api.hip
+++ b/modelcompression_amd/csrc/api.hip
@@ -713,13 +713,26 @@
     return cast_q8_any(src, pixels, src_ld, src_choff, C, dst, dst_ld, dst_choff, 1, stream);
 }
 
-extern "C" int mcamd_conv_dgrad(const mcamd_conv_geom* g, const void* dy, int32_t dy_ld, int32_t dy_choff,
-                                const void* wp_dgrad, const mcamd_conv_epilogue* epi, void* stream) {
+static ConvRoute dgrad_route(const mcamd_conv_geom* g, bool concurrent, int mode) {
+    return conv_route(g, concurrent ? DIR_DGRAD_CONCURRENT : DIR_DGRAD, mode, MCAMD_DST_PLAIN, false);
+}
+
+extern "C" int32_t mcamd_conv_dgrad_sums_rows(const mcamd_conv_geom* g, int32_t concurrent) {
+    if (!g || g->stem) return 0;
+    const ConvRoute r = dgrad_route(g, concurrent != 0, MCAMD_EPI_RAW_F16);
+    return mcamd_igemm_sums_ok(r) ? r.rows : 0;
+}
+
+extern "C" int mcamd_conv_dgrad_sums(const mcamd_conv_geom* g, const void* dy, int32_t dy_ld, int32_t dy_choff,
+                                     const void* wp_dgrad, const mcamd_conv_epilogue* epi, const mcamd_dgrad_sums* sums,
+                                     void* stream) {
     if (mcamd_recording()) {
         MCAMD_REQUIRE(g && epi, "conv_dgrad: null geometry / epilogue");
         const mcamd_conv_geom g_ = *g;
         const mcamd_conv_epilogue e_ = *epi;
-        return mcamd_rec_push(stream, [=](void* s) { return mcamd_conv_dgrad(&g_, dy, dy_ld, dy_choff, wp_dgrad, &e_, s); });
+        if (!sums) return mcamd_rec_push(stream, [=](void* s) { return mcamd_conv_dgrad_sums(&g_, dy, dy_ld, dy_choff, wp_dgrad, &e_, nullptr, s); });
+        const mcamd_dgrad_sums s_ = *sums;
+        return mcamd_rec_push(stream, [=](void* s) { return mcamd_conv_dgrad_sums(&g_, dy, dy_ld, dy_choff, wp_dgrad, &e_, &s_, s); });
     }
     if (check_geom(g, "conv_dgrad")) return MCAMD_EINVAL;
     MCAMD_REQUIRE(g->x_wrap == 0 && g->x_f8 == 0, "conv_dgrad: x_wrap / x_f8 are forward-only fields");
@@ -733,9 +746,38 @@
     MCAMD_REQUIRE(epi && epi->mode != MCAMD_EPI_PAD_F16 && !epi->stats && epi->dst_mode == 0 && !epi->y2,
                   "conv_dgrad: epilogue must be mode 0 (no stats) or 1");
     a.concurrent = epi->concurrent != 0;
-    const ConvRoute r = conv_route(g, a.concurrent ? DIR_DGRAD_CONCURRENT : DIR_DGRAD, epi->mode, MCAMD_DST_PLAIN, false);
+    const ConvRoute r = dgrad_route(g, a.concurrent, epi->mode);
     if (fill_epilogue(a, epi, g->cin, "conv_dgrad", r.rows)) return MCAMD_EINVAL;
+    if (sums && sums->slab) {
+        const mcamd_dgrad_sums* s = sums;
+        MCAMD_REQUIRE(epi->mode == MCAMD_EPI_RAW_F16, "conv_dgrad: producer sums go with epilogue mode 0");
+        MCAMD_REQUIRE(mcamd_igemm_sums_ok(r) && s->rows == r.rows,
+                      "conv_dgrad: sums.rows must be mcamd_conv_dgrad_sums_rows() = %d (got %d; 0: this launch cannot take sums)",
+                      mcamd_igemm_sums_ok(r) ? r.rows : 0, s->rows);
+        MCAMD_REQUIRE(s->act && s->scale && s->shift && s->mean && s->invstd, "conv_dgrad: sums: null argument");
+        MCAMD_REQUIRE(s->C > 0 && s->C % 8 == 0 && s->ch_lo >= 0 && s->ch_lo % 8 == 0 && s->ch_lo + s->C <= g->cin,
+                      "conv_dgrad: sums: producer columns [%d, %d) must be whole groups of 8 inside the %d channels of G",
+                      s->ch_lo, s->ch_lo + s->C, g->cin);
+        MCAMD_REQUIRE(s->ld >= s->C, "conv_dgrad: sums.ld (%d) must be >= C (%d)", s->ld, s->C);
+        MCAMD_REQUIRE(s->act_ld % 8 == 0 && s->act_choff % 8 == 0 && s->act_choff >= 0 && s->act_choff + s->C <= s->act_ld &&
+                          (s->act_pad == 0 || s->act_pad == 1),
+                      "conv_dgrad: sums: activation slice [%d, %d) does not fit act_ld %d", s->act_choff, s->act_choff + s->C, s->act_ld);
+        MCAMD_REQUIRE(!s->y || (s->y_ld % 4 == 0 && s->y_choff % 4 == 0 && s->y_choff >= 0 && s->y_choff + s->C <= s->y_ld),
+                      "conv_dgrad: sums: fp32 y slice [%d, %d) does not fit y_ld %d", s->y_choff, s->y_choff + s->C, s->y_ld);
+        MCAMD_REQUIRE(s->slope > 0.f, "conv_dgrad: sums need an invertible activation (slope > 0)");
+        a.bsum.slab = s->slab, a.bsum.ld = s->ld;
+        a.bsum.act = (const half_t*)s->act, a.bsum.act_ld = s->act_ld, a.bsum.act_choff = s->act_choff, a.bsum.act_pw = s->act_pad ? 1 : 2;
+        a.bsum.scale = s->scale, a.bsum.shift = s->shift, a.bsum.mean = s->mean, a.bsum.invstd = s->invstd;
+        a.bsum.y = s->y, a.bsum.y_ld = s->y_ld, a.bsum.y_choff = s->y_choff;
+        a.bsum.ch_lo = s->ch_lo, a.bsum.C = s->C;
+        a.bsum.slope = s->slope;
+    }
     return launch_route(a, r, g, (hipStream_t)stream);
+}
+
+extern "C" int mcamd_conv_dgrad(const mcamd_conv_geom* g, const void* dy, int32_t dy_ld, int32_t dy_choff,
+                                const void* wp_dgrad, const mcamd_conv_epilogue* epi, void* stream) {
+    return mcamd_conv_dgrad_sums(g, dy, dy_ld, dy_choff, wp_dgrad, epi, nullptr, stream);
 }
 
 static WgradPlan wgrad_plan_for(const mcamd_conv_geom* g) {
diff --git a/modelcompression_amd/csrc/bn_act.hip b/modelcompression_amd/csrc/bn_act.hip
--- a/modelcompression_amd/csrc/bn_act.hip
+++ b/modelcompression_amd/csrc/bn_act.hip
@@ -527,22 +527,6 @@
     }
 }
 
-constexpr float BN_ACT_T = 0.03125f;
-
-__device__ __forceinline__ bool act_xhat_source(const float (&sc)[8], const float (&sh)[8], const float (&mu)[8],
-                                                const float (&is)[8], bool have_y, float (&off)[8], float (&mul)[8],
-                                                bool (&usey)[8]) {
-    bool any = false;
-#pragma unroll
-    for (int i = 0; i < 8; ++i) {
-        const float beta = sh[i] + mu[i] * sc[i];
-        usey[i] = have_y && fabsf(sc[i]) < BN_ACT_T * fmaxf(fabsf(beta), 1.f) * is[i];
-        off[i] = usey[i] ? mu[i] : beta;
-        mul[i] = usey[i] ? is[i] : (sc[i] != 0.f ? is[i] / sc[i] : 0.f);
-        any |= usey[i];
-    }
-    return any;
-}
 
 template <int PHASE>
 __global__ __launch_bounds__(256) void bn_plain_bwd_act_kernel(ActBwdArgs a) {
@@ -1036,7 +1020,7 @@
     block_partials_to_slab(sb, sg, CH, a.slab, a.C);
 }
 
-__global__ __launch_bounds__(1024) void bn_bwd_finalize_kernel(const float* slab, int nblocks, int C, double count,
+__global__ __launch_bounds__(1024) void bn_bwd_finalize_kernel(const float* slab, int nblocks, int ld, int C, double count,
                                                                float inv_scale, float* dgamma, float* dbeta,
                                                                float* coef, const int* perm, int skip_from) {
     __shared__ double red[2][16][RED_CPB];
@@ -1045,8 +1029,8 @@
     double sb = 0.0, sg = 0.0;
     if (c < C) {
         for (int p = ry; p < nblocks; p += RED_RG) {
-            sb += (double)slab[((long long)p * 2 + 0) * C + c];
-            sg += (double)slab[((long long)p * 2 + 1) * C + c];
+            sb += (double)slab[((long long)p * 2 + 0) * ld + c];
+            sg += (double)slab[((long long)p * 2 + 1) * ld + c];
         }
     }
     block_reduce2(sb, sg, red);
@@ -1349,7 +1333,16 @@
         else if (y32) hipLaunchKernelGGL((bn_plain_bwd_kernel<PHASE, true>), dim3(grid), dim3(256), 0, st, a);    \
         else hipLaunchKernelGGL((bn_plain_bwd_kernel<PHASE, false>), dim3(grid), dim3(256), 0, st, a);            \
     } while (0)
-    if (pool_fast && a.pool_out && a.act) hipLaunchKernelGGL(bn_pool_sums_kernel<true>, dim3(grid), dim3(256), 0, st, a);
+    const float* fin_slab = (const float*)a.slab;
+    int fin_rows = grid, fin_ld = d->C;
+    if (d->sums) {
+        MCAMD_REQUIRE(plain_fast && a.act, "bn_act_bwd: `sums` is for PLAIN blocks without a second gradient, with `act`");
+        MCAMD_REQUIRE(d->sums_rows > 0 && d->sums_ld >= d->C, "bn_act_bwd: sums_rows (%d) must be positive and sums_ld (%d) >= C",
+                      d->sums_rows, d->sums_ld);
+        fin_slab = d->sums, fin_rows = d->sums_rows, fin_ld = d->sums_ld;
+    }
+    if (d->sums) {
+    } else if (pool_fast && a.pool_out && a.act) hipLaunchKernelGGL(bn_pool_sums_kernel<true>, dim3(grid), dim3(256), 0, st, a);
     else if (pool_fast && a.pool_out) hipLaunchKernelGGL(bn_pool_sums_kernel<false>, dim3(grid), dim3(256), 0, st, a);
     else if (pool_fast) POOL_LAUNCH(0);
     else if (plain_fast) PLAIN_LAUNCH(0);
@@ -1357,7 +1350,7 @@
         BWD_LAUNCH(0)
     }
     MCAMD_LAUNCH_CHECK("bn_act_bwd reduce");
-    hipLaunchKernelGGL(bn_bwd_finalize_kernel, dim3((d->C + RED_CPB - 1) / RED_CPB), dim3(1024), 0, st, (const float*)a.slab, grid, d->C,
+    hipLaunchKernelGGL(bn_bwd_finalize_kernel, dim3((d->C + RED_CPB - 1) / RED_CPB), dim3(1024), 0, st, fin_slab, fin_rows, fin_ld, d->C,
                        count, 1.0f / d->grad_scale, d->dgamma, d->dbeta, coef, (const int*)d->chan_perm,
                        d->skip_dead_param_grads);
     MCAMD_LAUNCH_CHECK("bn_act_bwd finalize");
diff --git a/modelcompression_amd/csrc/common.h b/modelcompression_amd/csrc/common.h
--- a/modelcompression_amd/csrc/common.h
+++ b/modelcompression_amd/csrc/common.h
@@ -80,6 +80,23 @@
     return (((long long)b * (H + pw) + h + 1) * (W + pw) + w + 1) * ld;
 }
 
+constexpr float BN_ACT_T = 0.03125f;
+
+__device__ __forceinline__ bool act_xhat_source(const float (&sc)[8], const float (&sh)[8], const float (&mu)[8],
+                                                const float (&is)[8], bool have_y, float (&off)[8], float (&mul)[8],
+                                                bool (&usey)[8]) {
+    bool any = false;
+#pragma unroll
+    for (int i = 0; i < 8; ++i) {
+        const float beta = sh[i] + mu[i] * sc[i];
+        usey[i] = have_y && fabsf(sc[i]) < BN_ACT_T * fmaxf(fabsf(beta), 1.f) * is[i];
+        off[i] = usey[i] ? mu[i] : beta;
+        mul[i] = usey[i] ? is[i] : (sc[i] != 0.f ? is[i] / sc[i] : 0.f);
+        any |= usey[i];
+    }
+    return any;
+}
+
 template <int CPR>
 __device__ __forceinline__ int swz(int row) {
     return CPR == 4 ? ((row >> 2) & 3) : ((row >> 1) & 7);
diff --git a/modelcompression_amd/csrc/conv_epi.h b/modelcompression_amd/csrc/conv_epi.h
--- a/modelcompression_amd/csrc/conv_epi.h
+++ b/modelcompression_amd/csrc/conv_epi.h
@@ -155,6 +155,144 @@
     }
 }
 
+template <class T>
+__device__ __forceinline__ const T* pin_here(const T* p) {
+    asm volatile("" : "+s"(p));
+    return p;
+}
+__host__ __device__ constexpr int sums_vals(int cols, int nt) { return (2 * cols + nt - 1) / nt; }
+__host__ __device__ constexpr size_t sums_lds_bytes(int nt) { return (size_t)16 * (nt + 8) * sizeof(float); }
+
+__host__ __device__ constexpr int sums_slots(int rows, int cols, int nt) { return rows * (cols / 8) / nt; }
+__host__ __device__ constexpr int sums_early(int rows, int cols, int nt) {
+    return rows * cols >= 256 * 256 && sums_slots(rows, cols, nt) > 8 ? 8 : sums_slots(rows, cols, nt);
+}
+
+template <int ROWS, int COLS, int NT>
+__device__ __forceinline__ void sums_prefetch(const IgemmArgs& __restrict__ a, int mt, int nt, int tid,
+                                              h8_t (&aq)[sums_early(ROWS, COLS, NT)]) {
+    constexpr int CH = COLS / 8, RSTEP = NT / CH, NSLOT = sums_early(ROWS, COLS, NT);
+    static_assert(NT % CH == 0 && (ROWS * CH) % NT == 0, "a thread keeps its 8 channels for all its slots");
+    const int ch = tid % CH, row0 = tid / CH;
+    const int n0 = nt * COLS + ch * 8;
+    const int c = n0 - a.bsum.ch_lo;
+    const bool live = n0 < a.N && c >= 0 && c < a.bsum.C;
+    const half_t* act = pin_here(a.bsum.act) + a.bsum.act_choff + c;
+    int m = mt * ROWS + row0;
+    int b, h, w;
+    split_pixel(m, a.HW, a.W, b, h, w);
+    const int sb_ = RSTEP / a.HW, srem = RSTEP - sb_ * a.HW;
+    const int sh_ = srem / a.W, sw_ = srem - sh_ * a.W;
+#pragma unroll
+    for (int k = 0; k < NSLOT; ++k) {
+#pragma unroll
+        for (int i = 0; i < 8; ++i) aq[k][i] = (half_t)0.f;
+        if (live && m < a.M) aq[k] = *(const h8_t*)(act + pad_off(b, h, w, a.H, a.W, a.bsum.act_ld, a.bsum.act_pw));
+        m += RSTEP;
+        w += sw_;
+        if (w >= a.W) w -= a.W, ++h;
+        h += sh_;
+        if (h >= a.H) h -= a.H, ++b;
+        b += sb_;
+    }
+}
+
+template <int ROWS, int COLS, int NT>
+__device__ __forceinline__ void store_raw_tile_sums(const IgemmArgs& __restrict__ a, char* smem, int mt, int nt, int tid,
+                                                    const h8_t (&aq)[sums_early(ROWS, COLS, NT)],
+                                                    float (&tot)[sums_vals(COLS, NT)]) {
+    constexpr int CH = COLS / 8, RSTEP = NT / CH, NSLOT = sums_slots(ROWS, COLS, NT), PITCH = NT + 8;
+    constexpr int EARLY = sums_early(ROWS, COLS, NT);
+    const half_t* ct = (const half_t*)smem;
+    half_t* y = (half_t*)a.y;
+    const int ch = tid % CH, row0 = tid / CH;
+    const int n0 = nt * COLS + ch * 8;
+    const int c = n0 - a.bsum.ch_lo;
+    const bool col_ok = n0 < a.N;
+    const bool live = col_ok && c >= 0 && c < a.bsum.C;
+    float sb[8], sg[8], off[8], mul[8];
+    bool usey[8];
+    bool need_y = false;
+#pragma unroll
+    for (int i = 0; i < 8; ++i) sb[i] = sg[i] = 0.f, off[i] = 0.f, mul[i] = 0.f, usey[i] = false;
+    if (live) {
+        const float *scp = pin_here(a.bsum.scale) + c, *shp = pin_here(a.bsum.shift) + c;
+        const float *mup = pin_here(a.bsum.mean) + c, *isp = pin_here(a.bsum.invstd) + c;
+        float sc[8], sh[8], mu[8], is[8];
+#pragma unroll
+        for (int i = 0; i < 8; ++i) sc[i] = scp[i], sh[i] = shp[i], mu[i] = mup[i], is[i] = isp[i];
+        need_y = act_xhat_source(sc, sh, mu, is, a.bsum.y != nullptr, off, mul, usey);
+    }
+    const float slope = a.bsum.slope, inv_slope = 1.0f / slope;
+#pragma unroll
+    for (int k = 0; k < NSLOT; ++k) {
+        const int row = row0 + k * RSTEP, m = mt * ROWS + row;
+        if (!col_ok || m >= a.M) continue;
+        const h8_t gq = *(const h8_t*)(ct + row * COLS + ch * 8);
+        *(h8_t*)(y + (long long)m * a.y_ld + a.y_choff + n0) = gq;
+        if (!live) continue;
+        h8_t av8;
+        if (k < EARLY) {
+            av8 = aq[k];
+        } else {
+            int b, h, w;
+            split_pixel(m, a.HW, a.W, b, h, w);
+            av8 = *(const h8_t*)(a.bsum.act + pad_off(b, h, w, a.H, a.W, a.bsum.act_ld, a.bsum.act_pw) + a.bsum.act_choff + c);
+        }
+        float z[8];
+#pragma unroll
+        for (int i = 0; i < 8; ++i) {
+            const float av = (float)av8[i];
+            z[i] = av > 0.f ? av : av * inv_slope;
+        }
+        if (need_y) {
+            const float* yp = a.bsum.y + (long long)m * a.bsum.y_ld + a.bsum.y_choff + c;
+#pragma unroll
+            for (int i = 0; i < 8; ++i) z[i] = usey[i] ? yp[i] : z[i];
+        }
+#pragma unroll
+        for (int i = 0; i < 8; ++i) {
+            const float gv = (float)gq[i];
+            const float gz = (float)av8[i] > 0.f ? gv : gv * slope;
+            sb[i] += gz;
+            sg[i] += gz * ((z[i] - off[i]) * mul[i]);
+        }
+    }
+    __syncthreads();
+    float* red = (float*)smem;
+#pragma unroll
+    for (int i = 0; i < 8; ++i) {
+        red[i * PITCH + tid] = sb[i];
+        red[(8 + i) * PITCH + tid] = sg[i];
+    }
+    __syncthreads();
+#pragma unroll
+    for (int k = 0; k < sums_vals(COLS, NT); ++k) {
+        const int t = tid + k * NT;
+        if (t < 2 * COLS) {
+            const int which = t / COLS, col = t - which * COLS;
+            const int v = which * 8 + (col & 7), chq = col >> 3;
+            float s = 0.f;
+            for (int r = 0; r < RSTEP; ++r) s += red[v * PITCH + r * CH + chq];
+            tot[k] += s;
+        }
+    }
+}
+
+template <int COLS, int NT>
+__device__ __forceinline__ void store_tile_sums_slab(const IgemmArgs& __restrict__ a, int pslot, int nt, int tid,
+                                                     const float (&tot)[sums_vals(COLS, NT)]) {
+#pragma unroll
+    for (int k = 0; k < sums_vals(COLS, NT); ++k) {
+        const int t = tid + k * NT;
+        if (t < 2 * COLS) {
+            const int which = t / COLS, col = t - which * COLS;
+            const int n = nt * COLS + col, c = n - a.bsum.ch_lo;
+            if (n < a.N && c >= 0 && c < a.bsum.C) a.bsum.slab[((long long)pslot * 2 + which) * a.bsum.ld + c] = tot[k];
+        }
+    }
+}
+
 template <int BMW, int PITCH, int WM, int WN, int TM, int TN, class ScaleOf>
 __device__ __forceinline__ bool write_ch_tile(const IgemmArgs& __restrict__ a, const f32x16_t (&acc)[TM][TN], ScaleOf scale_of, bool need_b,
                                               bool need_h, char* bt, half_t* ht, int nt, int wm, int wn, int lane) {
diff --git a/modelcompression_amd/csrc/conv_igemm.hip b/modelcompression_amd/csrc/conv_igemm.hip
--- a/modelcompression_amd/csrc/conv_igemm.hip
+++ b/modelcompression_amd/csrc/conv_igemm.hip
@@ -51,6 +51,10 @@
 #pragma unroll
     for (int j = 0; j < TN; ++j) s1[j] = s2[j] = 0.f;
     bool sat = false;
+    constexpr bool SUMS = EPI == MCAMD_EPI_RAW_F16_SUMS;
+    float tot[SUMS ? sums_vals(BN, NT) : 1];
+#pragma unroll
+    for (int k = 0; k < (SUMS ? sums_vals(BN, NT) : 1); ++k) tot[k] = 0.f;
 
     for (int mt = pslot; mt < a.num_mtiles; mt += a.num_pslots) {
         long long abase[A_IT];
@@ -188,6 +192,8 @@
                     }
             }
         } else {
+            h8_t aq[SUMS ? sums_early(BM, BN, NT) : 1];
+            if constexpr (SUMS) sums_prefetch<BM, BN, NT>(a, mt, nt, tid, aq);
             __syncthreads();
             half_t* ct = (half_t*)smem;
             const int mlim = a.M - mt * BM;
@@ -224,11 +230,13 @@
             }
             __syncthreads();
             if constexpr (EPI == MCAMD_EPI_PAD_F16) store_pad_tile<BM, BN, BN, NT>(a, nullptr, ct, false, false, mt, nt, tid);
+            else if constexpr (SUMS) store_raw_tile_sums<BM, BN, NT>(a, smem, mt, nt, tid, aq, tot);
             else store_raw_tile<BM, BN, NT>(a, ct, mt, nt, tid);
         }
     }
 
     if (sat && a.overflow) atomicOr(a.overflow, 1);
+    if constexpr (SUMS) store_tile_sums_slab<BN, NT>(a, pslot, nt, tid, tot);
     if ((EPI == MCAMD_EPI_RAW_F16 || EPI == MCAMD_EPI_RAW_F32) && a.stats) {
 #pragma unroll
         for (int j = 0; j < TN; ++j) {
@@ -346,6 +354,7 @@
     size_t lds = NSTAGE * STAGE_BYTES;
     if (lds < (size_t)BM * BN * 2) lds = (size_t)BM * BN * 2;
     if (lds < (size_t)(BM / WM) * 2 * BN * 4) lds = (size_t)(BM / WM) * 2 * BN * 4;
+    if (EPI == MCAMD_EPI_RAW_F16_SUMS && lds < sums_lds_bytes(NT)) lds = sums_lds_bytes(NT);
     if (lds > 64 * 1024) MCAMD_LDS_OPT_IN((igemm_kernel<BM, BN, WM, WN, BK, NSTAGE, EPI>), lds);
     hipLaunchKernelGGL((igemm_kernel<BM, BN, WM, WN, BK, NSTAGE, EPI>), dim3(round_up_int(rows, 8) * ntiles + 8), dim3(NT), lds, st, a);
 }
@@ -355,7 +364,14 @@
     if (a.mode == MCAMD_EPI_NCHW_F32) launch_inst<BM, BN, WM, WN, BK, NSTAGE, MCAMD_EPI_NCHW_F32>(a, rows, ntiles, st);
     else if (a.mode == MCAMD_EPI_RAW_F32) launch_inst<BM, BN, WM, WN, BK, NSTAGE, MCAMD_EPI_RAW_F32>(a, rows, ntiles, st);
     else if (a.mode == MCAMD_EPI_PAD_F16) launch_inst<BM, BN, WM, WN, BK, NSTAGE, MCAMD_EPI_PAD_F16>(a, rows, ntiles, st);
+    else if (a.bsum.slab) {
+        if constexpr (BN >= 64) launch_inst<BM, BN, WM, WN, BK, NSTAGE, MCAMD_EPI_RAW_F16_SUMS>(a, rows, ntiles, st);
+    }
     else launch_inst<BM, BN, WM, WN, BK, NSTAGE, MCAMD_EPI_RAW_F16>(a, rows, ntiles, st);
+}
+
+bool mcamd_igemm_sums_ok(const ConvRoute& r) {
+    return r.kernel == ROUTE_PP || (r.kernel == ROUTE_IGEMM && r.bn >= 64);
 }
 
 int mcamd_igemm_launch(IgemmArgs& a, const ConvRoute& r, hipStream_t st) {
diff --git a/modelcompression_amd/csrc/conv_igemm_pp.hip b/modelcompression_amd/csrc/conv_igemm_pp.hip
--- a/modelcompression_amd/csrc/conv_igemm_pp.hip
+++ b/modelcompression_amd/csrc/conv_igemm_pp.hip
@@ -92,6 +92,10 @@
 #pragma unroll
     for (int j = 0; j < TN; ++j) s1[j] = s2[j] = 0.f;
     bool sat = false;
+    constexpr bool SUMS = EPI == MCAMD_EPI_RAW_F16_SUMS;
+    float tot[SUMS ? sums_vals(BN, NT) : 1];
+#pragma unroll
+    for (int k = 0; k < (SUMS ? sums_vals(BN, NT) : 1); ++k) tot[k] = 0.f;
 
     for (int mt = pslot; mt < a.num_mtiles; mt += a.num_pslots) {
         long long abase[A_IT];
@@ -292,6 +296,8 @@
                     }
             }
         } else {
+            h8_t aq[SUMS ? sums_early(BM, BN, NT) : 1];
+            if constexpr (SUMS) sums_prefetch<BM, BN, NT>(a, mt, nt, tid, aq);
             __syncthreads();
             half_t* ct = (half_t*)smem;
             const int mlim = a.M - mt * BM;
@@ -328,11 +334,13 @@
             }
             __syncthreads();
             if constexpr (EPI == MCAMD_EPI_PAD_F16) store_pad_tile<BM, BN, BN, NT>(a, nullptr, ct, false, false, mt, nt, tid);
+            else if constexpr (SUMS) store_raw_tile_sums<BM, BN, NT>(a, smem, mt, nt, tid, aq, tot);
             else store_raw_tile<BM, BN, NT>(a, ct, mt, nt, tid);
         }
     }
 
     if (sat && a.overflow) atomicOr(a.overflow, 1);
+    if constexpr (SUMS) store_tile_sums_slab<BN, NT>(a, pslot, nt, tid, tot);
     if ((EPI == MCAMD_EPI_RAW_F16 || EPI == MCAMD_EPI_RAW_F32) && a.stats) {
 #pragma unroll
         for (int j = 0; j < TN; ++j) {
@@ -366,7 +374,7 @@
 template <int EPI, int BM, int BN, int MS, bool F8 = false>
 static void launch_pp(const IgemmArgs& a, int rows, int ntiles, hipStream_t st) {
     constexpr size_t ring = (size_t)NST * (BM + BN) * CPR * 16;
-    static_assert((size_t)BM * BN * 2 <= ring, "output tile fits the ring");
+    static_assert((size_t)BM * BN * 2 <= ring && sums_lds_bytes(NT) <= ring, "output tile (and the partials of the sums form) fit the ring");
     MCAMD_LDS_OPT_IN((igemm_pp_kernel<EPI, BM, BN, MS, F8>), ring);
     hipLaunchKernelGGL((igemm_pp_kernel<EPI, BM, BN, MS, F8>), dim3(round_up_int(rows, 8) * ntiles + 8), dim3(NT), ring, st, a);
 }
@@ -404,6 +412,7 @@
     if (a.mode == MCAMD_EPI_NCHW_F32) PP_CASE(MCAMD_EPI_NCHW_F32);
     else if (a.mode == MCAMD_EPI_RAW_F32) PP_CASE(MCAMD_EPI_RAW_F32);
     else if (a.mode == MCAMD_EPI_PAD_F16) PP_CASE(MCAMD_EPI_PAD_F16);
+    else if (a.bsum.slab) PP_CASE(MCAMD_EPI_RAW_F16_SUMS);
     else PP_CASE(MCAMD_EPI_RAW_F16);
 #undef PP_CASE
 #undef PP_SHAPE
diff --git a/modelcompression_amd/csrc/kernels.h b/modelcompression_amd/csrc/kernels.h
--- a/modelcompression_amd/csrc/kernels.h
+++ b/modelcompression_amd/csrc/kernels.h
@@ -1,5 +1,21 @@
 #pragma once
 #include "common.h"
+
+struct DgradSums {
+    float* slab;
+    const half_t* act;
+    const float* scale;
+    const float* shift;
+    const float* mean;
+    const float* invstd;
+    const float* y;
+    int act_ld, act_choff, act_pw;
+    int y_ld, y_choff;
+    int ch_lo, C;
+    int ld;
+    float slope;
+};
+#define MCAMD_EPI_RAW_F16_SUMS 4
 
 struct IgemmArgs {
     const half_t* x;
@@ -35,6 +51,7 @@
     int wrap;
     int f8_from;
     int f8_sb;
+    DgradSums bsum;
 };
 
 
@@ -88,6 +105,7 @@
 ConvRoute mcamd_igemm_route(long long M, int n, int cin_tap, int ktot, bool raw_epilogue, bool concurrent);
 int mcamd_igemm_pp_launch(const IgemmArgs& a, int bm, int bn, int rows, int ntiles, hipStream_t st);
 int mcamd_igemm_launch(IgemmArgs& a, const ConvRoute& r, hipStream_t st);
+bool mcamd_igemm_sums_ok(const ConvRoute& r);
 int mcamd_sparse24_launch(IgemmArgs& a, const void* idx, hipStream_t st);
 int mcamd_pack_sparse24_launch(const float* w, const float* mask, void* vals, void* idx, int cout, int cin, int ntaps,
                                int cin_tap, int kb, hipStream_t st);
diff --git a/modelcompression_amd/engine.py b/modelcompression_amd/engine.py
--- a/modelcompression_amd/engine.py
+++ b/modelcompression_amd/engine.py
@@ -117,6 +117,8 @@
         self.bn_narrow_on = True
         self.bwd_from_act = True
         self.pool_act_on = True
+        self.dgrad_bn_sums = os.environ.get("MCAMD_DGRAD_BN_SUMS", "1") == "1"
+        self._dgrad_sums_cache = {}
         self._side_stream = None
         self._side_concurrent = True
         self._side_ws = None
@@ -1145,7 +1147,43 @@
                            lay.scale, lay.shift, lay.mean, lay.invstd, lay.slope, self.bufs[t.buf], t.ld, t.choff, None,
                            eps=bn.eps, cout=lay.cout, planes=self.act_planes, x_lo=lay.sh_img_lo, wp_lo=lay.sh_wp_lo)
 
-    def bn_act_bwd_layer(self, lay, g, g_ld, g_choff, g2, g2_ld, g2_choff, dy, dgamma, dbeta, grad_scale):
+    def _dgrad_sums(self, lay, concurrent):
+        if not (self.dgrad_bn_sums and self.bwd_from_act and self.precise) or lay.gin is None:
+            return None
+        key = (lay.li, bool(concurrent), self._plan_epoch)
+        hit = self._dgrad_sums_cache.get(key, False)
+        if hit is not False:
+            return hit
+        res = None
+        if lay.fold is None and not lay.gather and lay.in_perm is None and lay.geom_act is lay.geom:
+            for prod in self.layers:
+                if prod.is_last or prod.fused_stem or prod.stem_shadow or prod.bn is None or prod.out_t is None:
+                    continue
+                if self.consumer_of.get(prod.out_id) is not lay or prod.mode != L.DST_PLAIN or prod.slope <= 0.0:
+                    continue
+                if prod.out2_id is not None and prod.out2_id in self.consumer_of:
+                    continue
+                if (prod.keep is not None or prod.perm is not None or prod.fold is not None or prod.skip_dead or prod.fold_consumers
+                        or prod.bn_width or prod.border is not None or prod.cout % 8 != 0):
+                    continue
+                t = prod.out_t
+                ch_lo = t.choff - lay.tin.choff
+                if t.buf != lay.tin.buf or t.ld != lay.tin.ld or ch_lo < 0 or ch_lo % 8 != 0 or ch_lo + prod.cout > lay.geom.cin:
+                    continue
+                rows = ops.dgrad_sums_rows(lay.geom_act, concurrent)
+                if rows <= 0:
+                    continue
+                slab = torch.empty(rows, 2, prod.cout, dtype=torch.float32, device=self.device)
+                y = prod.y if (prod.y is not None and prod.y.dtype == torch.float32) else None
+                desc = ops.dgrad_sums(slab, self.bufs[t.buf], t.ld, t.choff, self._pad_for(t.W), prod.scale, prod.shift, prod.mean,
+                                      prod.invstd, prod.slope, prod.cout, ch_lo=ch_lo, y=y, y_ld=prod.cout, y_choff=0)
+                res = (desc, slab, prod)
+                break
+        self._dgrad_sums_cache = {k: v for k, v in self._dgrad_sums_cache.items() if k[2] == self._plan_epoch}
+        self._dgrad_sums_cache[key] = res
+        return res
+
+    def bn_act_bwd_layer(self, lay, g, g_ld, g_choff, g2, g2_ld, g2_choff, dy, dgamma, dbeta, grad_scale, sums=None):
         cb = lay.bn_width or lay.cout
         act = {}
         if self.bwd_from_act and self.precise and lay.mode == L.DST_PLAIN and g2 is None:
@@ -1158,6 +1196,8 @@
                 t = lay.out_t
                 act.update(pool_out=self.bufs[t.buf], pool_out_ld=t.ld, pool_out_choff=t.choff,
                            pool_out_pad=self._pad_for(t.W))
+        if sums is not None:
+            act["sums"] = sums
         ops.bn_act_bwd(self.B, lay.H, lay.W, cb, lay.y, lay.cout, 0, lay.scale, lay.shift, lay.mean,
                        lay.invstd, lay.slope, lay.mode, g, g_ld, g_choff, dy, lay.cout_p, 0,
                        dgamma, dbeta, grad_scale, g2, g2_ld, g2_choff,
@@ -1232,6 +1272,7 @@
 
     def _backward_body(self, gmap, main, side, S, D, ready):
         pending, chunk = [], self.wgrad_chunk
+        sums_of = {}
 
         def flush():
             if not pending:
@@ -1276,7 +1317,7 @@
                     c2, t2 = self.consumer_of[lay.out2_id], lay.out2_t
                     g2, g2_ld, g2_choff = c2.gin, c2.tin.ld, t2.choff
                 self.bn_act_bwd_layer(lay, cons.gin, cons.tin.ld, t.choff, g2, g2_ld or 0, g2_choff or 0, lay.dy,
-                                      gmap[id(lay.bn.weight)], gmap[id(lay.bn.bias)], D)
+                                      gmap[id(lay.bn.weight)], gmap[id(lay.bn.bias)], D, sums=sums_of.pop(lay.li, None))
             mask = lay.conv.mask.contiguous() if lay.conv.mask_flag else None
             dbias = gmap[id(lay.conv.bias)] if lay.conv.bias is not None else None
             def wgrad_of(ws, lay=lay, mask=mask, dbias=dbias):
@@ -1307,9 +1348,12 @@
                 if len(pending) >= chunk or lay.li <= 1:
                     flush()
             if lay.li > 0:
+                conc = side is not None and self._side_concurrent
+                ds = self._dgrad_sums(lay, conc)
+                if ds is not None:
+                    sums_of[ds[2].li] = ds[1]
                 self._timed('dgrad', lay, ops.conv_dgrad_raw, lay.geom_act, lay.dy, lay.cout_p, 0, lay.wd, lay.gin, lay.tin.ld,
-                            lay.tin.choff, overflow=self.overflow,
-                            concurrent=side is not None and self._side_concurrent)
+                            lay.tin.choff, overflow=self.overflow, concurrent=conc, sums=ds[0] if ds is not None else None)
         if side is not None:
             flush()
             ops.stream_wait(main, side)
diff --git a/modelcompression_amd/ops.py b/modelcompression_amd/ops.py
--- a/modelcompression_amd/ops.py
+++ b/modelcompression_amd/ops.py
@@ -5,7 +5,7 @@
 import torch
 
 from . import _lib as L
-from ._lib import (ConvGeom, ConvEpilogue, ActDesc, ActBwdDesc, ChanMap, PackJob, StemBlockDesc, FoldDesc, FoldJob, check, ptr,
+from ._lib import (ConvGeom, ConvEpilogue, ActDesc, ActBwdDesc, DgradSums, ChanMap, PackJob, StemBlockDesc, FoldDesc, FoldJob, check, ptr,
                    stream_ptr)
 
 HALF = torch.float16
@@ -179,9 +179,31 @@
     check(L.lib().mcamd_conv_fwd(C.byref(g), ptr(x), ptr(wp), C.byref(e), stream_ptr()), "mcamd_conv_fwd")
 
 
-def conv_dgrad_raw(g, dy, dy_ld, dy_choff, wpd, out, out_ld, out_choff=0, overflow=None, concurrent=False):
+def dgrad_sums_rows(g, concurrent=False):
+    return int(L.lib().mcamd_conv_dgrad_sums_rows(C.byref(g), 1 if concurrent else 0))
+
+
+def dgrad_sums(slab, act, act_ld, act_choff, act_pad, scale, shift, mean, invstd, slope, C_, ch_lo=0, y=None, y_ld=0, y_choff=0):
+    _need_cuda(slab, act, scale, shift, mean, invstd, y)
+    assert slab.dtype == torch.float32 and slab.dim() == 3 and slab.shape[1] == 2 and slab.is_contiguous()
+    assert y is None or y.dtype == torch.float32
+    d = DgradSums()
+    d.slab, d.rows, d.ld = slab.data_ptr(), slab.shape[0], slab.shape[2]
+    d.act, d.act_ld, d.act_choff, d.act_pad = act.data_ptr(), act_ld, act_choff, act_pad
+    d.scale, d.shift, d.mean, d.invstd = scale.data_ptr(), shift.data_ptr(), mean.data_ptr(), invstd.data_ptr()
+    d.slope = slope
+    d.y, d.y_ld, d.y_choff = (y.data_ptr() if y is not None else None), y_ld, y_choff
+    d.ch_lo, d.C = ch_lo, C_
+    return d
+
+
+def conv_dgrad_raw(g, dy, dy_ld, dy_choff, wpd, out, out_ld, out_choff=0, overflow=None, concurrent=False, sums=None):
     e = _epi(L.EPI_RAW_F16, out, out_ld, out_choff, overflow=overflow)
     e.concurrent = 1 if concurrent else 0
+    if sums is not None:
+        check(L.lib().mcamd_conv_dgrad_sums(C.byref(g), ptr(dy), dy_ld, dy_choff, ptr(wpd), C.byref(e), C.byref(sums), stream_ptr()),
+              "mcamd_conv_dgrad_sums")
+        return
     check(L.lib().mcamd_conv_dgrad(C.byref(g), ptr(dy), dy_ld, dy_choff, ptr(wpd), C.byref(e), stream_ptr()),
           "mcamd_conv_dgrad")
 
@@ -309,8 +331,11 @@
 def bn_act_bwd(B, H, W, C_, y, y_ld, y_choff, scale, shift, mean, invstd, slope, mode, g, g_ld, g_choff, dy, dy_ld,
                dy_choff, dgamma, dbeta, grad_scale=1.0, g2=None, g2_ld=0, g2_choff=0, workspace=None, dy_keep=None,
                perm=None, overflow=None, skip_dead_from=0, dy_pad=0, act=None, act_ld=0, act_choff=0, act_pad=0,
-               pool_out=None, pool_out_ld=0, pool_out_choff=0, pool_out_pad=0):
+               pool_out=None, pool_out_ld=0, pool_out_choff=0, pool_out_pad=0, sums=None):
     d = ActBwdDesc()
+    if sums is not None:
+        assert sums.dtype == torch.float32 and sums.dim() == 3 and sums.shape[1] == 2 and sums.is_contiguous()
+        d.sums, d.sums_rows, d.sums_ld = sums.data_ptr(), sums.shape[0], sums.shape[2]
     d.skip_dead_param_grads = int(skip_dead_from)
     d.dy_pad = dy_pad
     d.B, d.H, d.W, d.C = B, H, W, C_
```
